# ogulcanaydogan/llm-slo-ebpf-toolkit

Measured on AMD Instinct MI355X. Metric: fault-replay attribution throughput through the agent's BPF-ring -> GPU path (events/s, node-wide); held-out attribution macro-F1 and agent CPU overhead % reported alongside, higher is better.
Workload: dtype fp64 posteriors / fp32 features (exact-int64 time joins)

## Files before the change

### llm_slo_ebpf_toolkit_amd/agent/worker.py

```python

from __future__ import annotations

import collections
import os
import time
import traceback
from dataclasses import dataclass, field
from typing import Deque, Dict, List, Optional, Tuple

import numpy as np

RING_TAIL = 8


@dataclass
class WorkerSpec:
    rank: int
    world: int
    device: int
    engine: str
    source: str
    ring_name: str
    pin_dir: str
    user_rec: int
    sig_cap: int
    span_cap: int
    group_cap: int
    user_cap: int
    window_ms: float
    ttft_slo_ms: float
    halo_ms: float
    import_cap: int
    xchg_cap: int
    model_image: bytes
    pods: Optional[Tuple[np.ndarray, np.ndarray]] = None
    master: Tuple[str, int] = ("127.0.0.1", 0)
    env: Dict[str, str] = field(default_factory=dict)
    halo_windows: int = 3
    split: bool = False
    app_image: bytes = b""
    open_requests: int = 0
    open_reorder_ms: float = 2000.0
    sli_sketch: int = 0
    exemplars: int = 0
    exemplar_windows: int = 3
    pod_breakdown: int = 0
    pod_windows: int = 3
    pod_pairs: int = 4096
    breach_onset: int = 0
    onset_bin_ns: int = 125_000_000
    onset_ref_ppm: int = 20000
    onset_alarm: int = 3


POD_RESULT_KEYS = tuple(f"pod_{s}_{f}" for s in ("win", "rec") for f in ("n", "b", "pods", "pods_b", "k_top", "top"))


def groups_of(rank: int, world: int, n_groups: int) -> int:
    return len(range(rank, n_groups, world))


def merge_results(parts: List[dict], n_groups: int) -> dict:
    world = len(parts)
    out = {}
    for key in ("post", "conf", "feat", "pred", "evbits", "sli", "app", "late", "sli_raw", "late_raw", "deadline",
                "deadline_dup", "ttft_n", "ttft_sum_ms", "ttft_le", "ttft_q", "ttft_q_roll", "ttft_n_roll", "ex_n",
                "ex_k_win", "ex_win", "ex_k_recent", "ex_recent", *POD_RESULT_KEYS, "onset_rows"):
        if key not in parts[0]:
            continue
        ref = np.asarray(parts[0][key])
        arr = np.zeros((n_groups,) + ref.shape[1:], dtype=ref.dtype)
        for r, p in enumerate(parts):
            n = groups_of(r, world, n_groups)
            arr[r::world][:n] = np.asarray(p[key])[:n]
        out[key] = arr
    return out


class PrevJoiner:

    def __init__(self, world: int):
        self.world = int(world)
        self.parts: Dict[int, Dict[int, dict]] = {}

    def add(self, replies) -> List[List[dict]]:
        for r in replies:
            for p in r.get("prevs", ()):
                self.parts.setdefault(int(p["k"]), {})[int(r["rank"])] = p
        out = []
        for k in sorted(self.parts):
            if len(self.parts[k]) < self.world:
                break
            got = self.parts.pop(k)
            out.append([got[i] for i in sorted(got)])
        return out

    def reset(self, world: int) -> None:
        self.world = int(world)
        self.parts.clear()


class WorkerCore:

    def __init__(self, spec: WorkerSpec, comm=None, group=None, shared: bool = True, rings=None):
        from ..collector import bpf
        from ..pipeline.window import RingWindowSource, WindowPipeline
        from ..runtime import load

        self.spec = spec
        shard = spec.rank if spec.split else 0
        if rings is None:
            rt = load()
            names = bpf.RingNames.of(spec.ring_name, shard)
            if spec.source == "bpf":
                ring = rt.Ringbuf.open_pinned(os.path.join(spec.pin_dir, "mislo_events" + (str(shard) if shard else "")))
            else:
                ring = rt.Ringbuf.attach_shm(names.ring)
            rings = (ring, rt.HostRing(0, spec.user_rec, names.user, True), rt.HostRing(0, 64, names.spans, True))
        ring, user, spans = rings
        self.rings = rings
        self.pipe = WindowPipeline(spec.sig_cap, spec.span_cap, spec.group_cap, spec.device, comm, model="bayes",
                                   learn=False, window_ms=2000.0, user_cap=spec.user_cap,
                                   ttft_slo_ms=spec.ttft_slo_ms, halo_ms=spec.halo_ms, halo_windows=spec.halo_windows,
                                   import_cap=spec.import_cap,
                                   xchg_cap=spec.xchg_cap, shard=(spec.rank, spec.world), engine=spec.engine,
                                   group=group, model_image=np.frombuffer(spec.model_image, dtype=np.uint8),
                                   split_rings=spec.split, open_requests=spec.open_requests,
                                   open_reorder_ms=spec.open_reorder_ms, sli_sketch=spec.sli_sketch,
                                   exemplars=spec.exemplars, exemplar_windows=spec.exemplar_windows,
                                   pod_breakdown=spec.pod_breakdown, pod_windows=spec.pod_windows,
                                   pod_pairs=spec.pod_pairs, breach_onset=spec.breach_onset,
                                   onset_bin_ns=spec.onset_bin_ns, onset_ref_ppm=spec.onset_ref_ppm,
                                   onset_alarm=spec.onset_alarm)
        self.src = RingWindowSource(self.pipe, ring, user, spans, cfg_set=lambda i, v: None,
                                    shared=shared and not spec.split)
        if spec.pods is not None:
            self.pipe.eng.set_pods(*spec.pods)
        if spec.app_image:
            from ..ops.engine import app_from_bytes

            img = np.frombuffer(spec.app_image, dtype=np.uint8)
            self.pipe.eng.set_app_model(img)
            self.pipe.app = self.pipe.model.app = app_from_bytes(img)
        self.pending: Deque[Tuple[int, float, int]] = collections.deque()
        self.windows = 0
        self.collect_s = self.collect_wait_s = 0.0

    @classmethod
    def adopt(cls, spec: WorkerSpec, pipe, src) -> "WorkerCore":
        core = cls.__new__(cls)
        core.spec, core.pipe, core.src = spec, pipe, src
        core.rings = (src.ring, src.user_ring, src.span_ring)
        core.pending = collections.deque()
        core.windows = 0
        core.collect_s = core.collect_wait_s = 0.0
        return core

    @property
    def max_pending(self) -> int:
        return max(1, int(self.pipe.nb) - 1)

    def window(self, cut, n_groups: int, pods=None, labels=None) -> dict:
        if pods is not None and len(pods[0]):
            self.pipe.eng.set_pods(*pods)
        t0 = time.perf_counter()
        r = self.src.stage(cut, n_groups, labels, with_labels=labels is not None, learn=False)
        host_us = 1e6 * (time.perf_counter() - t0)
        out = {"rank": self.spec.rank, "k": r["k"], "staged": r, "done": self.src.done()}
        self.pending.append((r["k"], host_us, n_groups))
        prevs = []
        while len(self.pending) > 1 and (len(self.pending) > self.max_pending or
                                         self.pipe.eng.query(self.pending[0][0])):
            prevs.append(self._collect(*self.pending.popleft()))
        out["prevs"] = prevs
        self.windows += 1
        return out

    def start_at(self, kernel: int, user: int, spans: int) -> dict:
        src = self.src
        if src.ring is not None:
            kernel = max(int(kernel), src.kpos)
            src.kpos = src.kernel_done = src.kernel_seen = kernel
            if not src.shared:
                src.ring.set_consumer_pos(max(src.ring.consumer_pos, kernel))
        if src.user_ring is not None:
            du = max(0, int(user) - src.upos)
            src.upos += du
            src._release_user(du, 0)
        if src.span_ring is not None:
            ds = max(0, int(spans) - src.spos)
            src.spos += ds
            src._release_user(0, ds)
        return {"rank": self.spec.rank, "done": src.done()}

    def collect(self, timeout_s: float) -> dict:
        deadline = time.perf_counter() + max(0.0, float(timeout_s))
        prevs = []
        while self.pending:
            k = self.pending[0][0]
            while not self.pipe.eng.query(k):
                if time.perf_counter() >= deadline:
                    return {"rank": self.spec.rank, "prevs": prevs}
                time.sleep(2e-4)
            prevs.append(self._collect(*self.pending.popleft()))
        if prevs:
            self.src.reap()
        return {"rank": self.spec.rank, "prevs": prevs}

    def _collect(self, k: int, host_us: float, n_groups: int) -> dict:
        pipe = self.pipe
        t0 = time.perf_counter()
        pipe.wait(k)
        t1 = time.perf_counter()
        self.collect_wait_s += t1 - t0
        try:
            return self._read(k, host_us, n_groups)
        finally:
            self.collect_s += time.perf_counter() - t0

    def _read(self, k: int, host_us: float, n_groups: int) -> dict:
        pipe = self.pipe
        pk = np.asarray(pipe.eng.packet(k), dtype=np.float64)
        d = {"k": k, "ring": pk[-RING_TAIL:].copy(), "host_us": host_us, "latency_ms": float(pipe.window_ms(k)[0])}
        if self.spec.rank == 0:
            d["packet"] = pk
            d["results"] = pipe.results_all(k, n_groups) if self.spec.world > 1 else [pipe.results(k, n_groups)]
            if pipe.tracker is not None:
                from ..pipeline.openreq import stats_dict

                d["open_requests"] = stats_dict(pipe.open_results(k, n_groups)["stats"])
            if pipe.sketch is not None:
                from ..pipeline.slisketch import stats_dict as sketch_stats

                d["ttft_sketch"] = sketch_stats(pipe.sli_results(k, n_groups)["stats"])
            if pipe.exemplars is not None:
                from ..pipeline.exemplars import stats_dict as exemplar_stats

                d["exemplars"] = exemplar_stats(pipe.exemplar_results(k, n_groups)["stats"])
            if pipe.pods is not None:
                from ..pipeline.podrank import stats_dict as pod_stats

                d["pod_breakdown"] = pod_stats(pipe.pod_results(k, n_groups)["stats"])
            if pipe.onset is not None:
                from ..pipeline.onset import stats_dict as onset_stats

                d["breach_onset"] = onset_stats(pipe.onset_results(k, n_groups)["stats"])
        return d

    def stop(self) -> dict:
        out = {"rank": self.spec.rank, "done": None, "prevs": []}
        while self.pending:
            out["prevs"].append(self._collect(*self.pending.popleft()))
        self.src.drain()
        out["done"] = self.src.done()
        out["summary"] = self.pipe.summary() if self.spec.rank == 0 else None
        return out

    def close(self) -> None:
        self.pipe.close()



def worker_main(spec: WorkerSpec, conn) -> None:
    os.environ.update(spec.env)
    core = None
    group = None
    try:
        comm = None
        if spec.world > 1 and spec.engine == "gpu":
            from ..ops import load_agent

            mod = load_agent()
            if spec.rank == 0:
                uid = mod.unique_id()
                conn.send(("uid", uid))
            else:
                uid = conn.recv()[1]
            comm = (uid, spec.rank, spec.world)
        elif spec.world > 1:
            import torch.distributed as dist

            os.environ.update(MASTER_ADDR=spec.master[0], MASTER_PORT=str(spec.master[1]))
            dist.init_process_group("gloo", rank=spec.rank, world_size=spec.world)
            group = dist.group.WORLD
        core = WorkerCore(spec, comm=comm, group=group, shared=True)
        conn.send(("ready", {"rank": spec.rank, "pid": os.getpid(), "device": spec.device}))
        while True:
            msg = conn.recv()
            if msg[0] == "window":
                conn.send(("window", core.window(*msg[1:])))
            elif msg[0] == "collect":
                conn.send(("collect", core.collect(*msg[1:])))
            elif msg[0] == "start_at":
                conn.send(("start_at", core.start_at(*msg[1:])))
            elif msg[0] == "stop":
                conn.send(("stopped", core.stop()))
                break
            else:
                raise ValueError(f"unknown worker message {msg[0]!r}")
    except (EOFError, KeyboardInterrupt):
        pass
    except Exception:
        try:
            conn.send(("error", traceback.format_exc()))
        except (OSError, BrokenPipeError):
            pass
        raise
    finally:
        if core is not None:
            core.close()
        if group is not None:
            import torch.distributed as dist

            dist.destroy_process_group()


class WorkerError(RuntimeError):
    def __init__(self, msg: str, rank: Optional[int] = None):
        super().__init__(msg)
        self.rank = rank


class RemoteWorker:

    def __init__(self, spec: WorkerSpec, ctx):
        self.spec = spec
        self.conn, child = ctx.Pipe()
        self.proc = ctx.Process(target=worker_main, args=(spec, child), name=f"mislo-worker-{spec.rank}", daemon=True)
        self.proc.start()
        child.close()

    @property
    def pid(self) -> int:
        return int(self.proc.pid or 0)

    def recv(self, timeout: float = 600.0):
        if not self.conn.poll(timeout):
            raise WorkerError(f"worker {self.spec.rank} did not answer in {timeout:.0f} s", self.spec.rank)
        try:
            msg = self.conn.recv()
        except (EOFError, OSError) as exc:
            raise WorkerError(f"worker {self.spec.rank} exited (code {self.proc.exitcode})", self.spec.rank) from exc
        if msg[0] == "error":
            raise WorkerError(f"worker {self.spec.rank} failed:\n{msg[1]}", self.spec.rank)
        return msg

    def ready(self) -> bool:
        return self.conn.poll(0)

    @property
    def alive(self) -> bool:
        return self.proc.is_alive()

    def send(self, msg) -> None:
        self.conn.send(msg)

    def close(self, timeout: float = 30.0) -> None:
        self.proc.join(timeout)
        if self.proc.is_alive():
            self.proc.terminate()
            self.proc.join(10)
        if self.proc.is_alive():
            self.proc.kill()
            self.proc.join(5)


class LocalWorker:

    def __init__(self, spec: WorkerSpec, rings=None):
        self.spec = spec
        self.core = WorkerCore(spec, shared=False, rings=rings)
        self._reply = None

    @property
    def pid(self) -> int:
        return os.getpid()

    def send(self, msg) -> None:
        if msg[0] == "window":
            self._reply = ("window", self.core.window(*msg[1:]))
        elif msg[0] == "collect":
            self._reply = ("collect", self.core.collect(*msg[1:]))
        elif msg[0] == "start_at":
            self._reply = ("start_at", self.core.start_at(*msg[1:]))
        elif msg[0] == "stop":
            self._reply = ("stopped", self.core.stop())

    def recv(self, timeout: float = 600.0):
        r, self._reply = self._reply, None
        return r

    def ready(self) -> bool:
        return True

    alive = True

    def close(self, timeout: float = 30.0) -> None:
        self.core.close()


class WorkerPool:

    def __init__(self, specs: List[WorkerSpec], rings, in_process: bool = False):
        import multiprocessing as mp

        self.rings = rings
        self.world = len(specs)
        if in_process:
            if self.world != 1:
                raise ValueError("in-process workers: exactly one")
            self.workers = [LocalWorker(specs[0], rings)]
        else:
            ctx = mp.get_context("spawn")
            self.workers = [RemoteWorker(s, ctx) for s in specs]
            try:
                if self.world > 1 and specs[0].engine == "gpu":
                    uid = self.workers[0].recv()[1]
                    for w in self.workers[1:]:
                        w.send(("uid", uid))
                for w in self.workers:
                    w.recv()
            except BaseException:
                self.close()
                raise
        self.in_process = in_process
        self.split = bool(specs[0].split) and self.world > 1
        r = rings
        self._rel_user = r[1].tail if r[1] is not None else 0
        self._rel_spans = r[2].tail if r[2] is not None else 0

    def pids(self) -> List[int]:
        return [w.pid for w in self.workers]

    def window(self, cut, n_groups: int, pods=None, timeout: float = 600.0) -> List[dict]:
        for w in self.workers:
            c = cut[w.spec.rank] if isinstance(cut, (list, tuple)) and not hasattr(cut, "kernel") else cut
            try:
                w.send(("window", c, groups_of(w.spec.rank, self.world, n_groups), pods))
            except (OSError, BrokenPipeError) as exc:
                raise WorkerError(f"worker {w.spec.rank} is gone ({exc})", w.spec.rank) from exc
        replies = self._gather(timeout)
        self._release(replies)
        return replies

    def collect(self, wait_s: float, timeout: float = 600.0) -> List[dict]:
        for w in self.workers:
            try:
                w.send(("collect", float(wait_s)))
            except (OSError, BrokenPipeError) as exc:
                raise WorkerError(f"worker {w.spec.rank} is gone ({exc})", w.spec.rank) from exc
        return self._gather(max(timeout, wait_s + 30.0))

    def start_at(self, positions, timeout: float = 120.0) -> List[dict]:
        for w in self.workers:
            pos = positions[w.spec.rank] if isinstance(positions, list) else positions
            try:
                w.send(("start_at",) + tuple(int(x) for x in pos))
            except (OSError, BrokenPipeError) as exc:
                raise WorkerError(f"worker {w.spec.rank} is gone ({exc})", w.spec.rank) from exc
        replies = self._gather(timeout)
        self._release(replies)
        return replies

    def _gather(self, timeout: float) -> List[dict]:
        replies: List[Optional[dict]] = [None] * self.world
        deadline = time.monotonic() + timeout
        while any(r is None for r in replies):
            got = False
            for i, w in enumerate(self.workers):
                if replies[i] is None and w.ready():
                    replies[i] = w.recv()[1]
                    got = True
            if got:
                continue
            dead = self.dead_ranks()
            if dead:
                raise WorkerError(f"worker {dead[0]} exited", dead[0])
            if time.monotonic() > deadline:
                late = next(i for i, r in enumerate(replies) if r is None)
                raise WorkerError(f"worker {late} did not answer in {timeout:.0f} s", late)
            time.sleep(0.0005)
        return replies

    def dead_ranks(self) -> List[int]:
        return [w.spec.rank for w in self.workers if not w.alive]

    def _release(self, replies: List[dict]) -> None:
        if self.in_process or self.split:
            return
        ring, user, spans = self.rings
        dones = [r["done"] for r in replies if r.get("done") is not None]
        if not dones:
            return
        k = min(d[0] for d in dones)
        if ring is not None and k > ring.consumer_pos:
            ring.set_consumer_pos(k)
        u = min(d[1] for d in dones)
        if user is not None and u > self._rel_user:
            user.release(u - self._rel_user)
            self._rel_user = u
        s = min(d[2] for d in dones)
        if spans is not None and s > self._rel_spans:
            spans.release(s - self._rel_spans)
            self._rel_spans = s

    def stop(self) -> List[dict]:
        for w in self.workers:
            w.send(("stop",))
        replies = []
        for w in self.workers:
            try:
                replies.append(w.recv(120)[1])
            except WorkerError:
                replies.append({"rank": w.spec.rank, "done": None})
        self._release(replies)
        return replies

    def close(self, timeout: float = 30.0) -> None:
        for w in self.workers:
            w.close(timeout)
```

### llm_slo_ebpf_toolkit_amd/ops/csrc/agent_bindings.cpp

```cpp
#include <pybind11/numpy.h>
#include <pybind11/pybind11.h>
#include <pybind11/stl.h>

#include <cstring>
#include <memory>
#include <stdexcept>

#include "engine.h"
#include "exemplars.h"
#include "onset.h"
#include "openreq.h"
#include "podrank.h"
#include "slisketch.h"

namespace py = pybind11;
using namespace mislo;

namespace {

template <class T>
py::array_t<T> copy_array(const T* p, std::vector<py::ssize_t> shape) {
  py::array_t<T> a(shape);
  size_t n = 1;
  for (auto s : shape) n *= (size_t)s;
  if (n) std::memcpy(a.mutable_data(), p, n * sizeof(T));
  return a;
}

void set_tables_np(py::array_t<int8_t, py::array::c_style | py::array::forcecast> type_slot,
                   py::array_t<float, py::array::c_style | py::array::forcecast> scale,
                   py::array_t<float, py::array::c_style | py::array::forcecast> warn,
                   py::array_t<float, py::array::c_style | py::array::forcecast> err,
                   py::array_t<float, py::array::c_style | py::array::forcecast> edges) {
  Tables t;
  std::memset(&t, 0, sizeof(t));
  if (type_slot.size() != kMaxTypes || scale.size() != kSlots || warn.size() != kSlots || err.size() != kSlots ||
      edges.size() != kSlots * kBuckets)
    throw std::invalid_argument("table shapes");
  std::memcpy(t.type_slot, type_slot.data(), sizeof(t.type_slot));
  std::memcpy(t.scale, scale.data(), sizeof(t.scale));
  std::memcpy(t.warn, warn.data(), sizeof(t.warn));
  std::memcpy(t.err, err.data(), sizeof(t.err));
  std::memcpy(t.edges, edges.data(), sizeof(t.edges));
  engine_set_tables(t);
}

}

class PyEngine {
 public:
  PyEngine(int device, int sig_cap, int span_cap, int group_cap, int user_cap, int n_buffers, int max_ahead,
           double window_ms, double threshold, int fanout, int group_mode, bool use_graphs, bool device_refit,
           int n_dom, float ttft_slo_ms, double halo_ms, int import_cap, int xchg_cap, int shard_rank,
           int shard_world, int halo_windows, bool split_rings) {
    if (shard_world < 1 || shard_rank < 0 || shard_rank >= shard_world) throw std::invalid_argument("shard rank / world");
    EngineConfig c;
    c.device = device;
    c.sig_cap = sig_cap;
    c.span_cap = span_cap;
    c.group_cap = group_cap;
    c.user_cap = user_cap;
    c.n_buffers = n_buffers;
    c.max_ahead = max_ahead;
    c.window_ms = window_ms;
    c.threshold = threshold;
    c.fanout = fanout;
    c.group_mode = group_mode;
    c.use_graphs = use_graphs;
    c.device_refit = device_refit;
    c.n_dom = n_dom;
    c.ttft_slo_ms = ttft_slo_ms;
    c.halo_ms = halo_ms;
    c.halo_windows = halo_windows;
    c.import_cap = import_cap;
    c.xchg_cap = xchg_cap;
    c.shard_rank = shard_rank;
    c.shard_world = shard_world;
    c.split_rings = split_rings;
    e_ = std::make_unique<WindowEngine>(c);
  }
  bool register_host(uintptr_t addr, size_t bytes) {
    return e_->register_host(reinterpret_cast<const void*>(addr), bytes);
  }
  void submit(int64_t k, const std::vector<std::pair<uintptr_t, size_t>>& kernel,
              const std::vector<std::pair<uintptr_t, size_t>>& user,
              const std::vector<std::pair<uintptr_t, size_t>>& spans, int n_groups, py::object labels,
              std::vector<int64_t> bases, bool with_labels, bool learn, int user_rec) {
    WindowInput in;
    auto conv = [](const std::vector<std::pair<uintptr_t, size_t>>& v, std::vector<Seg>& out) {
      for (auto& p : v) out.push_back(Seg{reinterpret_cast<const void*>(p.first), p.second});
    };
    conv(kernel, in.kernel);
    conv(user, in.user);
    conv(spans, in.spans);
    in.n_groups = n_groups;
    in.user_rec = user_rec;
    std::vector<int32_t> lab;
    if (!labels.is_none()) {
      auto arr = labels.cast<py::array_t<int32_t, py::array::c_style | py::array::forcecast>>();
      lab.assign(arr.data(), arr.data() + arr.size());
      lab.resize(std::max<size_t>(lab.size(), (size_t)std::max(0, n_groups)), -1);
      in.labels = lab.data();
    }
    bases.resize(4, 0);
    for (int q = 0; q < 4; ++q) in.bases[q] = bases[q];
    py::gil_scoped_release nogil;
    e_->submit(k, in, with_labels, learn);
  }
  bool h2d_done(int64_t k) { return e_->h2d_done(k); }
  void wait_h2d(int64_t k) {
    py::gil_scoped_release nogil;
    e_->wait_h2d(k);
  }
  bool query(int64_t k) { return e_->query(k); }
  void wait(int64_t k) {
    py::gil_scoped_release nogil;
    e_->wait(k);
  }
  py::array_t<double> packet(int64_t k) { return copy_array(e_->packet(k), {kPacketLen}); }
  py::dict results(int64_t k, int n_groups) {
    if (n_groups < 0 || n_groups > eng().config().group_cap) throw std::invalid_argument("n_groups");
    return result_dict(e_->results(k), n_groups);
  }
  py::list results_all(int64_t k, int n_groups) {
    WindowEngine& e = eng();
    if (n_groups < 0 || n_groups > e.config().group_cap) throw std::invalid_argument("n_groups");
    const ResultLayout lay = e.layout();
    const uint8_t* base = e.results_all(k);
    py::list out;
    const int w = e.has_comm() ? e.world() : 1;
    for (int r = 0; r < w; ++r) out.append(result_dict(lay.view(base + (size_t)r * lay.bytes()), n_groups));
    return out;
  }
  static py::dict result_dict(const ResultView& r, int n_groups) {
    const py::ssize_t G = n_groups;
    py::dict d;
    d["post"] = copy_array(r.post, {G, 16});
    d["conf"] = copy_array(r.gconf, {G});
    d["feat"] = copy_array(r.feat, {G, 16});
    d["pred"] = copy_array(r.pred, {G});
    d["evbits"] = copy_array(r.evbits, {G, 16});
    d["sli"] = copy_array(r.sli, {G, 2});
    d["app"] = copy_array(r.app, {G, 2});
    d["late"] = copy_array(r.late, {G, 2});
    return d;
  }
  py::tuple window_ms(int64_t k) {
    std::pair<float, float> t;
    {
      py::gil_scoped_release nogil;
      t = e_->window_ms(k);
    }
    return py::make_tuple(t.first, t.second);
  }
  void set_model_bytes(py::array_t<uint8_t, py::array::c_style | py::array::forcecast> b) {
    e_->set_model_bytes(b.data(), (size_t)b.size());
  }
  void set_app_model(py::array_t<uint8_t, py::array::c_style | py::array::forcecast> b) {
    e_->set_app_model(b.data(), (size_t)b.size());
  }
  void set_refit(double alpha, double prior_pseudo, double inv_temp, double min_count, int cap_dom, double ceil) {
    eng().set_refit(alpha, prior_pseudo, inv_temp, min_count, cap_dom, ceil);
  }
  void refit_now() { eng().refit_now(); }
  py::dict score(py::array_t<float, py::array::c_style | py::array::forcecast> feat, py::object labels,
                 py::object app) {
    if (feat.ndim() != 2 || feat.shape(1) != 16) throw std::invalid_argument("feat must be float32 [n, 16]");
    const int n = (int)feat.shape(0);
    std::vector<int32_t> lab;
    if (!labels.is_none()) {
      auto a = labels.cast<py::array_t<int32_t, py::array::c_style | py::array::forcecast>>();
      if (a.size() != n) throw std::invalid_argument("labels must have n entries");
      lab.assign(a.data(), a.data() + n);
    }
    std::vector<uint32_t> appc;
    if (!app.is_none()) {
      auto a = app.cast<py::array_t<uint32_t, py::array::c_style | py::array::forcecast>>();
      if (a.size() != 2 * (py::ssize_t)n) throw std::invalid_argument("app must be uint32 [n, 2]");
      appc.assign(a.data(), a.data() + 2 * (size_t)n);
    }
    std::vector<double> post((size_t)n * 16), conf(n);
    std::vector<int32_t> pred(n);
    std::vector<uint32_t> ev((size_t)n * 16), cm(256);
    {
      py::gil_scoped_release nogil;
      eng().score_features(feat.data(), n, lab.empty() ? nullptr : lab.data(), post.data(), pred.data(), conf.data(),
                           ev.data(), cm.data(), appc.empty() ? nullptr : appc.data());
    }
    py::dict d;
    d["post"] = copy_array(post.data(), {n, 16});
    d["pred"] = copy_array(pred.data(), {n});
    d["conf"] = copy_array(conf.data(), {n});
    d["evbits"] = copy_array(ev.data(), {n, 16});
    d["confusion"] = copy_array(cm.data(), {16, 16});
    return d;
  }
  void set_p0(py::array_t<double, py::array::c_style | py::array::forcecast> p0) {
    if (p0.size() != kSlots * 16 && p0.size() != 2 * kSlots * 16)
      throw std::invalid_argument("p0 must be f64[256] (table) or f64[512] (table, floor)");
    e_->set_p0(p0.data(), (size_t)p0.size());
  }
  void set_pods(py::array_t<uint32_t, py::array::c_style | py::array::forcecast> pods,
                py::array_t<uint32_t, py::array::c_style | py::array::forcecast> sn) {
    if (pods.size() != sn.size()) throw std::invalid_argument("pods / svcnode size mismatch");
    e_->set_pods(pods.data(), sn.data(), (size_t)pods.size());
  }
  void inject_remote(py::buffer blocks, size_t stride, int world, int me) {
    py::buffer_info bi = blocks.request();
    if ((size_t)(bi.size * bi.itemsize) < stride * (size_t)std::max(world, 0)) throw std::invalid_argument("blocks too small");
    py::gil_scoped_release nogil;
    eng().inject_remote(bi.ptr, stride, world, me);
  }
  void set_join_params(double window_ms, double threshold, int fanout, int group_mode) {
    e_->set_join_params(window_ms, threshold, fanout, group_mode);
  }
  void init_comm(py::bytes id, int rank, int world) {
    std::string s = id;
    if (s.size() != sizeof(ncclUniqueId)) throw std::invalid_argument("unique id size");
    ncclUniqueId u;
    std::memcpy(&u, s.data(), sizeof(u));
    py::gil_scoped_release nogil;
    e_->init_comm(u, rank, world);
  }
  py::array_t<double> totals() {
    std::vector<double> t(kPacketLen);
    {
      py::gil_scoped_release nogil;
      e_->totals(t.data());
    }
    return copy_array(t.data(), {kPacketLen});
  }
  void reset_totals() {
    py::gil_scoped_release nogil;
    e_->reset_totals();
  }
  py::array_t<double> stats_acc() {
    std::vector<double> t(kStatsLen);
    {
      py::gil_scoped_release nogil;
      e_->stats_acc(t.data());
    }
    return copy_array(t.data(), {kStatsLen});
  }
  void restore(py::array_t<double, py::array::c_style | py::array::forcecast> stats,
               py::array_t<uint8_t, py::array::c_style | py::array::forcecast> model, int64_t folded) {
    if (stats.size() != kStatsLen) throw std::invalid_argument("stats must be f64[STATS_LEN]");
    eng().restore(stats.data(), model.data(), (size_t)model.size(), folded);
  }
  py::array_t<uint8_t> model_bytes() {
    std::vector<uint8_t> t(sizeof(PosteriorModel));
    {
      py::gil_scoped_release nogil;
      e_->model_bytes(t.data());
    }
    return copy_array(t.data(), {(py::ssize_t)t.size()});
  }
  void sync() {
    py::gil_scoped_release nogil;
    e_->sync();
  }
  std::vector<int64_t> import_state() {
    py::gil_scoped_release nogil;
    return eng().import_state();
  }
  py::bytes sent_block() {
    std::vector<uint8_t> b;
    {
      py::gil_scoped_release nogil;
      b = eng().sent_block();
    }
    return py::bytes(reinterpret_cast<const char*>(b.data()), b.size());
  }
  void close() {
    if (e_) {
      py::gil_scoped_release nogil;
      e_->sync();
      e_.reset();
    }
  }
  WindowEngine& eng() {
    if (!e_) throw std::logic_error("engine closed");
    return *e_;
  }
  int buffers() { return eng().buffers(); }
  int64_t folded() { return eng().windows_folded(); }
  size_t graphs() { return eng().graphs(); }
  double host_issue_us() { return eng().host_issue_us(); }
  double host_wait_us() { return eng().host_wait_us(); }
  double host_dma_issue_us() { return eng().host_dma_issue_us(); }
  double host_launch_us() { return eng().host_launch_us(); }
  bool has_comm() { return eng().has_comm(); }
  size_t staged_bytes() { return eng().staged_bytes(); }
  size_t direct_bytes() { return eng().direct_bytes(); }

 private:
  std::unique_ptr<WindowEngine> e_;
};

class PyOpenRequests {
 public:
  PyOpenRequests(int device, int64_t cap, int span_cap, int group_cap, int n_buffers, double slo_ms, double ttl_ms,
                 double reorder_ms) {
    openreq::Config c;
    c.device = device;
    c.cap = cap;
    c.span_cap = span_cap;
    c.group_cap = group_cap;
    c.n_buffers = n_buffers;
    c.slo_ms = slo_ms;
    c.ttl_ms = ttl_ms;
    c.reorder_ms = reorder_ms;
    openreq::validate(c);
    t_ = std::make_unique<OpenRequests>(c);
  }
  OpenRequests& t() {
    if (!t_) throw std::logic_error("open-request tracker closed");
    return *t_;
  }
  int64_t step(const std::vector<std::pair<uintptr_t, size_t>>& spans, int64_t cut_ns, int64_t prev_cut_ns,
               int n_groups) {
    OpenRequests& tr = t();
    py::gil_scoped_release nogil;
    return tr.step(spans, cut_ns, prev_cut_ns, n_groups);
  }
  bool query(int64_t i) { return t().query(i); }
  py::dict results(int64_t i, int n_groups) {
    OpenRequests& tr = t();
    if (n_groups < 0 || n_groups > tr.config().group_cap) throw std::invalid_argument("n_groups");
    const uint32_t* r;
    {
      py::gil_scoped_release nogil;
      r = tr.results(i);
    }
    const openreq::Layout& l = tr.result_layout();
    py::dict d;
    d["dl"] = copy_array(r + l.dl, {n_groups, 2});
    d["dup"] = copy_array(r + l.dup, {n_groups, 3});
    d["stats"] = copy_array(r + l.stats, {openreq::kStats});
    return d;
  }
  py::tuple step_ms(int64_t i) {
    std::pair<float, float> ms;
    {
      py::gil_scoped_release nogil;
      ms = t().step_ms(i);
    }
    return py::make_tuple(ms.first, ms.second);
  }
  py::tuple entries() {
    std::vector<uint64_t> k;
    std::vector<int64_t> tt;
    std::vector<uint32_t> g, s;
    {
      py::gil_scoped_release nogil;
      t().entries(k, tt, g, s);
    }
    const py::ssize_t n = (py::ssize_t)k.size();
    return py::make_tuple(copy_array(k.data(), {n}), copy_array(tt.data(), {n}), copy_array(g.data(), {n}),
                          copy_array(s.data(), {n}));
  }
  void sync() {
    py::gil_scoped_release nogil;
    t().sync();
  }
  void close() {
    if (t_) {
      py::gil_scoped_release nogil;
      t_.reset();
    }
  }

 private:
  std::unique_ptr<OpenRequests> t_;
};

class PySliSketch {
 public:
  PySliSketch(int device, int span_cap, int group_cap, int windows, int n_buffers) {
    slisketch::Config c;
    c.device = device;
    c.span_cap = span_cap;
    c.group_cap = group_cap;
    c.windows = windows;
    c.n_buffers = n_buffers;
    slisketch::validate(c);
    t_ = std::make_unique<SliSketch>(c);
  }
  SliSketch& t() {
    if (!t_) throw std::logic_error("ttft sketch closed");
    return *t_;
  }
  int64_t step(const std::vector<std::pair<uintptr_t, size_t>>& spans, int n_groups) {
    SliSketch& sk = t();
    py::gil_scoped_release nogil;
    return sk.step(spans, n_groups);
  }
  bool query(int64_t i) { return t().query(i); }
  py::dict results(int64_t i, int n_groups) {
    SliSketch& sk = t();
    if (n_groups < 0 || n_groups > sk.config().group_cap) throw std::invalid_argument("n_groups");
    const uint32_t* r;
    {
      py::gil_scoped_release nogil;
      r = sk.results(i);
    }
    const slisketch::Layout& l = sk.result_layout();
    const py::ssize_t G = n_groups;
    std::vector<uint64_t> sum((size_t)G);
    for (py::ssize_t g = 0; g < G; ++g)
      sum[(size_t)g] = (uint64_t)r[l.sum + 2 * g] | ((uint64_t)r[l.sum + 2 * g + 1] << 32);
    py::dict d;
    d["n"] = copy_array(r + l.n, {G});
    d["sum_milli"] = copy_array(sum.data(), {G});
    d["le"] = copy_array(r + l.le, {G, slisketch::kLe});
    d["q_win"] = copy_array(r + l.q_win, {G, slisketch::kQuantiles});
    d["n_roll"] = copy_array(r + l.n_roll, {G});
    d["q_roll"] = copy_array(r + l.q_roll, {G, slisketch::kQuantiles});
    d["stats"] = copy_array(r + l.stats, {slisketch::kStats});
    return d;
  }
  py::tuple step_ms(int64_t i) {
    std::pair<float, float> ms;
    {
      py::gil_scoped_release nogil;
      ms = t().step_ms(i);
    }
    return py::make_tuple(ms.first, ms.second);
  }
  py::array_t<uint32_t> rolling() { return rows(true); }
  py::array_t<uint32_t> window_hist() { return rows(false); }
  void sync() {
    py::gil_scoped_release nogil;
    t().sync();
  }
  void close() {
    if (t_) {
      py::gil_scoped_release nogil;
      t_.reset();
    }
  }

 private:
  py::array_t<uint32_t> rows(bool roll) {
    SliSketch& sk = t();
    std::vector<uint32_t> h;
    {
      py::gil_scoped_release nogil;
      h = roll ? sk.rolling() : sk.window_hist();
    }
    return copy_array(h.data(), {sk.config().group_cap, slisketch::kK});
  }
  std::unique_ptr<SliSketch> t_;
};

class PyExemplarTracker {
 public:
  PyExemplarTracker(int device, int k, int windows, int64_t span_cap, int group_cap, int n_buffers, bool lds) {
    if (span_cap < 1 || span_cap >= (int64_t(1) << 31))
      throw std::invalid_argument("request exemplars: span_cap must be in [1, 2^31)");
    exemplars::Config c;
    c.device = device;
    c.k = k;
    c.windows = windows;
    c.span_cap = (int)span_cap;
    c.group_cap = group_cap;
    c.n_buffers = n_buffers;
    c.lds = lds;
    exemplars::validate(c);
    t_ = std::make_unique<ExemplarTracker>(c);
  }
  ExemplarTracker& t() {
    if (!t_) throw std::logic_error("request exemplars closed");
    return *t_;
  }
  int64_t step(const std::vector<std::pair<uintptr_t, size_t>>& spans, int n_groups) {
    ExemplarTracker& ex = t();
    py::gil_scoped_release nogil;
    return ex.step(spans, n_groups);
  }
  bool query(int64_t i) { return t().query(i); }
  py::dict results(int64_t i, int n_groups) {
    ExemplarTracker& ex = t();
    if (n_groups < 0 || n_groups > ex.config().group_cap) throw std::invalid_argument("n_groups");
    const uint32_t* r;
    {
      py::gil_scoped_release nogil;
      r = ex.results(i);
    }
    const exemplars::Layout& l = ex.result_layout();
    const py::ssize_t G = n_groups, K = ex.config().k;
    py::dict d;
    d["n"] = copy_array(r + l.n, {G});
    d["k_win"] = copy_array(r + l.k_win, {G});
    d["k_recent"] = copy_array(r + l.k_recent, {G});
    d["win"] = copy_array(reinterpret_cast<const uint8_t*>(r + l.win), {G, K, exemplars::kRowBytes});
    d["recent"] = copy_array(reinterpret_cast<const uint8_t*>(r + l.recent), {G, K, exemplars::kRowBytes});
    d["stats"] = copy_array(r + l.stats, {exemplars::kStats});
    return d;
  }
  py::tuple step_ms(int64_t i) {
    std::vector<float> ms;
    {
      py::gil_scoped_release nogil;
      ms = t().step_ms(i);
    }
    return py::make_tuple(ms[0], ms[1], ms[2]);
  }
  py::tuple resident() {
    ExemplarTracker& ex = t();
    std::pair<std::vector<exemplars::Row>, std::vector<uint32_t>> h;
    {
      py::gil_scoped_release nogil;
      h = ex.resident();
    }
    const py::ssize_t H = ex.config().windows, G = ex.config().group_cap, K = ex.config().k;
    return py::make_tuple(copy_array(reinterpret_cast<const uint8_t*>(h.first.data()), {H, G, K, exemplars::kRowBytes}),
                          copy_array(h.second.data(), {H, G}));
  }
  void sync() {
    py::gil_scoped_release nogil;
    t().sync();
  }
  void close() {
    if (t_) {
      py::gil_scoped_release nogil;
      t_.reset();
    }
  }

 private:
  std::unique_ptr<ExemplarTracker> t_;
};

class PyPodRankTracker {
 public:
  PyPodRankTracker(int device, int k, int windows, int64_t pair_cap, int64_t span_cap, int group_cap, int n_buffers,
                   double slo_ms, bool lds) {
    if (span_cap < 1 || span_cap >= (int64_t(1) << 31))
      throw std::invalid_argument("pod breakdown: span_cap must be >= 1 and span_cap * windows < 2^22");
    if (pair_cap < 1 || pair_cap > podrank::kMaxPairCap)
      throw std::invalid_argument("pod breakdown: pair_cap must be in [1, 2^20]");
    podrank::Config c;
    c.device = device;
    c.k = k;
    c.windows = windows;
    c.pair_cap = (int)pair_cap;
    c.span_cap = (int)span_cap;
    c.group_cap = group_cap;
    c.n_buffers = n_buffers;
    c.slo_ms = slo_ms;
    c.lds = lds;
    podrank::validate(c);
    t_ = std::make_unique<PodRankTracker>(c);
  }
  PodRankTracker& t() {
    if (!t_) throw std::logic_error("pod breakdown closed");
    return *t_;
  }
  int64_t step(const std::vector<std::pair<uintptr_t, size_t>>& spans, int n_groups) {
    PodRankTracker& pr = t();
    py::gil_scoped_release nogil;
    return pr.step(spans, n_groups);
  }
  bool query(int64_t i) { return t().query(i); }
  py::dict results(int64_t i, int n_groups) {
    PodRankTracker& pr = t();
    if (n_groups < 0 || n_groups > pr.config().group_cap) throw std::invalid_argument("n_groups");
    const uint32_t* r;
    {
      py::gil_scoped_release nogil;
      r = pr.results(i);
    }
    const podrank::Layout& l = pr.result_layout();
    const py::ssize_t G = n_groups, K = pr.config().k;
    static const char* scope[2] = {"win", "rec"};
    py::dict d;
    for (int s = 0; s < 2; ++s) {
      const std::string p = std::string(scope[s]) + "_";
      d[py::str(p + "n")] = copy_array(r + l.n[s], {G});
      d[py::str(p + "b")] = copy_array(r + l.b[s], {G});
      d[py::str(p + "pods")] = copy_array(r + l.pods[s], {G});
      d[py::str(p + "pods_b")] = copy_array(r + l.pods_b[s], {G});
      d[py::str(p + "k_top")] = copy_array(r + l.k_top[s], {G});
      d[py::str(p + "top")] = copy_array(reinterpret_cast<const uint8_t*>(r + l.top[s]), {G, K, podrank::kRowBytes});
    }
    d["stats"] = copy_array(r + l.stats, {podrank::kStats});
    return d;
  }
  py::tuple step_ms(int64_t i) {
    std::vector<float> ms;
    {
      py::gil_scoped_release nogil;
      ms = t().step_ms(i);
    }
    return py::make_tuple(ms[0], ms[1], ms[2]);
  }
  py::list resident() {
    PodRankTracker& pr = t();
    std::vector<podrank::PairList> h;
    {
      py::gil_scoped_release nogil;
      h = pr.resident();
    }
    py::list out;
    for (const podrank::PairList& l : h) {
      const py::ssize_t n = (py::ssize_t)l.key.size();
      out.append(py::make_tuple(copy_array(reinterpret_cast<const uint64_t*>(l.key.data()), {n}), copy_array(l.n.data(), {n}),
                                copy_array(l.b.data(), {n}), copy_array(l.max.data(), {n}),
                                copy_array(reinterpret_cast<const uint64_t*>(l.sum.data()), {n})));
    }
    return out;
  }
  void sync() {
    py::gil_scoped_release nogil;
    t().sync();
  }
  void close() {
    if (t_) {
      py::gil_scoped_release nogil;
      t_.reset();
    }
  }

 private:
  std::unique_ptr<PodRankTracker> t_;
};

class PyOnsetTracker {
 public:
  PyOnsetTracker(int device, int64_t bins, int64_t bin_ns, int64_t ref_ppm, int64_t alarm, int64_t span_cap, int group_cap,
                 int n_buffers, double slo_ms, int64_t ring_records_max, bool lds) {
    if (bins < onset::kMinBins || bins > onset::kMaxBins)
      throw std::invalid_argument("breach onset: bins must be a power of two in [64, 8192]");
    if (span_cap < 1) throw std::invalid_argument("breach onset: span_cap must be >= 1");
    if (span_cap >= (int64_t(1) << 31)) throw std::invalid_argument("breach onset: the ring needs more than 2 GiB");
    onset::Config c;
    c.device = device;
    c.bins = (int)bins;
    c.bin_ns = bin_ns;
    c.ref_ppm = ref_ppm;
    c.alarm = alarm;
    c.span_cap = (int)span_cap;
    c.group_cap = group_cap;
    c.n_buffers = n_buffers;
    c.slo_ms = slo_ms;
    c.ring_records_max = ring_records_max;
    c.lds = lds;
    onset::validate(c);
    t_ = std::make_unique<OnsetTracker>(c);
  }
  OnsetTracker& t() {
    if (!t_) throw std::logic_error("breach onset closed");
    return *t_;
  }
  int64_t step(const std::vector<std::pair<uintptr_t, size_t>>& spans, int64_t cut_ns, int n_groups) {
    OnsetTracker& on = t();
    py::gil_scoped_release nogil;
    return on.step(spans, cut_ns, n_groups);
  }
  bool query(int64_t i) { return t().query(i); }
  py::dict results(int64_t i, int n_groups) {
    OnsetTracker& on = t();
    if (n_groups < 0 || n_groups > on.config().group_cap) throw std::invalid_argument("n_groups");
    const uint32_t* r;
    {
      py::gil_scoped_release nogil;
      r = on.results(i);
    }
    const onset::Layout& l = on.result_layout();
    py::dict d;
    d["rows"] = copy_array(reinterpret_cast<const uint8_t*>(r + l.rows), {(py::ssize_t)n_groups, onset::kRowBytes});
    d["stats"] = copy_array(r + l.stats, {onset::kStats});
    return d;
  }
  py::tuple step_ms(int64_t i) {
    std::vector<float> ms;
    {
      py::gil_scoped_release nogil;
      ms = t().step_ms(i);
    }
    return py::make_tuple(ms[0], ms[1], ms[2]);
  }
  py::tuple resident() {
    OnsetTracker& on = t();
    onset::Resident h;
    {
      py::gil_scoped_release nogil;
      h = on.resident();
    }
    return py::make_tuple(copy_array(reinterpret_cast<const uint64_t*>(h.cells.data()),
                                     {(py::ssize_t)on.config().group_cap, (py::ssize_t)on.config().bins}),
                          h.q_hi);
  }
  void sync() {
    py::gil_scoped_release nogil;
    t().sync();
  }
  void close() {
    if (t_) {
      py::gil_scoped_release nogil;
      t_.reset();
    }
  }

 private:
  std::unique_ptr<OnsetTracker> t_;
};

py::bytes unique_id() {
  ncclUniqueId u;
  const ncclResult_t r = ncclGetUniqueId(&u);
  if (r != ncclSuccess) throw std::runtime_error(std::string("ncclGetUniqueId: ") + ncclGetErrorString(r));
  return py::bytes(reinterpret_cast<const char*>(&u), sizeof(u));
}

PYBIND11_MODULE(_mislo_agent, m) {
  m.doc() = "MI355X LLM-SLO native window engine (HIP + RCCL, no PyTorch)";
  m.def("set_tables", &set_tables_np);
  m.def("unique_id", &unique_id);
  m.def("device_count", []() {
    int n = 0;
    return hipGetDeviceCount(&n) == hipSuccess ? n : 0;
  });
  m.attr("PACKET_LEN") = kPacketLen;
  m.attr("PACKET_LAYOUT") = py::make_tuple(kPacketHist, kPacketStatus, kPacketMisc, kPacketDbg, kPacketConf,
                                           kPacketStats, kPacketCount, kPacketRing);
  m.attr("STATS_OFF") = kStatsOff;
  m.attr("STATS_LEN") = kStatsLen;
  m.attr("POSTERIOR_MODEL_BYTES") = (int64_t)sizeof(PosteriorModel);
  m.attr("APP_MODEL_BYTES") = (int64_t)sizeof(AppModel);
  m.attr("APP_EVIDENCE_BIT") = kAppBit;
  m.attr("CTX_ROWS") = kCtxRows;
  m.attr("REC_STRIDE") = kRecStride;
  m.attr("SIGREC_BYTES") = (int)sizeof(SigRec);
  m.attr("RING_STATE") =
      py::make_tuple("first_busy", "foreign", "def_ctx", "def_trace", "discarded", "events", "other_shard");
  m.attr("OPENREQ_LDS_GROUPS") = openreq::kLdsGroups;
  m.attr("OPENREQ_MAX_PROBES") = openreq::kMaxProbes;
  m.attr("OPENREQ_STATS") = (int)openreq::kStats;
  py::class_<PyOpenRequests>(m, "OpenRequests")
      .def(py::init<int, int64_t, int, int, int, double, double, double>(), py::arg("device") = 0,
           py::arg("cap") = (int64_t)1 << 20, py::arg("span_cap") = 16384, py::arg("group_cap") = 64,
           py::arg("n_buffers") = 3, py::arg("slo_ms") = 800.0, py::arg("ttl_ms") = 120000.0,
           py::arg("reorder_ms") = 2000.0)
      .def("step", &PyOpenRequests::step, py::arg("spans"), py::arg("cut_ns"), py::arg("prev_cut_ns"),
           py::arg("n_groups"))
      .def("query", &PyOpenRequests::query)
      .def("results", &PyOpenRequests::results)
      .def("step_ms", &PyOpenRequests::step_ms)
      .def("entries", &PyOpenRequests::entries)
      .def("sync", &PyOpenRequests::sync)
      .def("close", &PyOpenRequests::close);
  m.attr("SLISKETCH_K") = slisketch::kK;
  m.attr("SLISKETCH_LO_KEY") = slisketch::kLo;
  m.attr("SLISKETCH_STATS") = (int)slisketch::kStats;
  {
    py::list edges, q;
    for (int j = 0; j < slisketch::kEdges; ++j) edges.append((double)slisketch::le_edge(j));
    for (int j = 0; j < slisketch::kQuantiles; ++j) q.append(slisketch::quantile_permille(j));
    m.attr("SLISKETCH_EDGES") = py::tuple(edges);
    m.attr("SLISKETCH_PERMILLE") = py::tuple(q);
  }
  py::class_<PySliSketch>(m, "SliSketch")
      .def(py::init<int, int, int, int, int>(), py::arg("device") = 0, py::arg("span_cap") = 16384,
           py::arg("group_cap") = 64, py::arg("windows") = 150, py::arg("n_buffers") = 3)
      .def("step", &PySliSketch::step, py::arg("spans"), py::arg("n_groups"))
      .def("query", &PySliSketch::query)
      .def("results", &PySliSketch::results)
      .def("step_ms", &PySliSketch::step_ms)
      .def("rolling", &PySliSketch::rolling)
      .def("window_hist", &PySliSketch::window_hist)
      .def("sync", &PySliSketch::sync)
      .def("close", &PySliSketch::close);
  m.attr("EXEMPLAR_MAX_K") = exemplars::kMaxK;
  m.attr("EXEMPLAR_MAX_H") = exemplars::kMaxH;
  m.attr("EXEMPLAR_LDS_GROUPS") = exemplars::kLdsGroups;
  m.attr("EXEMPLAR_ROW_BYTES") = exemplars::kRowBytes;
  m.attr("EXEMPLAR_STATS") = (int)exemplars::kStats;
  py::class_<PyExemplarTracker>(m, "ExemplarTracker")
      .def(py::init<int, int, int, int64_t, int, int, bool>(), py::arg("device") = 0, py::arg("k") = 3,
           py::arg("windows") = 3, py::arg("span_cap") = 16384, py::arg("group_cap") = 64, py::arg("n_buffers") = 3,
           py::arg("lds") = true)
      .def("step", &PyExemplarTracker::step, py::arg("spans"), py::arg("n_groups"))
      .def("query", &PyExemplarTracker::query)
      .def("results", &PyExemplarTracker::results)
      .def("step_ms", &PyExemplarTracker::step_ms)
      .def("resident", &PyExemplarTracker::resident)
      .def("sync", &PyExemplarTracker::sync)
      .def("close", &PyExemplarTracker::close);
  m.attr("PODRANK_MAX_K") = podrank::kMaxK;
  m.attr("PODRANK_MAX_H") = podrank::kMaxH;
  m.attr("PODRANK_ROW_BYTES") = podrank::kRowBytes;
  m.attr("PODRANK_STATS") = (int)podrank::kStats;
  m.attr("PODRANK_LDS_SLOTS") = podrank::kLdsSlots;
  m.def("podrank_slot_of", [](uint32_t g, uint32_t pod, uint32_t slots) { return podrank::slot_of(g, pod, slots); });
  py::class_<PyPodRankTracker>(m, "PodRankTracker")
      .def(py::init<int, int, int, int64_t, int64_t, int, int, double, bool>(), py::arg("device") = 0, py::arg("k") = 3,
           py::arg("windows") = 3, py::arg("pair_cap") = 4096, py::arg("span_cap") = 16384, py::arg("group_cap") = 64,
           py::arg("n_buffers") = 3, py::arg("slo_ms") = 800.0, py::arg("lds") = true)
      .def("step", &PyPodRankTracker::step, py::arg("spans"), py::arg("n_groups"))
      .def("query", &PyPodRankTracker::query)
      .def("results", &PyPodRankTracker::results)
      .def("step_ms", &PyPodRankTracker::step_ms)
      .def("resident", &PyPodRankTracker::resident)
      .def("sync", &PyPodRankTracker::sync)
      .def("close", &PyPodRankTracker::close);
  m.attr("ONSET_ROW_BYTES") = onset::kRowBytes;
  m.attr("ONSET_STATS") = (int)onset::kStats;
  m.attr("ONSET_LDS_SLOTS") = onset::kLdsSlots;
  m.attr("ONSET_BINS") = py::make_tuple(onset::kMinBins, onset::kMaxBins);
  py::class_<PyOnsetTracker>(m, "OnsetTracker")
      .def(py::init<int, int64_t, int64_t, int64_t, int64_t, int64_t, int, int, double, int64_t, bool>(),
           py::arg("device") = 0, py::arg("bins") = 1024, py::arg("bin_ns") = (int64_t)125000000,
           py::arg("ref_ppm") = (int64_t)20000, py::arg("alarm") = (int64_t)3, py::arg("span_cap") = 16384,
           py::arg("group_cap") = 64, py::arg("n_buffers") = 3, py::arg("slo_ms") = 800.0,
           py::arg("ring_records_max") = onset::kMaxRingRecords, py::arg("lds") = true)
      .def("step", &PyOnsetTracker::step, py::arg("spans"), py::arg("cut_ns"), py::arg("n_groups"))
      .def("query", &PyOnsetTracker::query)
      .def("results", &PyOnsetTracker::results)
      .def("step_ms", &PyOnsetTracker::step_ms)
      .def("resident", &PyOnsetTracker::resident)
      .def("sync", &PyOnsetTracker::sync)
      .def("close", &PyOnsetTracker::close);
  py::class_<PyEngine>(m, "WindowEngine")
      .def(py::init<int, int, int, int, int, int, int, double, double, int, int, bool, bool, int, float, double, int,
                    int, int, int, int, bool>(),
           py::arg("device") = 0, py::arg("sig_cap") = 1 << 20, py::arg("span_cap") = 16384, py::arg("group_cap") = 64,
           py::arg("user_cap") = 1 << 18, py::arg("n_buffers") = 3, py::arg("max_ahead") = 3,
           py::arg("window_ms") = 2000.0, py::arg("threshold") = 0.7, py::arg("fanout") = 3, py::arg("group_mode") = 1,
           py::arg("use_graphs") = true, py::arg("device_refit") = true, py::arg("n_dom") = 10,
           py::arg("ttft_slo_ms") = 800.0f, py::arg("halo_ms") = 0.0, py::arg("import_cap") = 0,
           py::arg("xchg_cap") = 0, py::arg("shard_rank") = 0, py::arg("shard_world") = 1,
           py::arg("halo_windows") = 3, py::arg("split_rings") = false)
      .def("register_host", &PyEngine::register_host)
      .def("submit", &PyEngine::submit, py::arg("k"), py::arg("kernel"), py::arg("user"), py::arg("spans"),
           py::arg("n_groups"), py::arg("labels") = py::none(), py::arg("bases") = std::vector<int64_t>{},
           py::arg("with_labels") = true, py::arg("learn") = false, py::arg("user_rec") = 64)
      .def("h2d_done", &PyEngine::h2d_done)
      .def("wait_h2d", &PyEngine::wait_h2d)
      .def("query", &PyEngine::query)
      .def("wait", &PyEngine::wait)
      .def("packet", &PyEngine::packet)
      .def("results", &PyEngine::results)
      .def("window_ms", &PyEngine::window_ms)
      .def("copy_ms", [](PyEngine& p, int64_t k) {
        py::gil_scoped_release nogil;
        return p.eng().copy_ms(k);
      })
      .def("set_model_bytes", &PyEngine::set_model_bytes)
      .def("set_app_model", &PyEngine::set_app_model)
      .def("set_p0", &PyEngine::set_p0)
      .def("set_refit", &PyEngine::set_refit, py::arg("alpha") = 2.0, py::arg("prior_pseudo") = 1.0,
           py::arg("inv_temp") = 1.0, py::arg("min_count") = 0.0, py::arg("cap_dom") = -1, py::arg("ceil") = 1.0)
      .def("refit_now", &PyEngine::refit_now)
      .def("set_device_refit", [](PyEngine& p, bool on) { p.eng().set_device_refit(on); })
      .def("score", &PyEngine::score, py::arg("feat"), py::arg("labels") = py::none(), py::arg("app") = py::none())
      .def("set_pods", &PyEngine::set_pods)
      .def("inject_remote", &PyEngine::inject_remote)
      .def("results_all", &PyEngine::results_all)
      .def("set_join_params", &PyEngine::set_join_params)
      .def("init_comm", &PyEngine::init_comm)
      .def("totals", &PyEngine::totals)
      .def("reset_totals", &PyEngine::reset_totals)
      .def("stats_acc", &PyEngine::stats_acc)
      .def("model_bytes", &PyEngine::model_bytes)
      .def("restore", &PyEngine::restore)
      .def("sync", &PyEngine::sync)
      .def("import_state", &PyEngine::import_state)
      .def("sent_block", &PyEngine::sent_block)
      .def("close", &PyEngine::close)
      .def_property_readonly("buffers", &PyEngine::buffers)
      .def_property_readonly("copy_lanes", [](PyEngine& p) { return p.eng().copy_lanes(); })
      .def_property_readonly("windows_folded", &PyEngine::folded)
      .def_property_readonly("graphs", &PyEngine::graphs)
      .def_property_readonly("host_issue_us", &PyEngine::host_issue_us)
      .def_property_readonly("host_wait_us", &PyEngine::host_wait_us)
      .def_property_readonly("host_dma_issue_us", &PyEngine::host_dma_issue_us)
      .def_property_readonly("host_launch_us", &PyEngine::host_launch_us)
      .def_property_readonly("host_pre_us", [](PyEngine& p) { return p.eng().host_pre_us(); })
      .def_property_readonly("host_dma_split_us", [](PyEngine& p) { return p.eng().host_dma_split_us(); })
      .def_property_readonly("host_tail_us", [](PyEngine& p) { return p.eng().host_tail_us(); })
      .def_property_readonly("has_comm", &PyEngine::has_comm)
      .def_property_readonly("rank", [](PyEngine& p) { return p.eng().rank(); })
      .def_property_readonly("world", [](PyEngine& p) { return p.eng().world(); })
      .def_property_readonly("staged_bytes", &PyEngine::staged_bytes)
      .def_property_readonly("direct_bytes", &PyEngine::direct_bytes);
}
```

### llm_slo_ebpf_toolkit_amd/ops/csrc/copylanes.h

```cpp
#pragma once

#include <cstdint>

namespace mislo {

constexpr int kMaxCopyLanes = 2;

inline int copy_lane(int64_t k, int lanes) { return lanes > 1 ? (int)(k % lanes) : 0; }

inline int copy_consults(int64_t k, int lanes, int64_t out[kMaxCopyLanes]) {
  int n = 0;
  for (int i = 0; i < (lanes > 1 ? lanes : 1) && k - i >= 0; ++i) out[n++] = k - i;
  return n;
}

struct CopiedUpTo {
  int64_t n = 0;

  void reused(int64_t k, int nb) {
    if (k - nb + 1 > n) n = k - nb + 1;
  }

  template <class Ready>
  bool done(int64_t k, int lanes, Ready&& ready) {
    if (k < n) return true;
    int64_t w[kMaxCopyLanes];
    const int c = copy_consults(k, lanes, w);
    for (int i = 0; i < c; ++i)
      if (w[i] >= n && !ready(w[i])) return false;
    n = k + 1;
    return true;
  }
};

}
```

### llm_slo_ebpf_toolkit_amd/ops/csrc/engine.h

```cpp
#pragma once

#include <hip/hip_runtime.h>
#include <rccl/rccl.h>

#include <map>
#include <tuple>
#include <type_traits>
#include <vector>

#include "copylanes.h"
#include "mislo_launch.h"
#include "mislo_packet.h"

namespace mislo {

constexpr uint32_t kCtxRows = 1u << 24;
constexpr uint32_t kPodRows = 1u << 20;
constexpr uint32_t kTraceIdRows = 1u << 24;
constexpr int kHeadBytes = 64;

struct Seg {
  const void* ptr;
  size_t bytes;
};

struct EngineConfig {
  int device = 0;
  int sig_cap = 1 << 20, span_cap = 16384, group_cap = 64;
  int user_cap = 1 << 18;
  int n_buffers = 3, max_ahead = 3;
  double window_ms = 2000.0, threshold = 0.7;
  int fanout = 3, group_mode = 1;
  bool use_graphs = true;
  bool device_refit = true;
  double alpha = 2.0, prior_pseudo = 1.0;
  double inv_temp = 1.0, min_count = 0.0;
  int cap_dom = -1;
  double lik_ceil = 1.0;
  int n_dom = 10;
  float ttft_slo_ms = 800.0f;
  double halo_ms = 0.0;
  int halo_windows = 3;
  int import_cap = 0;
  int xchg_cap = 0;
  int shard_rank = 0, shard_world = 1;
  bool split_rings = false;
};

template <class Byte>
struct ResultViewT {
  template <class T>
  using P = std::conditional_t<std::is_const_v<Byte>, const T, T>*;
  P<double> post;
  P<double> gconf;
  P<float> feat;
  P<int32_t> pred;
  P<uint32_t> evbits;
  P<uint32_t> sli;
  P<uint32_t> app;
  P<uint32_t> late;
};
using ResultView = ResultViewT<const uint8_t>;

struct ResultLayout {
  size_t G;
  size_t gconf() const { return 16 * G * 8; }
  size_t feat() const { return gconf() + G * 8; }
  size_t pred() const { return feat() + 16 * G * 4; }
  size_t evbits() const { return pred() + G * 4; }
  size_t sli() const { return evbits() + 16 * G * 4; }
  size_t bytes() const { return sli() + 6 * G * 4; }
  template <class Byte>
  ResultViewT<Byte> view(Byte* r) const {
    ResultViewT<Byte> v;
    auto set = [r](auto& p, size_t off) { p = reinterpret_cast<std::remove_reference_t<decltype(p)>>(r + off); };
    set(v.post, 0), set(v.gconf, gconf()), set(v.feat, feat()), set(v.pred, pred()), set(v.evbits, evbits());
    set(v.sli, sli()), set(v.app, sli() + 2 * G * 4), set(v.late, sli() + 4 * G * 4);
    return v;
  }
};

struct WindowInput {
  std::vector<Seg> kernel;
  std::vector<Seg> user;
  int user_rec = 64;
  std::vector<Seg> spans;
  int n_groups = 0;
  const int32_t* labels = nullptr;
  int64_t bases[4] = {0, 0, 0, 0};
};

class WindowEngine {
 public:
  explicit WindowEngine(const EngineConfig& cfg);
  ~WindowEngine();
  WindowEngine(const WindowEngine&) = delete;
  WindowEngine& operator=(const WindowEngine&) = delete;

  const EngineConfig& config() const { return cfg_; }
  int buffers() const { return nb_; }

  bool register_host(const void* ptr, size_t bytes);
  void submit(int64_t k, const WindowInput& in, bool with_labels, bool learn);
  bool h2d_done(int64_t k);
  void wait_h2d(int64_t k);
  int copy_lanes() const { return lanes_; }
  bool query(int64_t k);
  void wait(int64_t k);
  const double* packet(int64_t k) const { return bufs_[k % nb_].packet_host; }
  ResultView results(int64_t k) const { return layout().view<const uint8_t>(bufs_[k % nb_].res_host); }
  ResultLayout layout() const { return ResultLayout{(size_t)cfg_.group_cap}; }
  std::pair<float, float> window_ms(int64_t k);
  std::vector<float> copy_ms(int64_t k);

  void set_model_bytes(const void* bytes, size_t n);
  void set_refit(double alpha, double prior_pseudo, double inv_temp, double min_count, int cap_dom = -1,
                 double ceil = 1.0);
  void refit_now();
  void set_device_refit(bool on) { cfg_.device_refit = on; }
  void score_features(const float* feat, int n, const int32_t* labels, double* post, int32_t* pred, double* conf,
                      uint32_t* evbits, uint32_t* confusion, const uint32_t* app_cnt = nullptr);
  void set_app_model(const void* bytes, size_t n);
  void set_p0(const double* p0, size_t n);
  void set_pods(const uint32_t* pods, const uint32_t* svcnode, size_t n);
  void inject_remote(const void* blocks, size_t stride, int world, int me);
  void set_join_params(double window_ms, double threshold, int fanout, int group_mode);
  void init_comm(const ncclUniqueId& id, int rank, int world);
  bool has_comm() const { return comm_ != nullptr; }
  int rank() const { return rank_; }
  int world() const { return world_; }
  const uint8_t* results_all(int64_t k) const { return comm_ ? bufs_[k % nb_].res_all_host : bufs_[k % nb_].res_host; }
  size_t result_bytes() const { return layout().bytes(); }

  void totals(double* out);
  void reset_totals();
  void stats_acc(double* out);
  void restore(const double* stats, const void* model, size_t model_bytes, int64_t folded);
  void model_bytes(void* out);
  void sync();
  std::vector<int64_t> import_state();
  std::vector<uint8_t> sent_block();
  int64_t windows_folded() const { return folded_; }
  size_t staged_bytes() const { return staged_bytes_; }
  size_t direct_bytes() const { return direct_bytes_; }
  size_t graphs() const { return graphs_.size(); }
  double host_issue_us() const { return issue_n_ ? issue_us_ / issue_n_ : 0.0; }
  double host_wait_us() const { return issue_n_ ? wait_us_ / issue_n_ : 0.0; }
  double host_dma_issue_us() const { return issue_n_ ? dma_us_ / issue_n_ : 0.0; }
  double host_launch_us() const { return issue_n_ ? launch_us_ / issue_n_ : 0.0; }
  double host_pre_us() const { return issue_n_ ? pre_us_ / issue_n_ : 0.0; }
  double host_tail_us() const { return issue_n_ ? tail_us_ / issue_n_ : 0.0; }

 private:
  int rec_shard_rank() const { return cfg_.split_rings ? 0 : cfg_.shard_rank; }
  int rec_shard_world() const { return cfg_.split_rings ? 1 : cfg_.shard_world; }
  struct Buf;
  enum class Stage : int { Window, Records, Join, XchgSpans, XchgHead, Front, Back };
  static constexpr int kStageSlots = 8;
  void alloc();
  void enable_span_branch();
  void run_begin(const Buf& buf, hipStream_t st);
  void run_part1(const Buf& buf, hipStream_t st, bool xchg);
  void run_join_front(const Buf& buf, hipStream_t st, bool xchg);
  void run_join_back(const Buf& buf, int n_groups, bool with_labels, bool learn, hipStream_t st);
  void run_span_branch(const Buf& buf, hipStream_t st);
  void run_spans(const Buf& buf, hipStream_t st);
  void launch_part(Stage part, const Buf& buf, int n_groups, bool with_labels, bool learn);
  void merge_remote(const Buf& buf, const uint8_t* blocks, size_t stride, int world, int me, hipStream_t st);
  void refit(const double* add);
  SignalCols sig_cols(const Buf& buf) const;
  SpanCols span_cols(const Buf& buf) const;
  bool registered(const void* p, size_t n) const;
  size_t dma(const std::vector<Seg>& segs, uint8_t* dst, size_t cap, uint8_t*& staging, size_t& st_off,
             hipStream_t st);
  struct Owner {
    std::vector<hipEvent_t> events;
    std::vector<void*> dev, host;
    std::vector<hipStream_t> streams;
    void free_dev(void* p);
    ~Owner();
  } own_;
  template <class T>
  T* dalloc(size_t n, bool zero = false);
  void* host_alloc(size_t bytes, unsigned flags);
  void* host_block(size_t bytes);
  hipEvent_t mk_event(unsigned flags);
  hipStream_t mk_stream(bool high_priority = false);

  EngineConfig cfg_;
  int nb_, max_ahead_;
  size_t off_kern_ = 0, off_user_ = 0, off_span_ = 0, in_bytes_ = 0;
  size_t kern_bytes() const { return (size_t)kRecStride * (((size_t)cfg_.sig_cap + kBatchSlots - 1) / kBatchSlots); }
  std::vector<std::pair<const uint8_t*, size_t>> registered_;
  size_t staged_bytes_ = 0, direct_bytes_ = 0;
  uint32_t *pod_sn_ = nullptr, *pod_host_ = nullptr;
  unsigned long long* trace_hash_ = nullptr;
  AppModel* app_dev_ = nullptr;
  int n_rows_ = 0;
  int gens_ = 1;
  int slots_ = 1;
  unsigned long long* tmax_ = nullptr;
  KeyTs* g_keys_ = nullptr;
  uint32_t *remote_n_ = nullptr, *sel_cnt_ = nullptr, *sel_off_ = nullptr;
  unsigned long long* sel_mask_ = nullptr;
  int sel_stride_ = 0;
  uint8_t *xsend_ = nullptr, *xrecv_ = nullptr;
  size_t xstride_ = 0, xrecv_bytes_ = 0;
  int nblk_imp_ = 0;
  bool spin_ = false;
  std::vector<uint8_t> inject_;
  size_t inject_stride_ = 0;
  int inject_world_ = 0, inject_me_ = 0;
  int rank_ = 0, world_ = 1;
  hipStream_t side_ = nullptr;
  hipStream_t front_ = nullptr;
  bool overlap_ = false;
  struct BufSet {
    GenMeta* gen;
    int* rows;
    uint32_t *ring_state, *hist, *status, *confusion, *cnt, *gcnt;
    unsigned long long *misc, *dbg, *top3, *gsum;
    double *stats, *stats_count;
    SpanRec* s_rec;
    PartCodes* s_part;
    uint32_t *s_items, *s_part_base, *probe_work;
    PreSpan* s_pre;
  };
  std::vector<BufSet> sets_;
  struct Buf {
    int b;
    uint8_t* in;
    uint8_t* head_host;
    uint8_t* staging;
    double *packet_dev, *packet_host;
    uint8_t *res_dev, *res_host;
    uint8_t *res_all_dev, *res_all_host;
    ResultViewT<uint8_t> res;
    SigRec* imp;
    uint32_t* remote_n;
    const BufSet* set;
    const GenMeta* gen_prev;
    hipEvent_t h2d_done, head_done, front_done, compute_done, comm_done, xchg_done;
    hipEvent_t t_start, t_comp0, t_comp1, t_end;
    const int* counts() const { return reinterpret_cast<const int*>(in); }
  };
  std::vector<Buf> bufs_;
  hipEvent_t ev_fork_ = nullptr, ev_sigbase_ = nullptr, ev_spans_ = nullptr;
  bool branch_ = false;
  bool xspan_ = false;
  bool exchange() const { return comm_ && cfg_.xchg_cap > 0 && cfg_.import_cap > 0; }
  JoinParams jp_{};
  int nblk_sig_ = 1, nblk_span_ = 1;
  hipStream_t copy_[kMaxCopyLanes] = {nullptr, nullptr};
  int lanes_ = 1;
  CopiedUpTo copied_;
  bool copied_ready(int64_t w, bool block);
  hipStream_t compute_ = nullptr, comm_stream_ = nullptr;
  ncclComm_t comm_ = nullptr;
  ncclComm_t xcomm_ = nullptr;
  uint32_t* ctx_tab_ = nullptr;
  double *totals_ = nullptr, *stats_acc_ = nullptr, *p0_ = nullptr;
  uint8_t* model_dev_ = nullptr;
  std::vector<uint8_t*> model_host_;
  int model_slot_ = 0;
  uint8_t* g_status_ = nullptr;
  PartCodes* g_part_ = nullptr;
  uint32_t *g_part_blk_ = nullptr, *g_part_off_ = nullptr, *g_part_tot_ = nullptr, *g_part_base_ = nullptr,
           *g_items_ = nullptr;
  SigRec* g_rec_ = nullptr;
  uint32_t *s_part_blk_ = nullptr, *s_part_off_ = nullptr, *s_part_tot_ = nullptr;
  float *attrs_ = nullptr, *conf_ = nullptr, *kernel_ms_ = nullptr;
  std::map<std::tuple<int, int, bool, bool>, hipGraphExec_t> graphs_;
  std::vector<bool> warm_;
  std::vector<hipGraph_t> graph_defs_;
  int64_t submitted_ = 0, folded_ = 0;
  double issue_us_ = 0, wait_us_ = 0, dma_us_ = 0, launch_us_ = 0, pre_us_ = 0, tail_us_ = 0;
  double split_us_[4] = {0, 0, 0, 0};

 public:
  std::vector<double> host_dma_split_us() const {
    std::vector<double> v;
    for (double x : split_us_) v.push_back(issue_n_ ? x / issue_n_ : 0.0);
    return v;
  }

 private:
  int64_t issue_n_ = 0;
};

void engine_set_tables(const Tables& t);

}
```

### llm_slo_ebpf_toolkit_amd/ops/csrc/engine.hip

```cpp
#include "engine.h"
#include "mislo_packet_kernels.h"

#include <algorithm>
#include <chrono>
#include <cstdlib>
#include <cmath>
#include <cstring>
#include <stdexcept>
#include <string>

namespace mislo {

namespace {

#define HIPCHECK(x)                                                                                  \
  do {                                                                                               \
    hipError_t _e = (x);                                                                             \
    if (_e != hipSuccess) throw std::runtime_error(std::string("HIP error: ") + hipGetErrorString(_e) + \
                                                   " at " #x);                                       \
  } while (0)

#define NCCLCHECK(x)                                                                                        \
  do {                                                                                                      \
    ncclResult_t _r = (x);                                                                                  \
    if (_r != ncclSuccess) throw std::runtime_error(std::string("RCCL error: ") + ncclGetErrorString(_r) + \
                                                    " at " #x);                                             \
  } while (0)

__global__ void k_accumulate(const double* __restrict__ packet, double* __restrict__ totals, int n,
                             double* __restrict__ host) {
  const int i = blockIdx.x * blockDim.x + threadIdx.x;
  if (i < n) {
    const double v = packet[i];
    totals[i] += v;
    host[i] = v;
  }
}

__global__ __launch_bounds__(256) void k_window_end(const uint32_t* hist, const uint32_t* status,
                                                    const unsigned long long* misc, const unsigned long long* dbg,
                                                    const uint32_t* confusion, const double* stats, const double* count,
                                                    const uint32_t* ring, double* __restrict__ packet,
                                                    double* __restrict__ totals, double* __restrict__ packet_host,
                                                    const uint4* __restrict__ res, uint4* __restrict__ res_host,
                                                    size_t res16) {
  const size_t t = blockIdx.x * (size_t)blockDim.x + threadIdx.x, stride = (size_t)gridDim.x * blockDim.x;
  if (t < (size_t)kPacketLen) {
    const double v = packet_value((int)t, hist, status, misc, dbg, confusion, stats, count, ring);
    packet[t] = v;
    totals[t] += v;
    packet_host[t] = v;
  }
  for (size_t i = t; i < res16; i += stride) res_host[i] = res[i];
}

__global__ void k_to_host(const uint4* __restrict__ src, uint4* __restrict__ dst, size_t n16) {
  for (size_t i = blockIdx.x * (size_t)blockDim.x + threadIdx.x; i < n16; i += (size_t)gridDim.x * blockDim.x)
    dst[i] = src[i];
}

void to_host(const void* src, void* dst, size_t bytes, hipStream_t st) {
  const size_t n16 = (bytes + 15) / 16;
  const int g = (int)std::min<size_t>(64, (n16 + 255) / 256);
  hipLaunchKernelGGL(k_to_host, dim3(g > 0 ? g : 1), dim3(256), 0, st, static_cast<const uint4*>(src),
                     static_cast<uint4*>(dst), n16);
}

constexpr unsigned kEvWait = hipEventDisableTiming | hipEventBlockingSync;
int env_int(const char* name, int unset) {
  const char* v = getenv(name);
  return v ? atoi(v) : unset;
}

struct Lap {
  using clock = std::chrono::steady_clock;
  clock::time_point t = clock::now();
  void operator()(double& acc) {
    const auto n = clock::now();
    acc += std::chrono::duration<double, std::micro>(n - t).count();
    t = n;
  }
};

}

void engine_set_tables(const Tables& t) { set_tables(&t); }

template <class T>
T* WindowEngine::dalloc(size_t n, bool zero) {
  void* p = nullptr;
  HIPCHECK(hipMalloc(&p, n * sizeof(T) + 64));
  own_.dev.push_back(p);
  if (zero) HIPCHECK(hipMemset(p, 0, n * sizeof(T)));
  return static_cast<T*>(p);
}

void* WindowEngine::host_alloc(size_t bytes, unsigned flags) {
  void* h = nullptr;
  HIPCHECK(hipHostMalloc(&h, bytes, flags));
  own_.host.push_back(h);
  return h;
}

void* WindowEngine::host_block(size_t bytes) {
  void* h = host_alloc((bytes + 15) & ~size_t(15), hipHostMallocCoherent | hipHostMallocMapped);
  std::memset(h, 0, bytes);
  return h;
}

hipEvent_t WindowEngine::mk_event(unsigned flags) {
  hipEvent_t e;
  HIPCHECK(hipEventCreateWithFlags(&e, flags));
  own_.events.push_back(e);
  return e;
}

hipStream_t WindowEngine::mk_stream(bool high_priority) {
  hipStream_t s;
  int lo = 0, hi = 0;
  if (high_priority) {
    HIPCHECK(hipDeviceGetStreamPriorityRange(&lo, &hi));
    HIPCHECK(hipStreamCreateWithPriority(&s, hipStreamNonBlocking, hi));
  } else {
    HIPCHECK(hipStreamCreateWithFlags(&s, hipStreamNonBlocking));
  }
  own_.streams.push_back(s);
  return s;
}

void WindowEngine::Owner::free_dev(void* p) {
  if (!p) return;
  dev.erase(std::find(dev.begin(), dev.end(), p));
  HIPCHECK(hipFree(p));
}

WindowEngine::Owner::~Owner() {
  for (hipEvent_t e : events) (void)hipEventDestroy(e);
  for (void* p : host) (void)hipHostFree(p);
  for (void* p : dev) (void)hipFree(p);
  for (hipStream_t s : streams) (void)hipStreamDestroy(s);
}

WindowEngine::WindowEngine(const EngineConfig& cfg) : cfg_(cfg) {
  if (cfg.sig_cap <= 0 || cfg.span_cap <= 0 || cfg.group_cap <= 0 || cfg.group_cap > 4096)
    throw std::invalid_argument("capacities out of range");
  if (cfg.sig_cap >= (1 << 27)) throw std::invalid_argument("sig_cap must be < 2^27 (top-3 key packing)");
  nb_ = std::max(2, cfg.n_buffers);
  max_ahead_ = std::min(nb_, std::max(1, cfg.max_ahead));
  if (cfg.user_cap <= 0 || cfg.user_cap > cfg.sig_cap) throw std::invalid_argument("user_cap must be in [1, sig_cap]");
  if (cfg.import_cap < 0 || cfg.xchg_cap < 0 || cfg.halo_ms < 0) throw std::invalid_argument("negative import sizes");
  if (cfg.halo_windows < 1 || cfg.halo_windows >= kMaxGens)
    throw std::invalid_argument("halo_windows must be in [1, 3] (resident generations)");
  gens_ = cfg.halo_ms > 0 ? 1 + cfg.halo_windows : 1;
  if (2LL * gens_ * ((long long)cfg.sig_cap + cfg.import_cap) >= (1LL << 27))
    throw std::invalid_argument("2 x generations x (sig_cap + import_cap) must be < 2^27 (top-3 key packing)");
  HIPCHECK(hipSetDevice(cfg.device));
  set_join_params(cfg.window_ms, cfg.threshold, cfg.fanout, cfg.group_mode);
  alloc();
}

void WindowEngine::set_join_params(double window_ms, double threshold, int fanout, int group_mode) {
  const int64_t ms = 1000000;
  int64_t outer = (int64_t)llround(window_ms * ms);
  if (outer <= 0) outer = 2000 * ms;
  if (outer >= (1LL << 35)) throw std::invalid_argument("window too large for top-3 key packing (< 34 s)");
  jp_.outer_ns = outer;
  const int64_t tw[4] = {outer, 100 * ms, 250 * ms, 500 * ms};
  for (int k = 0; k < 4; ++k) jp_.win_ns[k] = std::min(outer, tw[k]);
  const float cf[4] = {1.0f, 0.9f, 0.8f, 0.65f};
  for (int k = 0; k < 4; ++k) jp_.conf[k] = cf[k];
  jp_.threshold = threshold > 0 ? (float)threshold : 0.7f;
  if (fanout <= 0) fanout = 3;
  if (fanout > 3) throw std::invalid_argument("GPU join keeps at most 3 candidates per span");
  jp_.fanout = fanout;
  jp_.group_mode = group_mode;
  graphs_.clear();
}

void WindowEngine::alloc() {
  const int64_t S = cfg_.span_cap, G = cfg_.group_cap;
  n_rows_ = cfg_.sig_cap + cfg_.import_cap;
  const int64_t N = n_rows_;
  nblk_sig_ = decode_grid((int)N);
  nblk_span_ = decode_grid((int)S);
  const bool one_stream = env_int("MISLO_ONE_STREAM", 0) == 1;
  compute_ = mk_stream();
  copy_[0] = one_stream ? compute_ : mk_stream();
  spin_ = env_int("MISLO_SPIN_WAIT", 0) == 1;
  overlap_ = env_int("MISLO_WINDOW_OVERLAP", !one_stream) == 1 && !one_stream &&
             !(cfg_.xchg_cap > 0 && cfg_.import_cap > 0);
  if (overlap_) front_ = mk_stream();
  lanes_ = overlap_ && env_int("MISLO_COPY_LANES", nb_ >= 4 ? 2 : 1) == 2 ? 2 : 1;
  copy_[1] = lanes_ == 2 ? mk_stream(env_int("MISLO_COPY_LANE_PRIO", 1) != 0) : copy_[0];
  slots_ = gens_ + (overlap_ ? 1 : 0);
  {
    if (env_int("MISLO_SPAN_STREAM", !one_stream && !overlap_) == 1) enable_span_branch();
  }
  comm_stream_ = compute_;
  const size_t head = (kHeadBytes + 4 * (size_t)G + 63) & ~size_t(63);
  off_kern_ = head;
  off_user_ = (off_kern_ + kern_bytes() + 63) & ~size_t(63);
  off_span_ = off_user_ + 64 * (size_t)cfg_.user_cap;
  in_bytes_ = off_span_ + 64 * (size_t)S;
  const ResultLayout lay = layout();
  bufs_.assign(nb_, Buf{});
  for (Buf& buf : bufs_) {
    buf.in = dalloc<uint8_t>(in_bytes_, true);
    buf.head_host = static_cast<uint8_t*>(host_block(head));
    buf.packet_dev = dalloc<double>(kPacketLen, true);
    buf.packet_host = static_cast<double*>(host_block(kPacketLen * sizeof(double)));
    for (hipEvent_t* e : {&buf.head_done, &buf.compute_done, &buf.comm_done, &buf.front_done, &buf.xchg_done})
      *e = mk_event(kEvWait);
    buf.h2d_done = mk_event(hipEventBlockingSync);
    for (hipEvent_t* e : {&buf.t_start, &buf.t_comp0, &buf.t_comp1, &buf.t_end})
      *e = mk_event(hipEventDefault);
    buf.res_host = static_cast<uint8_t*>(host_block(lay.bytes()));
    buf.res_dev = dalloc<uint8_t>(lay.bytes(), true);
    buf.res = lay.view(buf.res_dev);
    buf.imp = cfg_.import_cap ? dalloc<SigRec>(cfg_.import_cap) : nullptr;
  }
  warm_.assign(kStageSlots * nb_, false);
  pod_sn_ = dalloc<uint32_t>(kPodRows, true);
  pod_host_ = static_cast<uint32_t*>(host_alloc(kPodRows * 4, hipHostMallocDefault));
  std::memset(pod_host_, 0, kPodRows * 4);
  trace_hash_ = dalloc<unsigned long long>(kTraceIdRows, true);
  tmax_ = dalloc<unsigned long long>(1, true);
  remote_n_ = dalloc<uint32_t>(nb_, true);
  for (int i = 0; i < (overlap_ ? nb_ : 1); ++i) {
    BufSet s{};
    s.rows = dalloc<int>(16, true);
    s.ring_state = dalloc<uint32_t>(kRsLen);
    s.gen = dalloc<GenMeta>(1);
    GenMeta g{};
    g.cur = (uint32_t)slots_ - 1;
    for (int a = 0; a < kMaxGens; ++a) g.cut[a] = INT64_MAX;
    HIPCHECK(hipMemcpy(s.gen, &g, sizeof(g), hipMemcpyHostToDevice));
    s.s_part = dalloc<PartCodes>(S);
    s.s_part_base = dalloc<uint32_t>(kKeyTypes * kParts + 1);
    s.s_items = dalloc<uint32_t>(kKeyTypes * S);
    s.s_pre = dalloc<PreSpan>((size_t)kKeyTypes * S);
    s.s_rec = dalloc<SpanRec>(S);
    s.probe_work = dalloc<uint32_t>(kProbeWorkLen, true);
    s.top3 = dalloc<unsigned long long>(3 * S);
    s.cnt = dalloc<uint32_t>(S);
    s.gsum = dalloc<unsigned long long>((size_t)kGroupStripes * G * kSlots);
    s.gcnt = dalloc<uint32_t>((size_t)kGroupStripes * G * kSlots);
    s.hist = dalloc<uint32_t>(kSlots * kBuckets);
    s.status = dalloc<uint32_t>(kSlots * 3);
    s.misc = dalloc<unsigned long long>(kPacketMisc);
    s.dbg = dalloc<unsigned long long>(kPacketDbg);
    s.confusion = dalloc<uint32_t>(kMaxDomains * kMaxDomains);
    s.stats = dalloc<double>(32 * 32);
    s.stats_count = dalloc<double>(kMaxDomains);
    sets_.push_back(s);
  }
  for (int b = 0; b < nb_; ++b) {
    bufs_[b].b = b;
    bufs_[b].set = &sets_[overlap_ ? b : 0];
    bufs_[b].gen_prev = sets_[overlap_ ? (b + nb_ - 1) % nb_ : 0].gen;
    bufs_[b].remote_n = remote_n_ + b;
  }
  sel_cnt_ = dalloc<uint32_t>(1024);
  sel_off_ = dalloc<uint32_t>(1024);
  xstride_ = sizeof(XRec) * (1 + (size_t)cfg_.xchg_cap);
  if (cfg_.xchg_cap) {
    xsend_ = dalloc<uint8_t>(xstride_, true);
    if (env_int("MISLO_SEL_TWO_PASS", 0) != 1) {
      sel_stride_ = decode_sel_stride(n_rows_);
      sel_mask_ = dalloc<unsigned long long>((size_t)decode_grid(n_rows_) * (size_t)sel_stride_);
    }
  }
  ctx_tab_ = dalloc<uint32_t>((size_t)kCtxRows * 4, true);
  totals_ = dalloc<double>(kPacketLen, true);
  stats_acc_ = dalloc<double>(kStatsLen, true);
  p0_ = dalloc<double>(2 * kSlots * 16, true);
  model_dev_ = dalloc<uint8_t>(sizeof(PosteriorModel), true);
  app_dev_ = dalloc<AppModel>(1, true);
  for (int i = 0; i < max_ahead_ + 2; ++i)
    model_host_.push_back(static_cast<uint8_t*>(host_alloc(sizeof(PosteriorModel), hipHostMallocDefault)));
  g_status_ = dalloc<uint8_t>(N);
  g_part_ = dalloc<PartCodes>(N);
  nblk_imp_ = cfg_.xchg_cap ? decode_grid(7 * cfg_.xchg_cap) : 0;
  g_part_blk_ = dalloc<uint32_t>((size_t)(nblk_sig_ + nblk_imp_) * kKeyTypes * kParts);
  g_part_off_ = dalloc<uint32_t>((size_t)(nblk_sig_ + nblk_imp_) * kKeyTypes * kParts);
  g_part_tot_ = dalloc<uint32_t>(kKeyTypes * kParts);
  g_part_base_ = dalloc<uint32_t>((size_t)slots_ * kBaseLen);
  g_items_ = dalloc<uint32_t>((size_t)slots_ * kKeyTypes * N);
  g_keys_ = dalloc<KeyTs>((size_t)slots_ * kKeyTypes * N);
  g_rec_ = dalloc<SigRec>((size_t)slots_ * N);
  s_part_blk_ = dalloc<uint32_t>((size_t)nblk_span_ * kKeyTypes * kParts);
  s_part_off_ = dalloc<uint32_t>((size_t)nblk_span_ * kKeyTypes * kParts);
  s_part_tot_ = dalloc<uint32_t>(kKeyTypes * kParts);
  attrs_ = dalloc<float>(S * kSlots);
  conf_ = dalloc<float>(S);
  kernel_ms_ = dalloc<float>(S);
  HIPCHECK(hipDeviceSynchronize());
}

WindowEngine::~WindowEngine() {
  (void)hipDeviceSynchronize();
  for (auto& kv : graphs_) (void)hipGraphExecDestroy(kv.second);
  for (auto g : graph_defs_) (void)hipGraphDestroy(g);
  if (xcomm_) ncclCommDestroy(xcomm_);
  if (comm_) ncclCommDestroy(comm_);
  for (auto& r : registered_) (void)hipHostUnregister(const_cast<uint8_t*>(r.first));
}

void WindowEngine::enable_span_branch() {
  if (branch_) return;
  side_ = mk_stream(env_int("MISLO_SPAN_STREAM_PRIO", 0) == 1);
  for (hipEvent_t* e : {&ev_fork_, &ev_sigbase_, &ev_spans_}) *e = mk_event(hipEventDisableTiming);
  xspan_ = env_int("MISLO_XCHG_SPAN_SIDE", 1) != 0;
  branch_ = true;
}

SignalCols WindowEngine::sig_cols(const Buf& buf) const {
  return SignalCols{g_rec_, g_status_, g_part_, g_items_, g_keys_, g_part_base_, buf.set->gen, (int64_t)n_rows_, gens_,
                    slots_};
}
SpanCols WindowEngine::span_cols(const Buf& buf) const { return SpanCols{buf.set->s_rec, buf.set->s_part}; }

bool WindowEngine::register_host(const void* ptr, size_t bytes) {
  if (!ptr || !bytes) return false;
  if (registered(ptr, bytes)) return true;
  if (hipHostRegister(const_cast<void*>(ptr), bytes, hipHostRegisterDefault) != hipSuccess) {
    (void)hipGetLastError();
    return false;
  }
  registered_.emplace_back(static_cast<const uint8_t*>(ptr), bytes);
  return true;
}

bool WindowEngine::registered(const void* p, size_t n) const {
  const uint8_t* q = static_cast<const uint8_t*>(p);
  for (const auto& r : registered_)
    if (q >= r.first && q + n <= r.first + r.second) return true;
  return false;
}

size_t WindowEngine::dma(const std::vector<Seg>& segs, uint8_t* dst, size_t cap, uint8_t*& staging, size_t& st_off,
                         hipStream_t st) {
  size_t off = 0;
  for (const Seg& s : segs) {
    if (!s.bytes) continue;
    if (off + s.bytes > cap) throw std::invalid_argument("window input exceeds the engine's capacity");
    const void* src = s.ptr;
    if (!registered(s.ptr, s.bytes)) {
      if (!staging) staging = static_cast<uint8_t*>(host_alloc(in_bytes_ - off_kern_, hipHostMallocDefault));
      std::memcpy(staging + st_off, s.ptr, s.bytes);
      src = staging + st_off;
      st_off += s.bytes;
      staged_bytes_ += s.bytes;
    } else {
      direct_bytes_ += s.bytes;
    }
    HIPCHECK(hipMemcpyAsync(dst + off, src, s.bytes, hipMemcpyHostToDevice, st));
    off += s.bytes;
  }
  return off;
}

bool WindowEngine::copied_ready(int64_t w, bool block) {
  const hipEvent_t ev = bufs_[w % nb_].h2d_done;
  if (block) {
    HIPCHECK(hipEventSynchronize(ev));
    return true;
  }
  const hipError_t e = hipEventQuery(ev);
  if (e == hipErrorNotReady) return false;
  HIPCHECK(e);
  return true;
}

bool WindowEngine::h2d_done(int64_t k) {
  if (k < 0 || k >= submitted_) return false;
  return copied_.done(k, lanes_, [this](int64_t w) { return copied_ready(w, false); });
}

void WindowEngine::wait_h2d(int64_t k) {
  if (k < 0 || k >= submitted_) throw std::invalid_argument("wait_h2d: the window has not been submitted");
  copied_.done(k, lanes_, [this](int64_t w) { return copied_ready(w, true); });
}

void WindowEngine::run_begin(const Buf& buf, hipStream_t st) {
  const BufSet& s = *buf.set;
  const int S = cfg_.span_cap, G = cfg_.group_cap;
  FillList fl{};
  auto add = [&](void* p, size_t bytes, uint32_t v) { fl.seg[fl.count++] = FillSeg{(uint32_t*)p, (uint32_t)(bytes / 4), v}; };
  add(s.hist, kSlots * kBuckets * 4, 0);
  add(s.status, kSlots * 3 * 4, 0);
  add(s.misc, kPacketMisc * 8, 0);
  add(s.dbg, kPacketDbg * 8, 0);
  add(s.confusion, kMaxDomains * kMaxDomains * 4, 0);
  add(s.stats, 32 * 32 * 8, 0);
  add(s.stats_count, kMaxDomains * 8, 0);
  add(s.top3, 3 * (size_t)S * 8, 0xFFFFFFFFu);
  add(s.cnt, (size_t)S * 4, 0);
  add(s.gsum, (size_t)kGroupStripes * G * kSlots * 8, 0);
  add(s.gcnt, (size_t)kGroupStripes * G * kSlots * 4, 0);
  add(buf.res.sli, (size_t)G * 6 * 4, 0);
  launch_window_begin(fl, s.gen, buf.gen_prev, tmax_, gens_, slots_, (long long)llround(cfg_.halo_ms * 1e6),
                      s.ring_state, buf.remote_n, buf.counts(), n_rows_, s.rows, st);
}

void WindowEngine::run_part1(const Buf& buf, hipStream_t st, bool xchg) {
  const BufSet& s = *buf.set;
  const int* counts = buf.counts();
  const int N = n_rows_;
  if (!(xchg && xspan_)) run_begin(buf, st);
  if (branch_ && !xchg) run_span_branch(buf, st);
  const TraceIds tt{trace_hash_, kTraceIdRows};
  launch_ring_defs(buf.in + off_kern_, counts, cfg_.sig_cap, ctx_tab_, kCtxRows, pod_sn_, kPodRows, tt, s.ring_state,
                   st);
  const bool fused_sel = xchg && sel_mask_;
  launch_decode_window(buf.in + off_kern_, buf.in + off_user_, counts, s.rows, N, buf.imp, ctx_tab_, (int)kCtxRows, tt,
                       s.ring_state, tmax_, pod_sn_, kPodRows, sig_cols(buf), s.hist, s.status, g_part_blk_, s.misc, st,
                       0, 0, 0, rec_shard_rank(), rec_shard_world(), fused_sel ? sel_cnt_ : nullptr,
                       fused_sel ? sel_mask_ : nullptr, sel_stride_);
  if (fused_sel)
    launch_select_masked(sig_cols(buf), s.rows, N, sel_cnt_, sel_off_, sel_mask_, sel_stride_,
                         reinterpret_cast<XRec*>(xsend_ + sizeof(XRec)), reinterpret_cast<uint32_t*>(xsend_),
                         (uint32_t)cfg_.xchg_cap, st, s.dbg + kDbgXchgDropped);
  else if (xchg)
    launch_select(sig_cols(buf), s.rows, counts, N, sel_cnt_, sel_off_, reinterpret_cast<XRec*>(xsend_ + sizeof(XRec)),
                  reinterpret_cast<uint32_t*>(xsend_), (uint32_t)cfg_.xchg_cap, st, s.dbg + kDbgXchgDropped);
}

void WindowEngine::run_join_front(const Buf& buf, hipStream_t st, bool xchg) {
  const BufSet& s = *buf.set;
  const int N = n_rows_;
  if (xchg) {
    const TraceIds tt{trace_hash_, kTraceIdRows};
    launch_decode_window(buf.in + off_kern_, buf.in + off_user_, buf.counts(), s.rows, N, buf.imp, ctx_tab_,
                         (int)kCtxRows, tt, s.ring_state, tmax_, pod_sn_, kPodRows, sig_cols(buf), s.hist, s.status,
                         g_part_blk_, s.misc, st, 1, nblk_imp_, nblk_sig_, rec_shard_rank(), rec_shard_world());
  }
  const bool branched = branch_ && !xchg;
  hipEvent_t sig_base = branched ? ev_sigbase_ : nullptr;
  if (!branched && !(xchg && xspan_)) run_spans(buf, st);
  const uint32_t* wspan = branched ? nullptr : s.s_part_base;
  const JoinParams* wjp = branched ? nullptr : &jp_;
  uint32_t* wlist = branched ? nullptr : s.probe_work;
  launch_partition_sig(sig_cols(buf), s.rows, N, nblk_sig_ + (xchg ? nblk_imp_ : 0), g_part_blk_, g_part_off_,
                       g_part_tot_, st, xchg ? nblk_sig_ : 0, sig_base, wspan, wjp, wlist);
  if (branched) {
    HIPCHECK(hipStreamWaitEvent(side_, ev_sigbase_, 0));
    launch_probe_work(s.s_part_base, sig_cols(buf), jp_, s.probe_work, side_);
    HIPCHECK(hipEventRecord(ev_spans_, side_));
    HIPCHECK(hipStreamWaitEvent(st, ev_spans_, 0));
  }
}

void WindowEngine::run_join_back(const Buf& buf, int n_groups, bool with_labels, bool learn, hipStream_t st) {
  const BufSet& s = *buf.set;
  const ResultViewT<uint8_t>& r = buf.res;
  const int* counts = buf.counts();
  const int32_t* labels = reinterpret_cast<const int32_t*>(buf.in + kHeadBytes);
  const int S = cfg_.span_cap, G = cfg_.group_cap;
  launch_probe(span_cols(buf), s.s_items, s.s_part_base, sig_cols(buf), S, jp_, s.top3, s.cnt, n_groups, s.gsum, s.gcnt,
               s.dbg, s.probe_work, s.s_pre, st);
  launch_finalize(counts + 1, S, s.top3, s.cnt, sig_cols(buf), span_cols(buf), jp_, nullptr, attrs_, conf_, kernel_ms_,
                  n_groups, s.gsum, s.gcnt, r.feat, s.dbg, st);
  const PosteriorModel* pm = reinterpret_cast<const PosteriorModel*>(model_dev_);
  if (learn)
    launch_posterior_stats(r.feat, counts + 2, G, pm, with_labels ? labels : nullptr, r.post, r.pred, r.gconf, r.evbits,
                           s.confusion, labels, nullptr, s.stats, s.stats_count, st, app_dev_, r.app);
  else
    launch_posterior(r.feat, counts + 2, G, pm, with_labels ? labels : nullptr, r.post, r.pred, r.gconf, r.evbits,
                     s.confusion, st, app_dev_, r.app);
  if (!comm_) {
    const size_t res16 = (result_bytes() + 15) / 16;
    const int g = (int)std::max<size_t>((kPacketLen + 255) / 256, std::min<size_t>(64, (res16 + 255) / 256));
    hipLaunchKernelGGL(k_window_end, dim3(g), dim3(256), 0, st, s.hist, s.status, s.misc, s.dbg, s.confusion, s.stats,
                       s.stats_count, s.ring_state, buf.packet_dev, totals_, buf.packet_host,
                       reinterpret_cast<const uint4*>(buf.res_dev), reinterpret_cast<uint4*>(buf.res_host), res16);
    return;
  }
  hipLaunchKernelGGL(k_pack, dim3((kPacketLen + 255) / 256), dim3(256), 0, st, s.hist, s.status, s.misc, s.dbg,
                     s.confusion, s.stats, s.stats_count, s.ring_state, buf.packet_dev);
}

void WindowEngine::run_spans(const Buf& buf, hipStream_t st) {
  const BufSet& s = *buf.set;
  const int* counts = buf.counts();
  const int S = cfg_.span_cap, G = cfg_.group_cap;
  const SpanMap sm{1, buf.res.sli, G, cfg_.ttft_slo_ms, cfg_.shard_rank, cfg_.shard_world,
                   s.gen, buf.res.app, buf.res.late};
  launch_decode_spans(buf.in + off_span_, counts + 1, S, span_cols(buf), s_part_blk_, ctx_tab_, (int)kCtxRows, st, &sm);
  launch_partition(s.s_part, counts + 1, S, nblk_span_, s_part_blk_, s_part_off_, s_part_tot_, s.s_part_base, s.s_items,
                   st);
  launch_span_sort(span_cols(buf), s.s_items, s.s_part_base, s.s_pre, st);
}

void WindowEngine::run_span_branch(const Buf& buf, hipStream_t st) {
  HIPCHECK(hipEventRecord(ev_fork_, st));
  HIPCHECK(hipStreamWaitEvent(side_, ev_fork_, 0));
  run_spans(buf, side_);
}

void WindowEngine::launch_part(Stage part, const Buf& buf, int n_groups, bool with_labels, bool learn) {
  hipStream_t cs = part == Stage::XchgSpans ? side_ : part == Stage::Front ? front_ : compute_;
  auto run = [&] {
    switch (part) {
      case Stage::Window:
        run_part1(buf, cs, false);
        run_join_front(buf, cs, false);
        return run_join_back(buf, n_groups, with_labels, learn, cs);
      case Stage::Records: return run_part1(buf, cs, true);
      case Stage::Join:
        run_join_front(buf, cs, true);
        return run_join_back(buf, n_groups, with_labels, learn, cs);
      case Stage::XchgSpans: return run_spans(buf, cs);
      case Stage::XchgHead: return run_begin(buf, cs);
      case Stage::Front:
        run_part1(buf, cs, false);
        return run_join_front(buf, cs, false);
      case Stage::Back: return run_join_back(buf, n_groups, with_labels, learn, cs);
    }
  };
  if (!cfg_.use_graphs) return run();
  const int slot = buf.b * kStageSlots + (int)part;
  auto key = part == Stage::Front ? std::make_tuple(slot, 0, false, false)
                                  : std::make_tuple(slot, n_groups, with_labels, learn);
  auto it = graphs_.find(key);
  if (it == graphs_.end() && !warm_[slot]) {
    run();
    warm_[slot] = true;
    return;
  }
  if (it == graphs_.end()) {
    hipGraph_t g;
    HIPCHECK(hipStreamBeginCapture(cs, hipStreamCaptureModeThreadLocal));
    run();
    HIPCHECK(hipStreamEndCapture(cs, &g));
    hipGraphExec_t ex;
    HIPCHECK(hipGraphInstantiate(&ex, g, nullptr, nullptr, 0));
    graph_defs_.push_back(g);
    it = graphs_.emplace(key, ex).first;
  }
  HIPCHECK(hipGraphLaunch(it->second, cs));
}

void WindowEngine::merge_remote(const Buf& buf, const uint8_t* blocks, size_t stride, int world, int me,
                                hipStream_t st) {
  launch_remote_merge(blocks, stride, world, me, buf.imp, buf.remote_n, (uint32_t)cfg_.import_cap, cfg_.xchg_cap, st,
                      buf.set->dbg + kDbgXchgDropped);
  launch_window_rows(buf.counts(), buf.remote_n, n_rows_, buf.set->rows, buf.set->gen, st);
}

void WindowEngine::refit(const double* add) {
  launch_refit_nb(stats_acc_, add, p0_, cfg_.alpha, cfg_.prior_pseudo, cfg_.n_dom,
                  reinterpret_cast<PosteriorModel*>(model_dev_), compute_, cfg_.inv_temp, cfg_.min_count,
                  p0_ + kSlots * 16, cfg_.cap_dom, cfg_.lik_ceil);
}

void WindowEngine::submit(int64_t k, const WindowInput& in, bool with_labels, bool learn) {
  Lap whole;
  if (k != submitted_) throw std::invalid_argument("windows must be submitted in order");
  const int n_groups = in.n_groups;
  if (n_groups < 0 || n_groups > cfg_.group_cap) throw std::invalid_argument("n_groups exceeds group capacity");
  size_t kb = 0, ub = 0, sb = 0;
  for (const Seg& s : in.kernel) kb += s.bytes;
  for (const Seg& s : in.user) ub += s.bytes;
  for (const Seg& s : in.spans) sb += s.bytes;
  if (in.user_rec != 64 && in.user_rec != 32 && in.user_rec != 24 && in.user_rec != 16)
    throw std::invalid_argument("user records are 64, 32, 24 or 16 bytes");
  if (kb % kRecStride || ub % in.user_rec || sb % 64) throw std::invalid_argument("segments must hold whole records");
  const size_t n_k = kb / kRecStride * kBatchSlots, n_u = ub / in.user_rec, n_s = sb / 64;
  if (n_k + n_u > (size_t)cfg_.sig_cap || n_u > (size_t)cfg_.user_cap || n_s > (size_t)cfg_.span_cap)
    throw std::invalid_argument("window exceeds the engine's capacity (events / user records / spans)");
  Buf& buf = bufs_[k % nb_];
  Lap phase;
  if (k >= max_ahead_) HIPCHECK(hipEventSynchronize(bufs_[(k - max_ahead_) % nb_].compute_done));
  if (k >= nb_) {
    HIPCHECK(hipEventSynchronize(buf.h2d_done));
    copied_.reused(k, nb_);
    HIPCHECK(hipEventSynchronize(buf.head_done));
  }
  phase(wait_us_);
  int32_t* c = reinterpret_cast<int32_t*>(buf.head_host);
  std::memset(c, 0, kHeadBytes);
  c[0] = (int32_t)(n_k + n_u);
  c[1] = (int32_t)n_s;
  c[2] = n_groups;
  c[4] = (int32_t)(uint32_t)(uint64_t)in.bases[0];
  c[5] = (int32_t)(uint32_t)((uint64_t)in.bases[0] >> 32);
  c[6] = in.user_rec;
  c[7] = 64;
  for (int q = 1; q < 4; ++q) {
    c[8 + 2 * (q - 1)] = (int32_t)(uint32_t)(uint64_t)in.bases[q];
    c[9 + 2 * (q - 1)] = (int32_t)(uint32_t)((uint64_t)in.bases[q] >> 32);
  }
  c[15] = (int32_t)n_k;
  int32_t* lab = reinterpret_cast<int32_t*>(buf.head_host + kHeadBytes);
  for (int g = 0; g < cfg_.group_cap; ++g) lab[g] = (in.labels && g < n_groups) ? in.labels[g] : -1;
  const hipStream_t cs = copy_[copy_lane(k, lanes_)];
  HIPCHECK(hipEventRecord(buf.t_start, cs));
  size_t st_off = 0;
  Lap part;
  dma(in.kernel, buf.in + off_kern_, kern_bytes(), buf.staging, st_off, cs);
  part(split_us_[0]);
  part(split_us_[1]);
  dma(in.user, buf.in + off_user_, 64 * (size_t)cfg_.user_cap, buf.staging, st_off, cs);
  part(split_us_[2]);
  dma(in.spans, buf.in + off_span_, 64 * (size_t)cfg_.span_cap, buf.staging, st_off, cs);
  part(split_us_[3]);
  HIPCHECK(hipEventRecord(buf.h2d_done, cs));
  phase(dma_us_);
  hipStream_t fs = overlap_ ? front_ : compute_;
  HIPCHECK(hipStreamWaitEvent(fs, buf.h2d_done, 0));
  if (overlap_ && k >= 2) HIPCHECK(hipStreamWaitEvent(fs, bufs_[(k - 2) % nb_].compute_done, 0));
  HIPCHECK(hipStreamWaitEvent(compute_, buf.comm_done, 0));
  const bool injected = !inject_.empty();
  if (injected) {
    HIPCHECK(hipMemcpyAsync(xrecv_, inject_.data(), inject_.size(), hipMemcpyHostToDevice, compute_));
    HIPCHECK(hipStreamSynchronize(compute_));
  }
  HIPCHECK(hipEventRecord(buf.t_comp0, fs));
  to_host(buf.head_host, buf.in, off_kern_, fs);
  HIPCHECK(hipEventRecord(buf.head_done, fs));
  if (cfg_.device_refit && k >= nb_) {
    refit(buf.packet_dev + kStatsOff);
    ++folded_;
  }
  const bool xchg = exchange() || injected;
  phase(pre_us_);
  if (overlap_) {
    if (xchg) throw std::logic_error("the exchange path does not run with overlapped windows");
    launch_part(Stage::Front, buf, n_groups, with_labels, learn);
    HIPCHECK(hipEventRecord(buf.front_done, front_));
    HIPCHECK(hipStreamWaitEvent(compute_, buf.front_done, 0));
    launch_part(Stage::Back, buf, n_groups, with_labels, learn);
  } else if (!xchg) {
    launch_part(Stage::Window, buf, n_groups, with_labels, learn);
  } else {
    if (xspan_) {
      launch_part(Stage::XchgHead, buf, n_groups, with_labels, learn);
      HIPCHECK(hipEventRecord(ev_fork_, compute_));
      HIPCHECK(hipStreamWaitEvent(side_, ev_fork_, 0));
      launch_part(Stage::XchgSpans, buf, n_groups, with_labels, learn);
      HIPCHECK(hipEventRecord(ev_spans_, side_));
    }
    launch_part(Stage::Records, buf, n_groups, with_labels, learn);
    if (injected) {
      merge_remote(buf, xrecv_, inject_stride_, inject_world_, inject_me_, compute_);
      inject_.clear();
    } else if (xcomm_) {
      NCCLCHECK(ncclAllGather(xsend_, xrecv_, xstride_, ncclUint8, xcomm_, compute_));
      merge_remote(buf, xrecv_, xstride_, world_, rank_, compute_);
    } else {
      HIPCHECK(hipEventRecord(buf.xchg_done, compute_));
      HIPCHECK(hipStreamWaitEvent(comm_stream_, buf.xchg_done, 0));
      NCCLCHECK(ncclAllGather(xsend_, xrecv_, xstride_, ncclUint8, comm_, comm_stream_));
      merge_remote(buf, xrecv_, xstride_, world_, rank_, comm_stream_);
      HIPCHECK(hipEventRecord(buf.xchg_done, comm_stream_));
      HIPCHECK(hipStreamWaitEvent(compute_, buf.xchg_done, 0));
    }
    if (xspan_) HIPCHECK(hipStreamWaitEvent(compute_, ev_spans_, 0));
    launch_part(Stage::Join, buf, n_groups, with_labels, learn);
  }
  phase(launch_us_);
  const size_t res_bytes = result_bytes();
  if (comm_) to_host(buf.res_dev, buf.res_host, res_bytes, compute_);
  HIPCHECK(hipEventRecord(buf.t_comp1, compute_));
  HIPCHECK(hipEventRecord(buf.compute_done, compute_));
  HIPCHECK(hipStreamWaitEvent(comm_stream_, buf.compute_done, 0));
  if (comm_) {
    NCCLCHECK(ncclGroupStart());
    NCCLCHECK(ncclAllReduce(buf.packet_dev, buf.packet_dev, kPacketLen - kPacketRing, ncclFloat64, ncclSum, comm_,
                            comm_stream_));
    NCCLCHECK(ncclAllGather(buf.res_dev, buf.res_all_dev, res_bytes, ncclUint8, comm_, comm_stream_));
    NCCLCHECK(ncclGroupEnd());
    to_host(buf.res_all_dev, buf.res_all_host, res_bytes * world_, comm_stream_);
    hipLaunchKernelGGL(k_accumulate, dim3((kPacketLen + 255) / 256), dim3(256), 0, comm_stream_, buf.packet_dev,
                       totals_, kPacketLen, buf.packet_host);
  }
  HIPCHECK(hipEventRecord(buf.t_end, comm_stream_));
  HIPCHECK(hipEventRecord(buf.comm_done, comm_stream_));
  ++submitted_;
  phase(tail_us_);
  whole(issue_us_);
  ++issue_n_;
}

bool WindowEngine::query(int64_t k) {
  const hipError_t e = hipEventQuery(bufs_[k % nb_].comm_done);
  if (e == hipSuccess) return true;
  if (e == hipErrorNotReady) return false;
  HIPCHECK(e);
  return false;
}

void WindowEngine::wait(int64_t k) {
  if (spin_) {
    while (!query(k)) {
    }
    return;
  }
  HIPCHECK(hipEventSynchronize(bufs_[k % nb_].comm_done));
}

std::vector<float> WindowEngine::copy_ms(int64_t k) {
  const Buf& buf = bufs_[k % nb_];
  float dur = 0.f, gap = -1.f;
  HIPCHECK(hipEventSynchronize(buf.h2d_done));
  HIPCHECK(hipEventElapsedTime(&dur, buf.t_start, buf.h2d_done));
  if (k >= 1 && nb_ > 1) HIPCHECK(hipEventElapsedTime(&gap, bufs_[(k - 1) % nb_].h2d_done, buf.t_start));
  return {dur, gap};
}

std::pair<float, float> WindowEngine::window_ms(int64_t k) {
  const Buf& buf = bufs_[k % nb_];
  float total = 0.f, comp = 0.f;
  HIPCHECK(hipEventSynchronize(buf.t_end));
  HIPCHECK(hipEventElapsedTime(&total, buf.t_start, buf.t_end));
  HIPCHECK(hipEventElapsedTime(&comp, buf.t_comp0, buf.t_comp1));
  return {total, comp};
}

void WindowEngine::set_model_bytes(const void* bytes, size_t n) {
  if (n != sizeof(PosteriorModel)) throw std::invalid_argument("model image must be POSTERIOR_MODEL_BYTES bytes");
  uint8_t* h = model_host_[model_slot_++ % model_host_.size()];
  std::memcpy(h, bytes, n);
  HIPCHECK(hipMemcpyAsync(model_dev_, h, n, hipMemcpyHostToDevice, compute_));
}

void WindowEngine::set_app_model(const void* bytes, size_t n) {
  if (n != sizeof(AppModel)) throw std::invalid_argument("application model must be APP_MODEL_BYTES bytes");
  uint8_t* h = model_host_[model_slot_++ % model_host_.size()];
  static_assert(sizeof(AppModel) <= sizeof(PosteriorModel), "the staging slots fit the application model");
  std::memcpy(h, bytes, n);
  HIPCHECK(hipMemcpyAsync(app_dev_, h, n, hipMemcpyHostToDevice, compute_));
}

void WindowEngine::set_p0(const double* p0, size_t n) {
  if (n != (size_t)kSlots * 16 && n != 2 * (size_t)kSlots * 16) throw std::invalid_argument("p0 must be f64[256] or [512]");
  HIPCHECK(hipMemset(p0_ + kSlots * 16, 0, kSlots * 16 * sizeof(double)));
  HIPCHECK(hipMemcpy(p0_, p0, n * sizeof(double), hipMemcpyHostToDevice));
}

void WindowEngine::set_refit(double alpha, double prior_pseudo, double inv_temp, double min_count, int cap_dom,
                             double ceil) {
  if (!(alpha > 0.0) || !(prior_pseudo >= 0.0) || !(inv_temp > 0.0) || !(min_count >= 0.0) || cap_dom >= cfg_.n_dom ||
      !(ceil > 0.0 && ceil <= 1.0))
    throw std::invalid_argument("refit parameters");
  cfg_.lik_ceil = ceil;
  cfg_.cap_dom = cap_dom < 0 ? -1 : cap_dom;
  cfg_.alpha = alpha;
  cfg_.prior_pseudo = prior_pseudo;
  cfg_.inv_temp = inv_temp;
  cfg_.min_count = min_count;
}

void WindowEngine::refit_now() { refit(nullptr); }

void WindowEngine::score_features(const float* feat, int n, const int32_t* labels, double* post, int32_t* pred,
                                  double* conf, uint32_t* evbits, uint32_t* confusion, const uint32_t* app_cnt) {
  if (n < 0) throw std::invalid_argument("n");
  sync();
  if (n == 0) return;
  const size_t o_n = (size_t)n * 16 * 4, o_lab = o_n + 64, o_post = (o_lab + (size_t)n * 4 + 63) & ~size_t(63);
  const size_t o_pred = o_post + (size_t)n * 16 * 8, o_conf = (o_pred + (size_t)n * 4 + 63) & ~size_t(63);
  const size_t o_ev = o_conf + (size_t)n * 8, o_cm = o_ev + (size_t)n * 16 * 4, o_app = o_cm + 16 * 16 * 4;
  const size_t bytes = o_app + (size_t)n * 2 * 4;
  uint8_t* d = dalloc<uint8_t>(bytes, true);
  HIPCHECK(hipMemcpy(d, feat, o_n, hipMemcpyHostToDevice));
  HIPCHECK(hipMemcpy(d + o_n, &n, sizeof(int), hipMemcpyHostToDevice));
  if (labels) HIPCHECK(hipMemcpy(d + o_lab, labels, (size_t)n * 4, hipMemcpyHostToDevice));
  if (app_cnt) HIPCHECK(hipMemcpy(d + o_app, app_cnt, (size_t)n * 2 * 4, hipMemcpyHostToDevice));
  launch_posterior(reinterpret_cast<const float*>(d), reinterpret_cast<const int*>(d + o_n), n,
                   reinterpret_cast<const PosteriorModel*>(model_dev_),
                   labels ? reinterpret_cast<const int32_t*>(d + o_lab) : nullptr, reinterpret_cast<double*>(d + o_post),
                   reinterpret_cast<int32_t*>(d + o_pred), reinterpret_cast<double*>(d + o_conf),
                   reinterpret_cast<uint32_t*>(d + o_ev), reinterpret_cast<uint32_t*>(d + o_cm), compute_,
                   app_cnt ? app_dev_ : nullptr, app_cnt ? reinterpret_cast<const uint32_t*>(d + o_app) : nullptr);
  HIPCHECK(hipStreamSynchronize(compute_));
  HIPCHECK(hipMemcpy(post, d + o_post, (size_t)n * 16 * 8, hipMemcpyDeviceToHost));
  HIPCHECK(hipMemcpy(pred, d + o_pred, (size_t)n * 4, hipMemcpyDeviceToHost));
  HIPCHECK(hipMemcpy(conf, d + o_conf, (size_t)n * 8, hipMemcpyDeviceToHost));
  HIPCHECK(hipMemcpy(evbits, d + o_ev, (size_t)n * 16 * 4, hipMemcpyDeviceToHost));
  HIPCHECK(hipMemcpy(confusion, d + o_cm, 16 * 16 * 4, hipMemcpyDeviceToHost));
  own_.free_dev(d);
}

void WindowEngine::set_pods(const uint32_t* pods, const uint32_t* svcnode, size_t n) {
  hipStream_t st = overlap_ ? front_ : compute_;
  HIPCHECK(hipStreamSynchronize(st));
  for (size_t i = 0; i < n; ++i)
    if (pods[i] < kPodRows) pod_host_[pods[i]] = svcnode[i];
  HIPCHECK(hipMemcpyAsync(pod_sn_, pod_host_, kPodRows * 4, hipMemcpyHostToDevice, st));
}

std::vector<uint8_t> WindowEngine::sent_block() {
  sync();
  std::vector<uint8_t> out(xsend_ ? xstride_ : 0);
  if (xsend_) HIPCHECK(hipMemcpy(out.data(), xsend_, xstride_, hipMemcpyDeviceToHost));
  return out;
}

std::vector<int64_t> WindowEngine::import_state() {
  sync();
  int rows[2];
  unsigned long long tmax = 0;
  GenMeta g{};
  std::vector<uint32_t> r(nb_);
  const BufSet& s = *bufs_[submitted_ ? (submitted_ - 1) % nb_ : 0].set;
  HIPCHECK(hipMemcpy(rows, s.rows, sizeof(rows), hipMemcpyDeviceToHost));
  HIPCHECK(hipMemcpy(&tmax, tmax_, 8, hipMemcpyDeviceToHost));
  HIPCHECK(hipMemcpy(&g, s.gen, sizeof(g), hipMemcpyDeviceToHost));
  HIPCHECK(hipMemcpy(r.data(), remote_n_, 4 * nb_, hipMemcpyDeviceToHost));
  std::vector<int64_t> out{rows[0], rows[1], (int64_t)tmax, gens_, g.cur, g.filled};
  for (int a = 0; a < kMaxGens; ++a) out.push_back(g.cut[a]);
  for (int a = 0; a < kMaxGens; ++a) out.push_back(a < gens_ ? g.n_rows[(g.cur + slots_ - a) % slots_] : 0);
  for (int b = 0; b < nb_; ++b) out.push_back(r[b]);
  return out;
}

void WindowEngine::inject_remote(const void* blocks, size_t stride, int world, int me) {
  if (!cfg_.import_cap || !cfg_.xchg_cap) throw std::logic_error("inject_remote needs import_cap and xchg_cap > 0");
  if (world < 1 || me < 0 || me >= world || stride < sizeof(XRec)) throw std::invalid_argument("bad exchange blocks");
  const uint8_t* h = static_cast<const uint8_t*>(blocks);
  for (int r = 0; r < world; ++r) {
    uint32_t c;
    std::memcpy(&c, h + (size_t)r * stride, 4);
    if ((size_t)c * sizeof(XRec) + sizeof(XRec) > stride) throw std::invalid_argument("block row count exceeds stride");
    if (r != me && c > (uint32_t)cfg_.xchg_cap) throw std::invalid_argument("block holds more rows than xchg_cap");
  }
  if (stride * world > xrecv_bytes_) {
    sync();
    own_.free_dev(xrecv_);
    xrecv_ = dalloc<uint8_t>(stride * world);
    xrecv_bytes_ = stride * world;
  }
  inject_.assign(h, h + stride * world);
  inject_stride_ = stride;
  inject_world_ = world;
  inject_me_ = me;
}

void WindowEngine::init_comm(const ncclUniqueId& id, int rank, int world) {
  if (comm_) throw std::logic_error("communicator already initialised");
  if (world < 1 || rank < 0 || rank >= world) throw std::invalid_argument("communicator rank / world");
  if (submitted_) throw std::logic_error("init_comm before the first window");
  HIPCHECK(hipSetDevice(cfg_.device));
  if (overlap_) {
    HIPCHECK(hipStreamSynchronize(front_));
    overlap_ = false;
    lanes_ = 1;
    if (!getenv("MISLO_SPAN_STREAM")) enable_span_branch();
  }
  NCCLCHECK(ncclCommInitRank(&comm_, world, id, rank));
  {
    comm_stream_ = mk_stream(env_int("MISLO_COMM_STREAM_PRIO", 1) != 0);
  }
  rank_ = rank;
  world_ = world;
  for (Buf& buf : bufs_) {
    buf.res_all_dev = dalloc<uint8_t>(result_bytes() * world);
    buf.res_all_host = static_cast<uint8_t*>(host_block(result_bytes() * world));
  }
  if (cfg_.xchg_cap) {
    if (world > 8) throw std::invalid_argument("the exchange is sized for <= 8 GPUs per node");
    own_.free_dev(xrecv_);
    xrecv_bytes_ = xstride_ * world;
    xrecv_ = dalloc<uint8_t>(xrecv_bytes_, true);
    const char* xv = getenv("MISLO_XCHG_STREAM");
    int split = (xv && std::strcmp(xv, "compute") == 0) ? 1 : 0;
    int* d_split = dalloc<int>(1);
    HIPCHECK(hipMemcpy(d_split, &split, sizeof(int), hipMemcpyHostToDevice));
    NCCLCHECK(ncclBroadcast(d_split, d_split, 1, ncclInt32, 0, comm_, comm_stream_));
    HIPCHECK(hipStreamSynchronize(comm_stream_));
    HIPCHECK(hipMemcpy(&split, d_split, sizeof(int), hipMemcpyDeviceToHost));
    own_.free_dev(d_split);
    if (split) NCCLCHECK(ncclCommSplit(comm_, 0, rank, &xcomm_, nullptr));
  }
}

void WindowEngine::totals(double* out) {
  sync();
  HIPCHECK(hipMemcpy(out, totals_, kPacketLen * sizeof(double), hipMemcpyDeviceToHost));
}

void WindowEngine::reset_totals() {
  sync();
  HIPCHECK(hipMemset(totals_, 0, kPacketLen * sizeof(double)));
}

void WindowEngine::stats_acc(double* out) {
  sync();
  HIPCHECK(hipMemcpy(out, stats_acc_, kStatsLen * sizeof(double), hipMemcpyDeviceToHost));
}

void WindowEngine::restore(const double* stats, const void* model, size_t n, int64_t folded) {
  if (n && n != sizeof(PosteriorModel)) throw std::invalid_argument("model image must be POSTERIOR_MODEL_BYTES bytes");
  sync();
  HIPCHECK(hipMemcpy(stats_acc_, stats, kStatsLen * sizeof(double), hipMemcpyHostToDevice));
  if (n) {
    HIPCHECK(hipMemcpy(model_dev_, model, n, hipMemcpyHostToDevice));
  } else {
    refit(nullptr);
    HIPCHECK(hipStreamSynchronize(compute_));
  }
  folded_ = folded;
}

void WindowEngine::model_bytes(void* out) {
  sync();
  HIPCHECK(hipMemcpy(out, model_dev_, sizeof(PosteriorModel), hipMemcpyDeviceToHost));
}

void WindowEngine::sync() {
  HIPCHECK(hipStreamSynchronize(copy_[0]));
  if (copy_[1] != copy_[0]) HIPCHECK(hipStreamSynchronize(copy_[1]));
  if (front_) HIPCHECK(hipStreamSynchronize(front_));
  HIPCHECK(hipStreamSynchronize(compute_));
  HIPCHECK(hipStreamSynchronize(comm_stream_));
}

}
```

### llm_slo_ebpf_toolkit_amd/pipeline/cpu.py

```python

from __future__ import annotations

import time
from dataclasses import dataclass
from typing import Dict, Optional

import numpy as np

from ..collector import records
from ..models.bayes import N_DOMAINS, LinearPosteriorModel, SufficientStats, app_counts, soft_labels
from . import oracle
from .window import PACKET_LAYOUT

PACKET_LEN = sum(PACKET_LAYOUT)


@dataclass
class CpuWindowResult:
    packet: np.ndarray
    feat: np.ndarray
    post: np.ndarray
    pred: np.ndarray
    join: oracle.JoinResult


STATS_OFF, STATS_LEN = sum(PACKET_LAYOUT[:5]), PACKET_LAYOUT[5] + PACKET_LAYOUT[6]


def build_packet(hist, status, misc, dbg, confusion, stats: SufficientStats) -> np.ndarray:
    p = np.zeros(PACKET_LEN, dtype=np.float64)
    o = 0
    parts = []
    st = np.zeros((32, 32))
    st[:16, :N_DOMAINS] = stats.elevated_sum
    st[16:, :N_DOMAINS] = stats.x_sum
    st[16:, 16:] = stats.xx
    cnt = np.zeros(16)
    cnt[:N_DOMAINS] = stats.count
    for arr in (hist, status, misc, dbg, confusion, st, cnt):
        parts.append(np.asarray(arr, dtype=np.float64).ravel())
    for part, n in zip(parts, PACKET_LAYOUT):
        assert part.size == n, (part.size, n)
        p[o:o + n] = part
        o += n
    return p


class CpuWindowEngine:
    def __init__(self, model: LinearPosteriorModel, window_ms: float = 2000.0, threshold: float = 0.7,
                 fanout: int = 3, group_mode: int = 1):
        self.model = model
        self.window_ms, self.threshold, self.fanout, self.group_mode = window_ms, threshold, fanout, group_mode

    def run(self, events: np.ndarray, spans: np.ndarray, n_groups: int, labels: Optional[np.ndarray] = None,
            n_local: Optional[int] = None, learn: bool = False, reduce_groups=None) -> CpuWindowResult:
        d = oracle.decode_events(events)
        n = events.shape[0]
        nl = n if n_local is None else int(n_local)
        loc = oracle.Decoded(*(getattr(d, f)[:nl] for f in ("ts", "val", "slot", "status", "pod", "pid",
                                                            "svcnode", "trace", "conn")))
        hist = oracle.histograms(loc)
        status = np.zeros((16, 3), dtype=np.int64)
        ok = loc.slot != oracle.NO_SLOT
        np.add.at(status, (loc.slot[ok].astype(np.int64), loc.status[ok].astype(np.int64)), 1)
        misc = np.zeros(PACKET_LAYOUT[2], dtype=np.int64)
        misc[0] = int((~ok).sum())
        misc[1] = int((loc.ts == 0).sum())
        misc[2:18] = oracle.value_sums_milli(loc)
        j = oracle.join(d, spans, n_groups, self.window_ms, self.threshold, self.fanout, self.group_mode)
        dbg = np.zeros(PACKET_LAYOUT[3], dtype=np.int64)
        dbg[0] = j.debug["candidates"]
        dbg[1] = j.debug["low_confidence"]
        dbg[3] = j.debug["fanout_dropped"]
        dbg[4] = j.debug["spans_enriched"]
        gsum, gcnt = j.gsum, j.gcnt
        if reduce_groups is not None:
            gsum, gcnt = reduce_groups(gsum, gcnt)
        feat = oracle.group_features(gsum, gcnt).astype(np.float64)
        post = self.model.posteriors(feat)
        pred = self.model.predict(feat) if n_groups else np.zeros(0, dtype=np.int64)
        conf = np.zeros((16, 16), dtype=np.int64)
        stats = SufficientStats()
        if labels is not None and n_groups:
            lab = np.asarray(labels[:n_groups], dtype=np.int64)
            m = lab >= 0
            np.add.at(conf, (lab[m], pred[m]), 1)
            if learn and m.any():
                stats.add(feat[m], lab[m])
        return CpuWindowResult(build_packet(hist, status, misc, dbg, conf, stats), feat.astype(np.float32), post,
                               pred, j)

    @staticmethod
    def unpack(packet: np.ndarray) -> Dict[str, np.ndarray]:
        from .window import unpack_packet

        return unpack_packet(packet)



def _read(addr: int, n: int) -> np.ndarray:
    import ctypes

    if n <= 0:
        return np.zeros(0, dtype=np.uint8)
    return np.ctypeslib.as_array((ctypes.c_uint8 * int(n)).from_address(int(addr))).copy()


def _gather(segs) -> np.ndarray:
    parts = [_read(a, n) for a, n in segs]
    return np.concatenate(parts) if parts else np.zeros(0, dtype=np.uint8)


def shard_owner(svcnode: np.ndarray, world: int) -> np.ndarray:
    svc = (np.asarray(svcnode, dtype=np.uint32) >> np.uint32(16)).astype(np.int64)
    return np.where(svc > 0, (svc - 1) % max(1, world), 0)


class CpuRingEngine:

    def __init__(self, device: int = 0, sig_cap: int = 1 << 20, span_cap: int = 16384, group_cap: int = 64, user_cap: int = 1 << 18,
                 n_buffers: int = 3, window_ms: float = 2000.0, threshold: float = 0.7, fanout: int = 3,
                 group_mode: int = 1, n_dom: int = N_DOMAINS, ttft_slo_ms: float = 800.0, halo_ms: float = 0.0,
                 import_cap: int = 0, xchg_cap: int = 0, shard_rank: int = 0, shard_world: int = 1, group=None,
                 halo_windows: int = 3, split_rings: bool = False, **_native_only):
        from ..parallel.exchange import ExchangeModel, torch_allgather

        self.sig_cap, self.span_cap, self.group_cap, self.user_cap = sig_cap, span_cap, group_cap, user_cap
        self.buffers = int(n_buffers)
        self.window_ms_, self.threshold, self.fanout, self.group_mode = window_ms, threshold, fanout, group_mode
        self.n_dom, self.ttft_slo_ms = n_dom, float(ttft_slo_ms)
        self.shard_rank, self.shard_world = int(shard_rank), int(shard_world)
        self.split_rings = bool(split_rings)
        self.group = group
        if group is not None:
            import torch.distributed as dist

            self.rank, self.world = dist.get_rank(group), dist.get_world_size(group)
        else:
            self.rank, self.world = 0, 1
        self.xm = ExchangeModel(self.rank, self.world, halo_ms, import_cap, xchg_cap if self.world > 1 else 0,
                                torch_allgather(group) if group is not None else None, halo_windows=halo_windows)
        self.table, self.tmap = oracle.CtxTable(), oracle.TraceMap()
        self.pod_sn: Dict[int, int] = {}
        self.model = None
        self.app = None
        self.win: Dict[int, dict] = {}
        self._totals = np.zeros(PACKET_LEN)
        self._stats_acc = np.zeros(STATS_LEN)
        self.windows_folded = 0
        self.graphs = 0
        self.staged_bytes = self.direct_bytes = 0
        self.host_issue_us = self.host_wait_us = self.host_dma_issue_us = self.host_launch_us = 0.0
        self.host_pre_us = self.host_tail_us = 0.0
        self.host_dma_split_us = [0.0, 0.0, 0.0, 0.0]

    @property
    def has_comm(self) -> bool:
        return self.group is not None and self.world > 1

    def register_host(self, addr: int, n: int) -> bool:
        return True

    def set_model_bytes(self, b) -> None:
        from ..ops.engine import model_from_bytes

        self.model_image = np.ascontiguousarray(b, dtype=np.uint8).copy()
        self.model = model_from_bytes(self.model_image)

    def model_bytes(self) -> np.ndarray:
        return self.model_image.copy()

    def set_app_model(self, b) -> None:
        from ..ops.engine import app_from_bytes

        self.app = app_from_bytes(b, self.n_dom)

    def set_p0(self, p0) -> None:
        pass

    def set_pods(self, pods, sn) -> None:
        self.pod_sn.update(zip(np.asarray(pods).tolist(), np.asarray(sn).tolist()))

    def init_comm(self, *a) -> None:
        raise RuntimeError("the CPU engine communicates over its torch.distributed group (gloo)")

    def submit(self, k: int, kernel, user, spans, n_groups: int, labels, bases, with_labels: bool, learn: bool,
               user_rec: int) -> None:
        t0 = time.perf_counter()
        framed = _gather(kernel)
        words = records.REC_STRIDE // 4
        fr = framed.view(np.uint32).reshape(-1, words) if len(framed) else np.zeros((0, words), np.uint32)
        busy = np.nonzero(fr[:, 0] & np.uint32(records.RB_BUSY))[0] if len(fr) else np.zeros(0, np.int64)
        first_busy = int(busy[0]) * records.BATCH_SLOTS if len(busy) else -1
        oracle.apply_ring_defs(framed, self.table, self.tmap, self.pod_sn)
        if first_busy >= 0:
            fr = fr.copy()
            fr[int(busy[0]):, 0] = np.uint32(records.RB_BUSY | records.REC_PAYLOAD)
            framed = fr.view(np.uint8).reshape(-1)
        ub = _gather(user)
        udt = {64: records.EVENT, 32: records.USER32, 24: records.USER24, 16: records.USER16}[int(user_rec)]
        u = ub.view(udt) if len(ub) else np.zeros(0, dtype=udt)
        d = oracle.decode_window(framed, u, self.table, self.tmap, bases, pod_sn=self.pod_sn)
        hdr, sl = records.framed_slots(framed) if len(fr) else (np.zeros(0, np.uint32), np.zeros((0, 4), np.uint32))
        valid_k = (hdr == records.REC_PAYLOAD) & ((sl[:, 1] & np.uint32(0xFF)) < records.DEF_FIRST)
        other = 0
        u_rec = u["pid_sig"] != np.uint32(records.USER16_CONT) if u.dtype == records.USER16 else np.ones(len(u), bool)
        is_rec = np.concatenate([valid_k, u_rec])
        if self.shard_world > 1 and not self.split_rings:
            mine = shard_owner(d.svcnode, self.shard_world) == self.shard_rank
            drop = is_rec & ~mine
            other = int(drop.sum())
            d = _holes(d, drop)
            is_rec = is_rec & ~drop
        events = int(valid_k.sum()) + int(u_rec.sum()) - other
        sp = _gather(spans)
        spr = oracle.spans_native(sp.view(records.SPAN) if len(sp) else np.zeros(0, records.SPAN))
        counted = (spr["flags"] & np.uint32(records.SPAN_NO_SLI)) == 0
        G = int(n_groups)
        grp_local = spr["group_id"].astype(np.int64)
        if self.shard_world > 1:
            mine_sp = grp_local % self.shard_world == self.shard_rank
            spr["ts_ns"] = np.where(mine_sp, spr["ts_ns"], 0)
            grp_local = grp_local // self.shard_world
            spr["group_id"] = grp_local.astype(spr["group_id"].dtype)
        else:
            mine_sp = np.ones(len(spr), bool)
        n_loc = len(d.ts)
        res = self.xm.window(d, spr, G, window_ms=self.window_ms_, threshold=self.threshold, fanout=self.fanout,
                             group_mode=self.group_mode)
        hist = oracle.histograms(d)
        status = np.zeros((16, 3), dtype=np.int64)
        ok = d.slot != oracle.NO_SLOT
        np.add.at(status, (d.slot[ok].astype(np.int64), d.status[ok].astype(np.int64)), 1)
        misc = np.zeros(PACKET_LAYOUT[2], dtype=np.int64)
        misc[0] = int(((~ok) & is_rec).sum())
        misc[1] = int(((d.ts == 0) & is_rec).sum())
        misc[2:18] = oracle.value_sums_milli(d)
        dbg = np.zeros(PACKET_LAYOUT[3], dtype=np.int64)
        dbg[0] = res.debug["candidates"]
        dbg[1] = res.debug["low_confidence"]
        dbg[3] = res.debug["fanout_dropped"]
        dbg[4] = res.debug["spans_enriched"]
        dbg[5], dbg[6] = self.xm.xchg_dropped, self.xm.import_dropped
        feat = res.feat.astype(np.float32)
        f64 = feat.astype(np.float64)
        D = self.n_dom
        post = np.zeros((G, 16))
        pred = np.zeros(G, np.int32)
        gconf = np.zeros(G)
        evbits = np.zeros((G, 16), np.uint32)
        okg = mine_sp & (grp_local >= 0) & (grp_local < G)
        app = app_counts(spr, G, mine=okg, groups=grp_local)
        if G and self.model is not None:
            self.model.app = self.app
            st = self.app.state(app, feat) if self.app is not None else None
            post[:, :D] = self.model.posteriors(f64, st)
            pred = self.model.predict(f64, st).astype(np.int32)
            gconf = post[np.arange(G), pred]
            evbits[:, :D] = self.model.evidence_bits(f64, st)
        conf = np.zeros((16, 16), dtype=np.int64)
        stats = SufficientStats()
        if labels is not None and G:
            lab = np.asarray(labels, dtype=np.int64)[:G]
            m = lab >= 0
            if with_labels:
                np.add.at(conf, (lab[m] & 0xFF, pred[m]), 1)
            if learn and m.any():
                stats.add(f64[m], soft_labels(lab[m]))
        sli = np.zeros((G, 2), np.uint32)
        late = np.zeros((G, 2), np.uint32)
        breach = spr["ttft_ms"] > np.float32(self.ttft_slo_ms)
        is_late = breach & ((spr["flags"] & np.uint32(records.SPAN_LATE)) != 0)
        ok = okg & counted
        np.add.at(sli[:, 0], grp_local[ok & ~is_late], 1)
        np.add.at(sli[:, 1], grp_local[ok & breach & ~is_late], 1)
        np.add.at(late[:, 0], grp_local[ok & is_late], 1)
        ring = np.zeros(PACKET_LAYOUT[7])
        ring[:7] = (first_busy, 0, 0, 0, 0, events, other)
        pk = build_packet(hist, status, misc, dbg, conf, stats)
        pk[PACKET_LEN - PACKET_LAYOUT[7]:] = ring
        out = {"post": post, "conf": gconf, "feat": feat, "pred": pred, "evbits": evbits, "sli": sli, "app": app,
               "late": late}
        outs = [out]
        if self.has_comm:
            import torch
            import torch.distributed as dist

            t = torch.from_numpy(pk[:PACKET_LEN - PACKET_LAYOUT[7]].copy())
            dist.all_reduce(t, group=self.group)
            pk[:PACKET_LEN - PACKET_LAYOUT[7]] = t.numpy()
            outs = [None] * self.world
            dist.all_gather_object(outs, out, group=self.group)
        self._totals += pk
        if learn:
            self._stats_acc += pk[STATS_OFF:STATS_OFF + STATS_LEN]
        ms = 1e3 * (time.perf_counter() - t0)
        self.win[k % max(1, self.buffers)] = {"k": k, "packet": pk, "res": out, "all": outs, "ms": ms,
                                             "rows": (n_loc, res.n_rows)}

    def _w(self, k: int) -> dict:
        w = self.win.get(k % max(1, self.buffers))
        if w is None or w["k"] != k:
            raise KeyError(f"window {k} is not held (only the last {self.buffers})")
        return w

    def h2d_done(self, k: int) -> bool:
        return True

    def wait_h2d(self, k: int) -> None:
        pass

    def query(self, k: int) -> bool:
        return True

    def wait(self, k: int) -> None:
        self._w(k)

    def packet(self, k: int) -> np.ndarray:
        return self._w(k)["packet"].copy()

    @staticmethod
    def _cut(r: dict, G: int) -> dict:
        return {key: np.asarray(v)[:G].copy() for key, v in r.items()}

    def results(self, k: int, n_groups: int) -> dict:
        return self._cut(self._w(k)["res"], n_groups)

    def results_all(self, k: int, n_groups: int) -> list:
        return [self._cut(r, n_groups) for r in self._w(k)["all"]]

    def window_ms(self, k: int):
        ms = self._w(k)["ms"]
        return ms, ms

    def copy_ms(self, k: int):
        return [0.0, 0.0]

    def inject_remote(self, blocks, stride, world, me) -> None:
        from ..parallel.exchange import parse_block

        b = np.ascontiguousarray(blocks, dtype=np.uint8)
        for r in range(world):
            if r != me:
                self.xm.injected = oracle.concat(self.xm.injected, parse_block(b[r * stride:(r + 1) * stride]))

    def import_state(self):
        return []

    def totals(self) -> np.ndarray:
        return self._totals.copy()

    def reset_totals(self) -> None:
        self._totals[:] = 0

    def stats_acc(self) -> np.ndarray:
        return self._stats_acc.copy()

    def restore(self, stats, model, folded) -> None:
        if stats is not None and len(stats) == STATS_LEN:
            self._stats_acc = np.asarray(stats, dtype=np.float64).copy()
        if len(model):
            self.set_model_bytes(model)

    def set_refit(self, alpha: float, prior_pseudo: float, inv_temp: float, min_count: float, cap_dom: int = -1,
                  ceil: float = 1.0) -> None:
        self.refit_params = (float(alpha), float(prior_pseudo), float(inv_temp), float(min_count), int(cap_dom),
                             float(ceil))

    def refit_now(self) -> None:
        pass

    def set_device_refit(self, on: bool) -> None:
        pass

    def sync(self) -> None:
        pass

    def close(self) -> None:
        self.win.clear()


def _holes(d: oracle.Decoded, m: np.ndarray) -> oracle.Decoded:
    out = oracle.Decoded(*(getattr(d, f).copy() for f in oracle.Decoded.__dataclass_fields__))
    for f, z in (("ts", 0), ("val", 0), ("slot", oracle.NO_SLOT), ("status", 0), ("pod", 0), ("pid", 0),
                 ("svcnode", 0), ("trace", 0), ("conn", 0)):
        getattr(out, f)[m] = z
    return out
```

### llm_slo_ebpf_toolkit_amd/pipeline/window.py

```python

from __future__ import annotations

import os
import time
from dataclasses import dataclass, field
from typing import Dict, List, Optional, Sequence, Tuple

import numpy as np

from ..collector import records
from ..models.bayes import LDA, N_DOMAINS, NaiveBayes, SufficientStats
from ..models.metrics import macro_f1_from_confusion
from ..signals import catalog

PACKET_LAYOUT = (256, 48, 18, 8, 256, 1024, 16, 8)
RS, BS = records.REC_STRIDE, records.BATCH_SLOTS
RING_FIELDS = ("first_busy", "foreign", "def_ctx", "def_trace", "discarded", "events", "other_shard")
USER_CAP = 1 << 18


def unpack_packet(p: np.ndarray) -> Dict[str, np.ndarray]:
    o = 0
    out = {}
    for name, n in zip(("hist", "status", "misc", "dbg", "confusion", "stats", "count", "ring"), PACKET_LAYOUT):
        out[name] = p[o:o + n]
        o += n
    out["hist"] = out["hist"].reshape(16, 16)
    out["status"] = out["status"].reshape(16, 3)
    out["confusion"] = out["confusion"].reshape(16, 16)
    out["stats"] = out["stats"].reshape(32, 32)
    out["value_sum"] = out["misc"][2:18] * 1e-3
    out["ring_state"] = {k: int(v) for k, v in zip(RING_FIELDS, out["ring"][:len(RING_FIELDS)])}
    return out


def stats_from_packet(p: Dict[str, np.ndarray]) -> SufficientStats:
    st = p["stats"]
    D = N_DOMAINS
    return SufficientStats(count=p["count"][:D].copy(), elevated_sum=st[:16, :D].copy(),
                           x_sum=st[16:, :D].copy(), xx=st[16:, 16:].copy())


def summarize(p: np.ndarray) -> Dict[str, object]:
    u = unpack_packet(p)
    conf = u["confusion"][:N_DOMAINS, :N_DOMAINS].astype(np.int64)
    return {
        "confusion": conf,
        "macro_f1": macro_f1_from_confusion(conf),
        "accuracy": float(np.trace(conf) / conf.sum()) if conf.sum() else 0.0,
        "hist": u["hist"].astype(np.int64),
        "status": u["status"].astype(np.int64),
        "dbg": u["dbg"].astype(np.int64),
        "misc": u["misc"].astype(np.int64),
        "ring": u["ring"].astype(np.int64),
        "stats": stats_from_packet(u),
    }


class WindowPipeline:

    def __init__(self, sig_cap: int, span_cap: int, group_cap: int, device: int = 0, comm=None,
                 model: str = "bayes_learned", seed: int = 42, window_ms: float = 2000.0, threshold: float = 0.7,
                 fanout: int = 3, group_mode: int = 1, learn: bool = True, use_graphs: bool = True,
                 max_ahead: int = 3, n_buffers: int = 3, user_cap: int = USER_CAP, ttft_slo_ms: float = 800.0,
                 halo_ms: float = 0.0, import_cap: int = 0, xchg_cap: int = 0, shard: Tuple[int, int] = (0, 1),
                 engine: str = "gpu", group=None, model_image: Optional[np.ndarray] = None, halo_windows: int = 3,
                 split_rings: bool = False, open_requests: int = 0, open_ttl_ms: float = 120000.0,
                 open_reorder_ms: Optional[float] = None, sli_sketch: int = 0, exemplars: int = 0,
                 exemplar_windows: int = 3, pod_breakdown: int = 0, pod_windows: int = 3, pod_pairs: int = 4096,
                 breach_onset: int = 0, onset_bin_ns: Optional[int] = None, onset_ref_ppm: int = 20000,
                 onset_alarm: int = 3):
        from ..ops.engine import model_bytes

        self.model_name, self.seed, self.learn = model, seed, learn
        self.device_refit = learn and model == "bayes_learned" and engine == "gpu" and model_image is None
        self._model_bytes = model_bytes
        user_cap = max(1, min(int(user_cap), int(sig_cap)))
        kw = dict(device=device, sig_cap=sig_cap, span_cap=span_cap, group_cap=group_cap, user_cap=user_cap,
                  n_buffers=n_buffers, window_ms=window_ms, threshold=threshold, fanout=fanout, group_mode=group_mode,
                  n_dom=N_DOMAINS, ttft_slo_ms=ttft_slo_ms, halo_ms=halo_ms, import_cap=import_cap, xchg_cap=xchg_cap,
                  shard_rank=int(shard[0]), shard_world=int(shard[1]), halo_windows=int(halo_windows),
                  split_rings=bool(split_rings))
        self.engine_kind = engine
        if engine == "cpu":
            from .cpu import CpuRingEngine

            self.mod = None
            self.stats_off, self.stats_len = sum(PACKET_LAYOUT[:5]), PACKET_LAYOUT[5] + PACKET_LAYOUT[6]
            self.eng = CpuRingEngine(group=group, **kw)
        elif engine == "gpu":
            from ..ops import load_agent

            self.mod = load_agent()
            if tuple(self.mod.PACKET_LAYOUT) != PACKET_LAYOUT:
                raise RuntimeError("stale _mislo_agent build: packet layout mismatch (rebuild with ops.build)")
            self.stats_off, self.stats_len = int(self.mod.STATS_OFF), int(self.mod.STATS_LEN)
            if os.environ.get("MISLO_GRAPHS", "") == "0":
                use_graphs = False
            self.eng = self.mod.WindowEngine(max_ahead=max_ahead, use_graphs=use_graphs,
                                             device_refit=self.device_refit, **kw)
        else:
            raise ValueError(f"unknown window engine {engine!r} (gpu | cpu)")
        self.halo_ms, self.import_cap, self.xchg_cap = halo_ms, import_cap, xchg_cap
        self.shard = (int(shard[0]), int(shard[1]))
        self.nb = self.eng.buffers
        self.sig_cap, self.span_cap, self.group_cap, self.user_cap = sig_cap, span_cap, group_cap, user_cap
        if comm is not None and comm[2] >= 1:
            self.eng.init_comm(comm[0], comm[1], comm[2])
        p0 = np.zeros((16, 16), dtype=np.float64)
        p0[:, :N_DOMAINS] = NaiveBayes.random_init_table(seed)
        self.eng.set_p0(p0.ravel())
        self.learned_kw: Dict[str, object] = {"seed": seed}
        self.cum_stats = SufficientStats()
        if model_image is not None:
            from ..ops.engine import model_from_bytes

            self.model = model_from_bytes(model_image)
            self.eng.set_model_bytes(np.ascontiguousarray(model_image, dtype=np.uint8))
        else:
            self.model = self._initial_model()
            self.eng.set_model_bytes(model_bytes(self.model))
        self.k = 0
        self.windows_folded_host = 0
        self.tracker = None
        self.open_skipped = 0
        self._open: Dict[int, Tuple[int, Optional[int]]] = {}
        if open_requests:
            if comm is not None or group is not None or int(shard[1]) > 1:
                raise ValueError("open-request tracking runs on one GPU: no communicator, no sharding "
                                 "(every GPU's results are gathered on the device)")
            tkw = dict(cap=int(open_requests), span_cap=span_cap, group_cap=group_cap, n_buffers=self.nb,
                       slo_ms=ttft_slo_ms, ttl_ms=open_ttl_ms,
                       reorder_ms=2.0 * window_ms if open_reorder_ms is None else open_reorder_ms, device=device)
            if engine == "gpu":
                from ..ops.openreq import OpenRequestTable

                self.tracker = OpenRequestTable(**tkw)
            else:
                from .openreq import OpenRequestOracle

                self.tracker = OpenRequestOracle(**tkw)
        self.sketch = None
        self._sli: Dict[int, Tuple[int, int]] = {}
        if sli_sketch:
            if comm is not None or group is not None or int(shard[1]) > 1:
                raise ValueError("the TTFT sketch runs on one GPU: no communicator, no sharding "
                                 "(every GPU's results are gathered on the device)")
            skw = dict(span_cap=span_cap, group_cap=group_cap, windows=int(sli_sketch), n_buffers=self.nb,
                       device=device)
            if engine == "gpu":
                from ..ops.slisketch import SliSketch

                self.sketch = SliSketch(**skw)
            else:
                from .slisketch import SliSketchOracle

                self.sketch = SliSketchOracle(**skw)
        self.exemplars = None
        self._ex: Dict[int, Tuple[int, int]] = {}
        if exemplars:
            if comm is not None or group is not None or int(shard[1]) > 1:
                raise ValueError("request exemplars run on one GPU: no communicator, no sharding "
                                 "(every GPU's results are gathered on the device)")
            ekw = dict(k=int(exemplars), windows=int(exemplar_windows), span_cap=span_cap, group_cap=group_cap,
                       n_buffers=self.nb, device=device)
            if engine == "gpu":
                from ..ops.exemplars import ExemplarTracker

                self.exemplars = ExemplarTracker(**ekw)
            else:
                from .exemplars import ExemplarOracle

                self.exemplars = ExemplarOracle(**ekw)
        self.pods = None
        self._pod: Dict[int, Tuple[int, int]] = {}
        if pod_breakdown:
            if comm is not None or group is not None or int(shard[1]) > 1:
                raise ValueError("the pod breakdown runs on one GPU: no communicator, no sharding "
                                 "(every GPU's results are gathered on the device)")
            pkw = dict(k=int(pod_breakdown), windows=int(pod_windows), pair_cap=int(pod_pairs), span_cap=span_cap,
                       group_cap=group_cap, n_buffers=self.nb, slo_ms=ttft_slo_ms, device=device)
            if engine == "gpu":
                from ..ops.podrank import PodRankTracker

                self.pods = PodRankTracker(**pkw)
            else:
                from .podrank import PodRankOracle

                self.pods = PodRankOracle(**pkw)
        self.onset = None
        self.onset_skipped = 0
        self._onset: Dict[int, Tuple[int, Optional[int]]] = {}
        if breach_onset:
            if comm is not None or group is not None or int(shard[1]) > 1:
                raise ValueError("the breach onset runs on one GPU: no communicator, no sharding "
                                 "(every GPU's results are gathered on the device)")
            bin_ns = max(1_000_000, int(round(window_ms * 1e6 / 16))) if onset_bin_ns is None else int(onset_bin_ns)
            okw = dict(bins=int(breach_onset), bin_ns=bin_ns, ref_ppm=int(onset_ref_ppm), alarm=int(onset_alarm),
                       span_cap=span_cap, group_cap=group_cap, n_buffers=self.nb, slo_ms=ttft_slo_ms, device=device)
            if engine == "gpu":
                from ..ops.onset import OnsetTracker

                self.onset = OnsetTracker(**okw)
            else:
                from .onset import OnsetOracle

                self.onset = OnsetOracle(**okw)

    def _initial_model(self):
        if self.model_name == "bayes":
            return NaiveBayes.ref()
        if self.model_name == "bayes_gpu":
            return NaiveBayes.gpu()
        return NaiveBayes.learned(SufficientStats(), seed=self.seed)

    def set_prior(self, init: Optional[np.ndarray] = None, floor: Optional[np.ndarray] = None,
                  cap_domain: Optional[str] = None, ceil: Optional[float] = None) -> None:
        p0 = np.zeros((2, 16, 16), dtype=np.float64)
        p0[0, :, :N_DOMAINS] = init if init is not None else NaiveBayes.random_init_table(self.seed)
        if floor is not None:
            p0[1, :, :N_DOMAINS] = floor
        self.eng.set_p0(p0.ravel())
        self.learned_kw = {"seed": self.seed, "init": init, "floor": floor, "cap_domain": cap_domain, "ceil": ceil}

    def lik_ceil(self) -> float:
        c = self.learned_kw.get("ceil")
        return 1.0 if c is None else float(c)

    def cap_dom(self) -> int:
        c = self.learned_kw.get("cap_domain")
        return -1 if c is None else catalog.DOMAIN_INDEX[str(c)]

    def submit(self, kernel, user, spans, n_groups: int, labels=None, bases=(0, 0, 0, 0), with_labels: bool = True,
               learn: Optional[bool] = None, user_rec: int = 64) -> int:
        if user_rec in (16, 24) and not any(int(b) for b in bases) and any(int(n) for _, n in user):
            raise ValueError("USER24 records need the window's epoch bases (all are 0)")
        k = self.k
        learn = (self.learn and with_labels) if learn is None else learn
        lab = None if labels is None else np.ascontiguousarray(labels, dtype=np.int32)
        self.eng.submit(k, list(kernel), list(user), list(spans), int(n_groups), lab, [int(b) for b in bases],
                        bool(with_labels), bool(learn), int(user_rec))
        self.k += 1
        if self.learn and not self.device_refit and k >= 2:
            self._host_refit(k - 2)
        return k

    def _host_refit(self, j: int) -> None:
        self.eng.wait(j)
        pk = unpack_packet(self.eng.packet(j))
        self.cum_stats = self.cum_stats.merge(stats_from_packet(pk))
        self.windows_folded_host += 1
        if self.model_name == "lda" and self.cum_stats.count.sum() > 32:
            self.model = LDA.fit(self.cum_stats)
        elif self.model_name in ("bayes_learned", "lda"):
            self.model = NaiveBayes.learned(self.cum_stats, **self.learned_kw)
        self.model.app = getattr(self, "app", None)
        self.eng.set_model_bytes(self._model_bytes(self.model))

    def wait(self, k: int) -> None:
        self.eng.wait(k)

    def packet(self, k: int) -> Dict[str, np.ndarray]:
        self.eng.wait(k)
        return unpack_packet(self.eng.packet(k))

    def results(self, k: int, n_groups: int) -> Dict[str, np.ndarray]:
        self.eng.wait(k)
        res = self.eng.results(k, n_groups)
        if self.tracker is not None:
            from .openreq import correct_results

            res = correct_results(res, self.open_results(k, n_groups))
        if self.sketch is not None:
            from .slisketch import result_keys

            res = dict(res)
            res.update(result_keys(self.sli_results(k, n_groups)))
        if self.exemplars is not None:
            from .exemplars import result_keys as exemplar_keys

            res = dict(res)
            res.update(exemplar_keys(self.exemplar_results(k, n_groups)))
        if self.pods is not None:
            from .podrank import result_keys as pod_keys

            res = dict(res)
            res.update(pod_keys(self.pod_results(k, n_groups)))
        if self.onset is not None:
            from .onset import result_keys as onset_keys

            res = dict(res)
            res.update(onset_keys(self.onset_results(k, n_groups)))
        return res

    def track_open(self, spans, cut_ns: int, prev_cut_ns: int, n_groups: int) -> None:
        if self.tracker is None:
            return
        step = None
        if int(cut_ns) > 0:
            step = self.tracker.step(list(spans), int(cut_ns), min(int(prev_cut_ns), int(cut_ns)), int(n_groups))
        else:
            self.open_skipped += 1
        self._open[self.k % self.nb] = (self.k, step)

    def open_results(self, k: int, n_groups: int) -> Dict[str, np.ndarray]:
        held = self._open.get(k % self.nb)
        if held is not None and held[0] == k and held[1] is not None:
            return self.tracker.results(held[1], n_groups)
        from .openreq import N_STATS

        return {"dl": np.zeros((n_groups, 2), np.uint32), "dup": np.zeros((n_groups, 3), np.uint32),
                "stats": np.zeros(N_STATS, np.uint32)}

    def track_sli(self, spans, n_groups: int) -> None:
        if self.sketch is None:
            return
        self._sli[self.k % self.nb] = (self.k, self.sketch.step(list(spans), int(n_groups)))

    def sli_results(self, k: int, n_groups: int) -> Dict[str, np.ndarray]:
        held = self._sli.get(k % self.nb)
        if held is not None and held[0] == k:
            return self.sketch.results(held[1], n_groups)
        from .slisketch import empty_result

        return empty_result(n_groups)

    def track_exemplars(self, spans, n_groups: int) -> None:
        if self.exemplars is None:
            return
        self._ex[self.k % self.nb] = (self.k, self.exemplars.step(list(spans), int(n_groups)))

    def exemplar_results(self, k: int, n_groups: int) -> Dict[str, np.ndarray]:
        held = self._ex.get(k % self.nb)
        if held is not None and held[0] == k:
            return self.exemplars.results(held[1], n_groups)
        from .exemplars import empty_result

        return empty_result(n_groups, self.exemplars.k)

    def track_pods(self, spans, n_groups: int) -> None:
        if self.pods is None:
            return
        self._pod[self.k % self.nb] = (self.k, self.pods.step(list(spans), int(n_groups)))

    def pod_results(self, k: int, n_groups: int) -> Dict[str, np.ndarray]:
        held = self._pod.get(k % self.nb)
        if held is not None and held[0] == k:
            return self.pods.results(held[1], n_groups)
        from .podrank import empty_result

        return empty_result(n_groups, self.pods.k)

    def track_onset(self, spans, cut_ns: int, n_groups: int) -> None:
        if self.onset is None:
            return
        step = None
        if int(cut_ns) > 0:
            step = self.onset.step(list(spans), int(cut_ns), int(n_groups))
        else:
            self.onset_skipped += 1
        self._onset[self.k % self.nb] = (self.k, step)

    def onset_results(self, k: int, n_groups: int) -> Dict[str, np.ndarray]:
        held = self._onset.get(k % self.nb)
        if held is not None and held[0] == k and held[1] is not None:
            return self.onset.results(held[1], n_groups)
        from .onset import empty_result

        return empty_result(n_groups)

    def close(self) -> None:
        if self.tracker is not None:
            self.tracker.close()
        if self.onset is not None:
            self.onset.close()
        if self.pods is not None:
            self.pods.close()
        if self.exemplars is not None:
            self.exemplars.close()
        if self.sketch is not None:
            self.sketch.close()
        self.eng.close()

    def results_all(self, k: int, n_groups: int) -> List[Dict[str, np.ndarray]]:
        self.eng.wait(k)
        return self.eng.results_all(k, n_groups)

    def inject_remote(self, blocks: np.ndarray, world: int, me: int) -> None:
        self.eng.inject_remote(np.ascontiguousarray(blocks, dtype=np.uint8), len(blocks) // world, world, me)

    def window_ms(self, k: int):
        return self.eng.window_ms(k)

    def set_model(self, model) -> None:
        self.model = model
        self.eng.set_model_bytes(self._model_bytes(model))
        if getattr(self, "app", None) is not None and model.app is None:
            model.app = self.app
        if model.app is not None:
            self.set_app(model.app)

    def set_app(self, app) -> None:
        from ..ops.engine import app_model_bytes

        self.app = app
        self.model.app = app
        self.eng.set_app_model(app_model_bytes(self.model))

    def drain(self) -> None:
        self.eng.sync()
        if self.tracker is not None:
            self.tracker.sync()
        if self.sketch is not None:
            self.sketch.sync()
        if self.exemplars is not None:
            self.exemplars.sync()
        if self.pods is not None:
            self.pods.sync()
        if self.onset is not None:
            self.onset.sync()

    def reset_totals(self) -> None:
        self.eng.reset_totals()

    @property
    def windows_folded(self) -> int:
        return int(self.eng.windows_folded) + self.windows_folded_host

    def summary(self) -> Dict[str, object]:
        return summarize(self.eng.totals())

    def state(self) -> Tuple[Dict[str, np.ndarray], Dict[str, object]]:
        self.drain()
        c = self.cum_stats
        stats = np.asarray(self.eng.stats_acc(), dtype=np.float64).copy()
        off, n = self.stats_off, self.stats_len
        pending = range(max(0, self.k - self.nb), self.k) if self.device_refit else range(0)
        for j in pending:
            stats += np.asarray(self.eng.packet(j), dtype=np.float64)[off:off + n]
        arrays = {"stats_acc": stats,
                  "model": np.asarray(self.eng.model_bytes(), dtype=np.uint8),
                  "host_count": c.count, "host_elevated_sum": c.elevated_sum, "host_x_sum": c.x_sum,
                  "host_xx": c.xx}
        meta = {"model": self.model_name, "seed": self.seed, "learn": self.learn, "windows": self.k,
                "windows_folded_device": int(self.eng.windows_folded) + len(pending),
                "windows_folded_host": self.windows_folded_host, "n_domains": N_DOMAINS}
        return arrays, meta

    def restore(self, arrays: Dict[str, np.ndarray], meta: Dict[str, object]) -> None:
        if meta.get("model") != self.model_name or int(meta.get("n_domains", N_DOMAINS)) != N_DOMAINS:
            raise ValueError(f"checkpoint of model {meta.get('model')!r} cannot resume {self.model_name!r}")
        model = np.zeros(0, np.uint8) if self.device_refit else np.asarray(arrays["model"], dtype=np.uint8)
        self.eng.restore(np.asarray(arrays["stats_acc"], dtype=np.float64), model,
                         int(meta.get("windows_folded_device", 0)))
        self.cum_stats = SufficientStats(count=np.array(arrays["host_count"], dtype=np.float64),
                                         elevated_sum=np.array(arrays["host_elevated_sum"], dtype=np.float64),
                                         x_sum=np.array(arrays["host_x_sum"], dtype=np.float64),
                                         xx=np.array(arrays["host_xx"], dtype=np.float64))
        self.windows_folded_host = int(meta.get("windows_folded_host", 0))
        if not self.device_refit and self.learn and self.cum_stats.count.sum() > 0:
            if self.model_name == "lda" and self.cum_stats.count.sum() > 32:
                self.model = LDA.fit(self.cum_stats)
            else:
                self.model = NaiveBayes.learned(self.cum_stats, **self.learned_kw)

    def save_checkpoint(self, path: str, extra_meta: Optional[Dict[str, object]] = None) -> None:
        from ..utils import checkpoint

        arrays, meta = self.state()
        meta.update(extra_meta or {})
        checkpoint.save(path, arrays, meta)

    def load_checkpoint(self, path: str) -> Dict[str, object]:
        from ..utils import checkpoint

        arrays, meta = checkpoint.load(path)
        self.restore(arrays, meta)
        return meta

    def host_model(self):
        if not self.device_refit:
            return self.model
        st = self.eng.stats_acc()
        s = SufficientStats(count=st[1024:1024 + N_DOMAINS].copy(),
                            elevated_sum=st[:1024].reshape(32, 32)[:16, :N_DOMAINS].copy(),
                            x_sum=st[:1024].reshape(32, 32)[16:, :N_DOMAINS].copy(),
                            xx=st[:1024].reshape(32, 32)[16:, 16:].copy())
        return NaiveBayes.learned(s, **self.learned_kw)



@dataclass
class Cut:
    kernel: int = (1 << 64) - 1
    user: int = (1 << 64) - 1
    spans: int = (1 << 64) - 1
    bases: Sequence[int] = (0, 0, 0, 0)
    t_ns: int = 0


class RingWindowSource:

    def __init__(self, pipe: WindowPipeline, ring=None, user_ring=None, span_ring=None, cfg_set=None,
                 shared: bool = False, flush=None):
        from ..runtime import load

        self.rt = load()
        self.pipe = pipe
        self.ring, self.user_ring, self.span_ring = ring, user_ring, span_ring
        if cfg_set is None and ring is not None and getattr(ring, "emulated", False):
            cfg_set = lambda i, v: ring.cfg_set(i, v)
        self.cfg_set = cfg_set
        self.flush = flush
        self.clock = records.EpochClock()
        self.direct = {}
        if ring is not None:
            self.direct["ring"] = pipe.eng.register_host(ring.data_address, ring.size)
            self.kpos = ring.consumer_pos
            self.kmask = ring.size - 1
        self.user_rec = int(user_ring.rec_size) if user_ring is not None else 64
        if self.user_rec not in (16, 24, 32, 64):
            raise ValueError(f"user ring holds {self.user_rec}-byte records (EVENT = 64, USER32 = 32, USER24 = 24, "
                             "USER16 = 16)")
        if user_ring is not None:
            self.direct["user"] = pipe.eng.register_host(user_ring.address, user_ring.capacity * self.user_rec)
            self.upos = user_ring.tail
        if span_ring is not None:
            self.direct["spans"] = pipe.eng.register_host(span_ring.address, span_ring.capacity * 64)
            self.spos = span_ring.tail
        self.shared = shared
        self.kernel_done = self.kpos if ring is not None else 0
        self.kernel_seen = self.kernel_done
        self.user_done = self.upos if user_ring is not None else 0
        self.span_done = self.spos if span_ring is not None else 0
        self.pending: List[tuple] = []
        self.late: List[tuple] = []
        self.late_dropped = 0
        self.last: Dict[str, int] = {}
        self.host_s = 0.0
        self.n = 0
        self.resubmitted = 0
        self.carried = 0
        self.reap_s = self.submit_s = 0.0
        self.prev_cut_ns = 0

    def publish_epoch(self, now_ns: Optional[int] = None) -> int:
        v = self.clock.publish(int(now_ns if now_ns is not None else time.time_ns()))
        if self.cfg_set is not None:
            self.cfg_set(self.rt.CFG_EPOCH, v)
        return v

    def cut(self, now_ns: Optional[int] = None) -> Cut:
        t = int(now_ns if now_ns is not None else time.time_ns())
        self.publish_epoch(t)
        if self.flush is not None:
            self.flush()
        return Cut(kernel=self.ring.producer_pos if self.ring is not None else 0,
                   user=self.user_ring.head if self.user_ring is not None else 0,
                   spans=self.span_ring.head if self.span_ring is not None else 0,
                   bases=self.clock.bases(), t_ns=t)

    def reap(self, keep: Optional[int] = None) -> None:
        eng = self.pipe.eng
        while self.pending and (eng.query(self.pending[0][0]) or (keep is not None and len(self.pending) > keep)):
            k, ranges, nu, ns, released = self.pending.pop(0)
            eng.wait(k)
            if not released:
                self._release_user(nu, ns)
            fb = int(eng.packet(k)[sum(PACKET_LAYOUT[:7])])
            if fb >= 0:
                skip = fb // BS
                for pos, n, k0 in ranges:
                    if skip >= n:
                        skip -= n
                        continue
                    self.late.append((pos + RS * skip, n - skip, k0))
                    self.resubmitted += BS * (n - skip)
                    skip = 0
            if ranges:
                self.kernel_seen = max(self.kernel_seen, max(p + RS * n for p, n, _ in ranges))
        if self.ring is not None:
            hold = min([p for p, _, _ in self.late] + [p for e in self.pending for p, _, _ in e[1]], default=None)
            self.kernel_done = max(self.kernel_done, min(hold, self.kernel_seen) if hold is not None else self.kernel_seen)
            if not self.shared:
                self.ring.set_consumer_pos(max(self.ring.consumer_pos, self.kernel_done))
        for e in self.pending:
            if not e[4] and eng.h2d_done(e[0]):
                self._release_user(e[2], e[3])
                e[4] = True

    def _release_user(self, nu: int, ns: int) -> None:
        self.user_done += nu
        self.span_done += ns
        if self.shared:
            return
        if self.user_ring is not None and nu:
            self.user_ring.release(nu)
        if self.span_ring is not None and ns:
            self.span_ring.release(ns)

    def done(self) -> Tuple[int, int, int]:
        return int(self.kernel_done), int(self.user_done), int(self.span_done)

    def _kernel_segments(self, pos: int, nbytes: int) -> List[Tuple[int, int]]:
        idx = pos & self.kmask
        first = min(nbytes, self.ring.size - idx)
        out = [(self.ring.data_address + idx, first)]
        if nbytes > first:
            out.append((self.ring.data_address, nbytes - first))
        return out

    def _ring_ranges(self, start: int, stop: int, rec: int, base: int, cap_pos: int, max_n: int):
        n = max(0, min(stop - start, max_n))
        out, pos, left = [], start, n
        while left:
            idx = pos & (cap_pos - 1)
            take = min(left, cap_pos - idx)
            out.append((base + idx * rec, take * rec))
            pos += take
            left -= take
        return out, n

    def stage(self, cut: Cut, n_groups: int, labels: Optional[np.ndarray] = None, with_labels: Optional[bool] = None,
              learn: Optional[bool] = None) -> Dict[str, int]:
        t0 = time.perf_counter()
        pipe = self.pipe
        self.reap(keep=pipe.nb - 1)
        t1 = time.perf_counter()
        self.reap_s += t1 - t0
        budget = pipe.sig_cap
        k_ranges, kern = [], []
        n_k = 0
        if self.ring is not None:
            late, self.late = self.late, []
            for pos, n, k0 in late:
                if pipe.k - k0 >= 3:
                    self.late_dropped += BS * n
                    continue
                take = min(n, (budget - n_k) // BS)
                if take < n:
                    self.late.append((pos + RS * take, n - take, k0))
                if take:
                    k_ranges.append((pos, take, k0))
                    kern += self._kernel_segments(pos, RS * take)
                    n_k += BS * take
            span_b = cut.kernel - self.kpos
            if span_b % RS:
                raise RuntimeError("BPF ring holds records of another size (the probes emit 8-slot batches only)")
            take = min(span_b // RS, (budget - n_k) // BS)
            self.carried += BS * (span_b // RS - take)
            if take:
                k_ranges.append((self.kpos, take, pipe.k))
                kern += self._kernel_segments(self.kpos, RS * take)
                n_k += BS * take
                self.kpos += RS * take
        user, n_u = [], 0
        if self.user_ring is not None:
            cap = self.user_ring.capacity
            user, n_u = self._ring_ranges(self.upos, cut.user, self.user_rec, self.user_ring.address, cap,
                                          min(pipe.user_cap, budget - n_k))
            self.carried += max(0, cut.user - self.upos) - n_u
            self.upos += n_u
        spans, n_s = [], 0
        if self.span_ring is not None:
            spans, n_s = self._ring_ranges(self.spos, cut.spans, 64, self.span_ring.address, self.span_ring.capacity,
                                           pipe.span_cap)
            self.carried += max(0, cut.spans - self.spos) - n_s
            self.spos += n_s
        wl = labels is not None if with_labels is None else with_labels
        if pipe.tracker is not None:
            pipe.track_open(spans, cut.t_ns, self.prev_cut_ns, n_groups)
            if int(cut.t_ns) > 0:
                self.prev_cut_ns = int(cut.t_ns)
        if pipe.sketch is not None:
            pipe.track_sli(spans, n_groups)
        if pipe.exemplars is not None:
            pipe.track_exemplars(spans, n_groups)
        if pipe.pods is not None:
            pipe.track_pods(spans, n_groups)
        if pipe.onset is not None:
            pipe.track_onset(spans, cut.t_ns, n_groups)
        t2 = time.perf_counter()
        k = pipe.submit(kern, user, spans, n_groups, labels, cut.bases, with_labels=wl, learn=learn,
                        user_rec=self.user_rec)
        self.submit_s += time.perf_counter() - t2
        self.pending.append([k, k_ranges, n_u, n_s, False])
        self.host_s += time.perf_counter() - t0
        self.n += 1
        self.last = {"k": k, "n_kernel": n_k, "n_user": n_u, "n_spans": n_s, "n_events": n_k + n_u}
        return self.last

    def step(self, n_groups: int, labels=None, cut: Optional[Cut] = None, with_labels: Optional[bool] = None) -> int:
        c = cut if cut is not None else self.cut()
        return self.stage(c, n_groups, labels, with_labels)["k"]

    def group_sli(self, k: int) -> np.ndarray:
        return self.pipe.results(k, self.pipe.group_cap)["sli"].astype(np.float64)

    def drain(self) -> None:
        self.pipe.drain()
        self.reap(keep=0)


@dataclass
class ReplayImage:
    framed: np.ndarray
    spans: np.ndarray
    user: np.ndarray
    bases: tuple
    n_groups: int
    labels: np.ndarray
    domains: List[List[str]] = field(default_factory=list)
    n_kernel: int = 0


def kernel_event_mask(events: np.ndarray) -> np.ndarray:
    from ..signals import catalog

    gpu_types = np.array([s.kernel_type for s in catalog.SIGNALS if s.name in catalog.GPU_SIGNALS], dtype=np.uint16)
    return ~np.isin(events["signal_type"], gpu_types)


def build_replay_images(windows, shift=None, window_ns: int = 1_000_000_000, sim_ring=None,
                        user_rec: int = 64) -> List[ReplayImage]:
    from ..runtime import load

    rt = load()
    shift = records.milli_shift_table() if shift is None else shift
    own = sim_ring is None
    if own:
        sim_ring = rt.Ringbuf.create_shm(f"/mislo-sim-{os.getpid()}-{id(windows)}", 1 << 16)
    sim = rt.ProbeSim(sim_ring, shift)
    clock = records.EpochClock()
    out = []
    for i, w in enumerate(windows):
        if i == 0:
            sim_ring.cfg_set(rt.CFG_EPOCH, clock.publish(int(w.t0_ns) - window_ns))
        km = kernel_event_mask(w.events)
        kev = np.ascontiguousarray(w.events[km])
        early = (kev["ts_ns"] < int(w.t0_ns)) & (kev["ts_ns"] != 0)
        parts = [sim.encode(np.ascontiguousarray(kev[early]), flush=False)]
        sim_ring.cfg_set(rt.CFG_EPOCH, clock.publish(int(w.t0_ns)))
        parts.append(sim.encode(np.ascontiguousarray(kev[~early]), flush=True))
        payload = np.concatenate(parts)
        uev = np.ascontiguousarray(w.events[~km])
        out.append(ReplayImage(framed=rt.frame_records(payload), spans=np.ascontiguousarray(w.spans),
                               user=records.to_user(uev, user_rec), bases=clock.bases(),
                               n_groups=w.n_groups,
                               labels=np.asarray(w.group_labels, dtype=np.int32), domains=list(w.group_domains),
                               n_kernel=int(km.sum())))
    return out


def build_shard_images(windows, world: int, pods, window_ns: int = 1_000_000_000,
                       user_rec: int = 64) -> List[List[ReplayImage]]:
    import dataclasses

    from ..collector.bpf import ShardRouter

    router = ShardRouter(world)
    router.set_pods(*pods)
    per_shard = []
    for r in range(world):
        ws = []
        for w in windows:
            ev = w.events[router.pod_shard(w.events["pod_id"]) == r]
            sp = w.spans[router.span_shard(w.spans) == r]
            ws.append(dataclasses.replace(w, events=np.ascontiguousarray(ev), spans=np.ascontiguousarray(sp)))
        per_shard.append(build_replay_images(ws, window_ns=window_ns, user_rec=user_rec))
    return [[per_shard[r][j] for r in range(world)] for j in range(len(windows))]
```

Before: 2.429 billion.

## Split window submit into copy-ahead H2D phase and chain phase

Splits engine submission into submit_copy (issue the H2D DMA for a window) and submit_chain (queue the compute chain). The worker now issues window k's copy before collecting older windows and waiting on compute_done, so the host-to-device transfer overlaps prior compute. Copy-completion events move into a separate ring of 2*nb marks so copies can run ahead of the buffer's compute cycle. It also adds an on-request second copy lane, warmed with a dummy transfer. The cost is more state-machine complexity and an extra front_done sync before buffer reuse, and the path only activates when no trackers, sketches, exemplars, pods or onset are configured.

```diff
diff --git a/llm_slo_ebpf_toolkit_amd/agent/worker.py b/llm_slo_ebpf_toolkit_amd/agent/worker.py
--- a/llm_slo_ebpf_toolkit_amd/agent/worker.py
+++ b/llm_slo_ebpf_toolkit_amd/agent/worker.py
@@ -145,6 +145,7 @@
         self.pending: Deque[Tuple[int, float, int]] = collections.deque()
         self.windows = 0
         self.collect_s = self.collect_wait_s = 0.0
+        self.pipe.prepare_copy_ahead()
 
     @classmethod
     def adopt(cls, spec: WorkerSpec, pipe, src) -> "WorkerCore":
@@ -154,6 +155,7 @@
         core.pending = collections.deque()
         core.windows = 0
         core.collect_s = core.collect_wait_s = 0.0
+        pipe.prepare_copy_ahead()
         return core
 
     @property
@@ -163,6 +165,8 @@
     def window(self, cut, n_groups: int, pods=None, labels=None) -> dict:
         if pods is not None and len(pods[0]):
             self.pipe.eng.set_pods(*pods)
+        if self.pipe.copy_ahead:
+            return self._window_copy_ahead(cut, n_groups, labels)
         t0 = time.perf_counter()
         r = self.src.stage(cut, n_groups, labels, with_labels=labels is not None, learn=False)
         host_us = 1e6 * (time.perf_counter() - t0)
@@ -171,6 +175,25 @@
         prevs = []
         while len(self.pending) > 1 and (len(self.pending) > self.max_pending or
                                          self.pipe.eng.query(self.pending[0][0])):
+            prevs.append(self._collect(*self.pending.popleft()))
+        out["prevs"] = prevs
+        self.windows += 1
+        return out
+
+    def _window_copy_ahead(self, cut, n_groups: int, labels) -> dict:
+        src = self.src
+        t0 = time.perf_counter()
+        src.stage_copy(cut, n_groups, labels)
+        t1 = time.perf_counter()
+        prevs = []
+        while len(self.pending) > self.max_pending:
+            prevs.append(self._collect(*self.pending.popleft()))
+        t2 = time.perf_counter()
+        r = src.stage_chain(with_labels=labels is not None, learn=False)
+        host_us = 1e6 * ((t1 - t0) + (time.perf_counter() - t2))
+        out = {"rank": self.spec.rank, "k": r["k"], "staged": r, "done": src.done()}
+        self.pending.append((r["k"], host_us, n_groups))
+        while len(self.pending) > 1 and self.pipe.eng.query(self.pending[0][0]):
             prevs.append(self._collect(*self.pending.popleft()))
         out["prevs"] = prevs
         self.windows += 1
diff --git a/llm_slo_ebpf_toolkit_amd/ops/csrc/agent_bindings.cpp b/llm_slo_ebpf_toolkit_amd/ops/csrc/agent_bindings.cpp
--- a/llm_slo_ebpf_toolkit_amd/ops/csrc/agent_bindings.cpp
+++ b/llm_slo_ebpf_toolkit_amd/ops/csrc/agent_bindings.cpp
@@ -82,10 +82,28 @@
   bool register_host(uintptr_t addr, size_t bytes) {
     return e_->register_host(reinterpret_cast<const void*>(addr), bytes);
   }
-  void submit(int64_t k, const std::vector<std::pair<uintptr_t, size_t>>& kernel,
-              const std::vector<std::pair<uintptr_t, size_t>>& user,
-              const std::vector<std::pair<uintptr_t, size_t>>& spans, int n_groups, py::object labels,
-              std::vector<int64_t> bases, bool with_labels, bool learn, int user_rec) {
+  using Ranges = std::vector<std::pair<uintptr_t, size_t>>;
+  void submit(int64_t k, const Ranges& kernel, const Ranges& user, const Ranges& spans, int n_groups,
+              py::object labels, std::vector<int64_t> bases, bool with_labels, bool learn, int user_rec) {
+    std::vector<int32_t> lab;
+    const WindowInput in = window_input(kernel, user, spans, n_groups, labels, std::move(bases), user_rec, lab);
+    py::gil_scoped_release nogil;
+    e_->submit(k, in, with_labels, learn);
+  }
+  void submit_copy(int64_t k, const Ranges& kernel, const Ranges& user, const Ranges& spans, int n_groups,
+                   py::object labels, std::vector<int64_t> bases, int user_rec) {
+    std::vector<int32_t> lab;
+    const WindowInput in = window_input(kernel, user, spans, n_groups, labels, std::move(bases), user_rec, lab);
+    py::gil_scoped_release nogil;
+    e_->submit_copy(k, in);
+  }
+  void submit_chain(int64_t k, int n_groups, bool with_labels, bool learn) {
+    py::gil_scoped_release nogil;
+    e_->submit_chain(k, n_groups, with_labels, learn);
+  }
+  static WindowInput window_input(const Ranges& kernel, const Ranges& user, const Ranges& spans, int n_groups,
+                                  py::object labels, std::vector<int64_t> bases, int user_rec,
+                                  std::vector<int32_t>& lab) {
     WindowInput in;
     auto conv = [](const std::vector<std::pair<uintptr_t, size_t>>& v, std::vector<Seg>& out) {
       for (auto& p : v) out.push_back(Seg{reinterpret_cast<const void*>(p.first), p.second});
@@ -95,7 +113,6 @@
     conv(spans, in.spans);
     in.n_groups = n_groups;
     in.user_rec = user_rec;
-    std::vector<int32_t> lab;
     if (!labels.is_none()) {
       auto arr = labels.cast<py::array_t<int32_t, py::array::c_style | py::array::forcecast>>();
       lab.assign(arr.data(), arr.data() + arr.size());
@@ -104,8 +121,7 @@
     }
     bases.resize(4, 0);
     for (int q = 0; q < 4; ++q) in.bases[q] = bases[q];
-    py::gil_scoped_release nogil;
-    e_->submit(k, in, with_labels, learn);
+    return in;
   }
   bool h2d_done(int64_t k) { return e_->h2d_done(k); }
   void wait_h2d(int64_t k) {
@@ -836,6 +852,11 @@
       .def("submit", &PyEngine::submit, py::arg("k"), py::arg("kernel"), py::arg("user"), py::arg("spans"),
            py::arg("n_groups"), py::arg("labels") = py::none(), py::arg("bases") = std::vector<int64_t>{},
            py::arg("with_labels") = true, py::arg("learn") = false, py::arg("user_rec") = 64)
+      .def("submit_copy", &PyEngine::submit_copy, py::arg("k"), py::arg("kernel"), py::arg("user"), py::arg("spans"),
+           py::arg("n_groups"), py::arg("labels") = py::none(), py::arg("bases") = std::vector<int64_t>{},
+           py::arg("user_rec") = 64)
+      .def("submit_chain", &PyEngine::submit_chain, py::arg("k"), py::arg("n_groups"), py::arg("with_labels") = true,
+           py::arg("learn") = false)
       .def("h2d_done", &PyEngine::h2d_done)
       .def("wait_h2d", &PyEngine::wait_h2d)
       .def("query", &PyEngine::query)
@@ -871,6 +892,11 @@
       .def("close", &PyEngine::close)
       .def_property_readonly("buffers", &PyEngine::buffers)
       .def_property_readonly("copy_lanes", [](PyEngine& p) { return p.eng().copy_lanes(); })
+      .def_property_readonly("copy_ahead", [](PyEngine& p) { return p.eng().copy_ahead(); })
+      .def("take_copy_lanes", [](PyEngine& p) {
+        py::gil_scoped_release nogil;
+        return p.eng().take_copy_lanes();
+      })
       .def_property_readonly("windows_folded", &PyEngine::folded)
       .def_property_readonly("graphs", &PyEngine::graphs)
       .def_property_readonly("host_issue_us", &PyEngine::host_issue_us)
diff --git a/llm_slo_ebpf_toolkit_amd/ops/csrc/copylanes.h b/llm_slo_ebpf_toolkit_amd/ops/csrc/copylanes.h
--- a/llm_slo_ebpf_toolkit_amd/ops/csrc/copylanes.h
+++ b/llm_slo_ebpf_toolkit_amd/ops/csrc/copylanes.h
@@ -13,6 +13,9 @@
   for (int i = 0; i < (lanes > 1 ? lanes : 1) && k - i >= 0; ++i) out[n++] = k - i;
   return n;
 }
+
+inline int copy_mark_slots(int nb) { return 2 * nb; }
+inline int copy_mark_slot(int64_t k, int nb) { return (int)(k % copy_mark_slots(nb)); }
 
 struct CopiedUpTo {
   int64_t n = 0;
diff --git a/llm_slo_ebpf_toolkit_amd/ops/csrc/engine.h b/llm_slo_ebpf_toolkit_amd/ops/csrc/engine.h
--- a/llm_slo_ebpf_toolkit_amd/ops/csrc/engine.h
+++ b/llm_slo_ebpf_toolkit_amd/ops/csrc/engine.h
@@ -102,9 +102,13 @@
 
   bool register_host(const void* ptr, size_t bytes);
   void submit(int64_t k, const WindowInput& in, bool with_labels, bool learn);
+  void submit_copy(int64_t k, const WindowInput& in);
+  void submit_chain(int64_t k, int n_groups, bool with_labels, bool learn);
+  bool copy_ahead() const { return copy_ahead_; }
   bool h2d_done(int64_t k);
   void wait_h2d(int64_t k);
   int copy_lanes() const { return lanes_; }
+  bool take_copy_lanes();
   bool query(int64_t k);
   void wait(int64_t k);
   const double* packet(int64_t k) const { return bufs_[k % nb_].packet_host; }
@@ -240,11 +244,16 @@
     uint32_t* remote_n;
     const BufSet* set;
     const GenMeta* gen_prev;
-    hipEvent_t h2d_done, head_done, front_done, compute_done, comm_done, xchg_done;
-    hipEvent_t t_start, t_comp0, t_comp1, t_end;
+    hipEvent_t head_done, front_done, compute_done, comm_done, xchg_done;
+    hipEvent_t t_comp0, t_comp1, t_end;
     const int* counts() const { return reinterpret_cast<const int*>(in); }
   };
   std::vector<Buf> bufs_;
+  struct CopyMark {
+    hipEvent_t t_start, h2d_done;
+  };
+  std::vector<CopyMark> marks_;
+  const CopyMark& mark(int64_t k) const { return marks_[copy_mark_slot(k, nb_)]; }
   hipEvent_t ev_fork_ = nullptr, ev_sigbase_ = nullptr, ev_spans_ = nullptr;
   bool branch_ = false;
   bool xspan_ = false;
@@ -253,6 +262,11 @@
   int nblk_sig_ = 1, nblk_span_ = 1;
   hipStream_t copy_[kMaxCopyLanes] = {nullptr, nullptr};
   int lanes_ = 1;
+  bool copy_ahead_ = false;
+  bool lane_on_request_ = false;
+  bool copy_open_ = false;
+  int copy_groups_ = 0;
+  int64_t copied_windows() const { return submitted_ + (copy_open_ ? 1 : 0); }
   CopiedUpTo copied_;
   bool copied_ready(int64_t w, bool block);
   hipStream_t compute_ = nullptr, comm_stream_ = nullptr;
diff --git a/llm_slo_ebpf_toolkit_amd/ops/csrc/engine.hip b/llm_slo_ebpf_toolkit_amd/ops/csrc/engine.hip
--- a/llm_slo_ebpf_toolkit_amd/ops/csrc/engine.hip
+++ b/llm_slo_ebpf_toolkit_amd/ops/csrc/engine.hip
@@ -66,6 +66,7 @@
                      static_cast<uint4*>(dst), n16);
 }
 
+constexpr int kCopyAheadDefault = 1;
 constexpr unsigned kEvWait = hipEventDisableTiming | hipEventBlockingSync;
 int env_int(const char* name, int unset) {
   const char* v = getenv(name);
@@ -190,7 +191,10 @@
   overlap_ = env_int("MISLO_WINDOW_OVERLAP", !one_stream) == 1 && !one_stream &&
              !(cfg_.xchg_cap > 0 && cfg_.import_cap > 0);
   if (overlap_) front_ = mk_stream();
-  lanes_ = overlap_ && env_int("MISLO_COPY_LANES", nb_ >= 4 ? 2 : 1) == 2 ? 2 : 1;
+  copy_ahead_ = overlap_ && env_int("MISLO_COPY_AHEAD", kCopyAheadDefault) == 1;
+  const char* lanes_env = getenv("MISLO_COPY_LANES");
+  lanes_ = overlap_ && (lanes_env ? atoi(lanes_env) == 2 : nb_ >= 4) ? 2 : 1;
+  lane_on_request_ = copy_ahead_ && !lanes_env && lanes_ == 1 && nb_ >= 3;
   copy_[1] = lanes_ == 2 ? mk_stream(env_int("MISLO_COPY_LANE_PRIO", 1) != 0) : copy_[0];
   slots_ = gens_ + (overlap_ ? 1 : 0);
   {
@@ -211,13 +215,16 @@
     buf.packet_host = static_cast<double*>(host_block(kPacketLen * sizeof(double)));
     for (hipEvent_t* e : {&buf.head_done, &buf.compute_done, &buf.comm_done, &buf.front_done, &buf.xchg_done})
       *e = mk_event(kEvWait);
-    buf.h2d_done = mk_event(hipEventBlockingSync);
-    for (hipEvent_t* e : {&buf.t_start, &buf.t_comp0, &buf.t_comp1, &buf.t_end})
-      *e = mk_event(hipEventDefault);
+    for (hipEvent_t* e : {&buf.t_comp0, &buf.t_comp1, &buf.t_end}) *e = mk_event(hipEventDefault);
     buf.res_host = static_cast<uint8_t*>(host_block(lay.bytes()));
     buf.res_dev = dalloc<uint8_t>(lay.bytes(), true);
     buf.res = lay.view(buf.res_dev);
     buf.imp = cfg_.import_cap ? dalloc<SigRec>(cfg_.import_cap) : nullptr;
+  }
+  marks_.assign((size_t)copy_mark_slots(nb_), CopyMark{});
+  for (CopyMark& m : marks_) {
+    m.t_start = mk_event(hipEventDefault);
+    m.h2d_done = mk_event(hipEventBlockingSync);
   }
   warm_.assign(kStageSlots * nb_, false);
   pod_sn_ = dalloc<uint32_t>(kPodRows, true);
@@ -361,7 +368,7 @@
 }
 
 bool WindowEngine::copied_ready(int64_t w, bool block) {
-  const hipEvent_t ev = bufs_[w % nb_].h2d_done;
+  const hipEvent_t ev = mark(w).h2d_done;
   if (block) {
     HIPCHECK(hipEventSynchronize(ev));
     return true;
@@ -373,12 +380,12 @@
 }
 
 bool WindowEngine::h2d_done(int64_t k) {
-  if (k < 0 || k >= submitted_) return false;
+  if (k < 0 || k >= copied_windows()) return false;
   return copied_.done(k, lanes_, [this](int64_t w) { return copied_ready(w, false); });
 }
 
 void WindowEngine::wait_h2d(int64_t k) {
-  if (k < 0 || k >= submitted_) throw std::invalid_argument("wait_h2d: the window has not been submitted");
+  if (k < 0 || k >= copied_windows()) throw std::invalid_argument("wait_h2d: the window has not been submitted");
   copied_.done(k, lanes_, [this](int64_t w) { return copied_ready(w, true); });
 }
 
@@ -554,9 +561,42 @@
                   p0_ + kSlots * 16, cfg_.cap_dom, cfg_.lik_ceil);
 }
 
+bool WindowEngine::take_copy_lanes() {
+  if (!lane_on_request_ || copy_open_) return lanes_ == 2;
+  lane_on_request_ = false;
+  HIPCHECK(hipSetDevice(cfg_.device));
+  const hipStream_t lane = mk_stream(env_int("MISLO_COPY_LANE_PRIO", 1) != 0);
+  const size_t n = std::min<size_t>(in_bytes_ - off_kern_, size_t(64) << 20);
+  void *h = nullptr, *d = nullptr;
+  hipError_t e = hipHostMalloc(&h, 2 * n, hipHostMallocDefault);
+  if (e == hipSuccess) e = hipMalloc(&d, 2 * n);
+  if (e == hipSuccess) {
+    std::memset(h, 0, 2 * n);
+    uint8_t *hp = static_cast<uint8_t*>(h), *dp = static_cast<uint8_t*>(d);
+    for (int round = 0; round < 2 && e == hipSuccess; ++round) {
+      e = hipMemcpyAsync(dp, hp, n, hipMemcpyHostToDevice, copy_[0]);
+      if (e == hipSuccess) e = hipMemcpyAsync(dp + n, hp + n, n, hipMemcpyHostToDevice, lane);
+    }
+    const hipError_t e0 = hipStreamSynchronize(copy_[0]), e1 = hipStreamSynchronize(lane);
+    if (e == hipSuccess) e = e0 != hipSuccess ? e0 : e1;
+  }
+  if (d) (void)hipFree(d);
+  if (h) (void)hipHostFree(h);
+  HIPCHECK(e);
+  copy_[1] = lane;
+  lanes_ = 2;
+  return true;
+}
+
 void WindowEngine::submit(int64_t k, const WindowInput& in, bool with_labels, bool learn) {
+  submit_copy(k, in);
+  submit_chain(k, in.n_groups, with_labels, learn);
+}
+
+void WindowEngine::submit_copy(int64_t k, const WindowInput& in) {
   Lap whole;
   if (k != submitted_) throw std::invalid_argument("windows must be submitted in order");
+  if (copy_open_) throw std::logic_error("submit_copy: the window's chain phase has not been queued");
   const int n_groups = in.n_groups;
   if (n_groups < 0 || n_groups > cfg_.group_cap) throw std::invalid_argument("n_groups exceeds group capacity");
   size_t kb = 0, ub = 0, sb = 0;
@@ -570,12 +610,14 @@
   if (n_k + n_u > (size_t)cfg_.sig_cap || n_u > (size_t)cfg_.user_cap || n_s > (size_t)cfg_.span_cap)
     throw std::invalid_argument("window exceeds the engine's capacity (events / user records / spans)");
   Buf& buf = bufs_[k % nb_];
+  const CopyMark& mk = mark(k);
   Lap phase;
-  if (k >= max_ahead_) HIPCHECK(hipEventSynchronize(bufs_[(k - max_ahead_) % nb_].compute_done));
+  if (!copy_ahead_ && k >= max_ahead_) HIPCHECK(hipEventSynchronize(bufs_[(k - max_ahead_) % nb_].compute_done));
   if (k >= nb_) {
-    HIPCHECK(hipEventSynchronize(buf.h2d_done));
+    HIPCHECK(hipEventSynchronize(mark(k - nb_).h2d_done));
     copied_.reused(k, nb_);
     HIPCHECK(hipEventSynchronize(buf.head_done));
+    if (copy_ahead_) HIPCHECK(hipEventSynchronize(buf.front_done));
   }
   phase(wait_us_);
   int32_t* c = reinterpret_cast<int32_t*>(buf.head_host);
@@ -595,7 +637,7 @@
   int32_t* lab = reinterpret_cast<int32_t*>(buf.head_host + kHeadBytes);
   for (int g = 0; g < cfg_.group_cap; ++g) lab[g] = (in.labels && g < n_groups) ? in.labels[g] : -1;
   const hipStream_t cs = copy_[copy_lane(k, lanes_)];
-  HIPCHECK(hipEventRecord(buf.t_start, cs));
+  HIPCHECK(hipEventRecord(mk.t_start, cs));
   size_t st_off = 0;
   Lap part;
   dma(in.kernel, buf.in + off_kern_, kern_bytes(), buf.staging, st_off, cs);
@@ -605,10 +647,24 @@
   part(split_us_[2]);
   dma(in.spans, buf.in + off_span_, 64 * (size_t)cfg_.span_cap, buf.staging, st_off, cs);
   part(split_us_[3]);
-  HIPCHECK(hipEventRecord(buf.h2d_done, cs));
+  HIPCHECK(hipEventRecord(mk.h2d_done, cs));
   phase(dma_us_);
+  copy_open_ = true;
+  copy_groups_ = n_groups;
+  whole(issue_us_);
+}
+
+void WindowEngine::submit_chain(int64_t k, int n_groups, bool with_labels, bool learn) {
+  Lap whole;
+  if (!copy_open_ || k != submitted_) throw std::logic_error("submit_chain: not the window submit_copy queued last");
+  if (n_groups != copy_groups_) throw std::invalid_argument("submit_chain: n_groups differs from the copy phase's");
+  Buf& buf = bufs_[k % nb_];
+  const CopyMark& mk = mark(k);
+  Lap phase;
+  if (copy_ahead_ && k >= max_ahead_) HIPCHECK(hipEventSynchronize(bufs_[(k - max_ahead_) % nb_].compute_done));
+  phase(wait_us_);
   hipStream_t fs = overlap_ ? front_ : compute_;
-  HIPCHECK(hipStreamWaitEvent(fs, buf.h2d_done, 0));
+  HIPCHECK(hipStreamWaitEvent(fs, mk.h2d_done, 0));
   if (overlap_ && k >= 2) HIPCHECK(hipStreamWaitEvent(fs, bufs_[(k - 2) % nb_].compute_done, 0));
   HIPCHECK(hipStreamWaitEvent(compute_, buf.comm_done, 0));
   const bool injected = !inject_.empty();
@@ -678,6 +734,7 @@
   HIPCHECK(hipEventRecord(buf.t_end, comm_stream_));
   HIPCHECK(hipEventRecord(buf.comm_done, comm_stream_));
   ++submitted_;
+  copy_open_ = false;
   phase(tail_us_);
   whole(issue_us_);
   ++issue_n_;
@@ -701,11 +758,11 @@
 }
 
 std::vector<float> WindowEngine::copy_ms(int64_t k) {
-  const Buf& buf = bufs_[k % nb_];
+  const CopyMark& mk = mark(k);
   float dur = 0.f, gap = -1.f;
-  HIPCHECK(hipEventSynchronize(buf.h2d_done));
-  HIPCHECK(hipEventElapsedTime(&dur, buf.t_start, buf.h2d_done));
-  if (k >= 1 && nb_ > 1) HIPCHECK(hipEventElapsedTime(&gap, bufs_[(k - 1) % nb_].h2d_done, buf.t_start));
+  HIPCHECK(hipEventSynchronize(mk.h2d_done));
+  HIPCHECK(hipEventElapsedTime(&dur, mk.t_start, mk.h2d_done));
+  if (k >= 1) HIPCHECK(hipEventElapsedTime(&gap, mark(k - 1).h2d_done, mk.t_start));
   return {dur, gap};
 }
 
@@ -713,7 +770,7 @@
   const Buf& buf = bufs_[k % nb_];
   float total = 0.f, comp = 0.f;
   HIPCHECK(hipEventSynchronize(buf.t_end));
-  HIPCHECK(hipEventElapsedTime(&total, buf.t_start, buf.t_end));
+  HIPCHECK(hipEventElapsedTime(&total, mark(k).t_start, buf.t_end));
   HIPCHECK(hipEventElapsedTime(&comp, buf.t_comp0, buf.t_comp1));
   return {total, comp};
 }
@@ -841,11 +898,12 @@
 void WindowEngine::init_comm(const ncclUniqueId& id, int rank, int world) {
   if (comm_) throw std::logic_error("communicator already initialised");
   if (world < 1 || rank < 0 || rank >= world) throw std::invalid_argument("communicator rank / world");
-  if (submitted_) throw std::logic_error("init_comm before the first window");
+  if (submitted_ || copy_open_) throw std::logic_error("init_comm before the first window");
   HIPCHECK(hipSetDevice(cfg_.device));
   if (overlap_) {
     HIPCHECK(hipStreamSynchronize(front_));
     overlap_ = false;
+    copy_ahead_ = lane_on_request_ = false;
     lanes_ = 1;
     if (!getenv("MISLO_SPAN_STREAM")) enable_span_branch();
   }
diff --git a/llm_slo_ebpf_toolkit_amd/pipeline/cpu.py b/llm_slo_ebpf_toolkit_amd/pipeline/cpu.py
--- a/llm_slo_ebpf_toolkit_amd/pipeline/cpu.py
+++ b/llm_slo_ebpf_toolkit_amd/pipeline/cpu.py
@@ -127,6 +127,7 @@
 
         self.sig_cap, self.span_cap, self.group_cap, self.user_cap = sig_cap, span_cap, group_cap, user_cap
         self.buffers = int(n_buffers)
+        self.copy_ahead = False
         self.window_ms_, self.threshold, self.fanout, self.group_mode = window_ms, threshold, fanout, group_mode
         self.n_dom, self.ttft_slo_ms = n_dom, float(ttft_slo_ms)
         self.shard_rank, self.shard_world = int(shard_rank), int(shard_world)
diff --git a/llm_slo_ebpf_toolkit_amd/pipeline/window.py b/llm_slo_ebpf_toolkit_amd/pipeline/window.py
--- a/llm_slo_ebpf_toolkit_amd/pipeline/window.py
+++ b/llm_slo_ebpf_toolkit_amd/pipeline/window.py
@@ -240,6 +240,35 @@
         lab = None if labels is None else np.ascontiguousarray(labels, dtype=np.int32)
         self.eng.submit(k, list(kernel), list(user), list(spans), int(n_groups), lab, [int(b) for b in bases],
                         bool(with_labels), bool(learn), int(user_rec))
+        self.k += 1
+        if self.learn and not self.device_refit and k >= 2:
+            self._host_refit(k - 2)
+        return k
+
+    @property
+    def copy_ahead(self) -> bool:
+        return bool(getattr(self.eng, "copy_ahead", False)) and all(
+            t is None for t in (self.tracker, self.sketch, self.exemplars, self.pods, self.onset))
+
+    def prepare_copy_ahead(self) -> bool:
+        if not self.copy_ahead:
+            return False
+        self.eng.take_copy_lanes()
+        return True
+
+    def submit_copy(self, kernel, user, spans, n_groups: int, labels=None, bases=(0, 0, 0, 0),
+                    user_rec: int = 64) -> int:
+        if user_rec in (16, 24) and not any(int(b) for b in bases) and any(int(n) for _, n in user):
+            raise ValueError("USER24 records need the window's epoch bases (all are 0)")
+        lab = None if labels is None else np.ascontiguousarray(labels, dtype=np.int32)
+        self.eng.submit_copy(self.k, list(kernel), list(user), list(spans), int(n_groups), lab,
+                             [int(b) for b in bases], int(user_rec))
+        return self.k
+
+    def submit_chain(self, n_groups: int, with_labels: bool = True, learn: Optional[bool] = None) -> int:
+        k = self.k
+        learn = (self.learn and with_labels) if learn is None else learn
+        self.eng.submit_chain(k, int(n_groups), bool(with_labels), bool(learn))
         self.k += 1
         if self.learn and not self.device_refit and k >= 2:
             self._host_refit(k - 2)
@@ -543,6 +572,8 @@
         self.carried = 0
         self.reap_s = self.submit_s = 0.0
         self.prev_cut_ns = 0
+        self.staged: Optional[list] = None
+        self._staged_groups = 0
 
     def publish_epoch(self, now_ns: Optional[int] = None) -> int:
         v = self.clock.publish(int(now_ns if now_ns is not None else time.time_ns()))
@@ -580,7 +611,8 @@
             if ranges:
                 self.kernel_seen = max(self.kernel_seen, max(p + RS * n for p, n, _ in ranges))
         if self.ring is not None:
-            hold = min([p for p, _, _ in self.late] + [p for e in self.pending for p, _, _ in e[1]], default=None)
+            held = self.pending + ([self.staged] if self.staged is not None else [])
+            hold = min([p for p, _, _ in self.late] + [p for e in held for p, _, _ in e[1]], default=None)
             self.kernel_done = max(self.kernel_done, min(hold, self.kernel_seen) if hold is not None else self.kernel_seen)
             if not self.shared:
                 self.ring.set_consumer_pos(max(self.ring.consumer_pos, self.kernel_done))
@@ -621,13 +653,8 @@
             left -= take
         return out, n
 
-    def stage(self, cut: Cut, n_groups: int, labels: Optional[np.ndarray] = None, with_labels: Optional[bool] = None,
-              learn: Optional[bool] = None) -> Dict[str, int]:
-        t0 = time.perf_counter()
+    def _take(self, cut: Cut):
         pipe = self.pipe
-        self.reap(keep=pipe.nb - 1)
-        t1 = time.perf_counter()
-        self.reap_s += t1 - t0
         budget = pipe.sig_cap
         k_ranges, kern = [], []
         n_k = 0
@@ -667,6 +694,16 @@
                                            pipe.span_cap)
             self.carried += max(0, cut.spans - self.spos) - n_s
             self.spos += n_s
+        return k_ranges, kern, n_k, user, n_u, spans, n_s
+
+    def stage(self, cut: Cut, n_groups: int, labels: Optional[np.ndarray] = None, with_labels: Optional[bool] = None,
+              learn: Optional[bool] = None) -> Dict[str, int]:
+        t0 = time.perf_counter()
+        pipe = self.pipe
+        self.reap(keep=pipe.nb - 1)
+        t1 = time.perf_counter()
+        self.reap_s += t1 - t0
+        k_ranges, kern, n_k, user, n_u, spans, n_s = self._take(cut)
         wl = labels is not None if with_labels is None else with_labels
         if pipe.tracker is not None:
             pipe.track_open(spans, cut.t_ns, self.prev_cut_ns, n_groups)
@@ -688,6 +725,42 @@
         self.host_s += time.perf_counter() - t0
         self.n += 1
         self.last = {"k": k, "n_kernel": n_k, "n_user": n_u, "n_spans": n_s, "n_events": n_k + n_u}
+        return self.last
+
+    def stage_copy(self, cut: Cut, n_groups: int, labels: Optional[np.ndarray] = None) -> int:
+        if not self.pipe.copy_ahead:
+            raise RuntimeError("stage_copy needs a pipeline with copy_ahead (use stage)")
+        if self.staged is not None:
+            raise RuntimeError("stage_copy: the previous window's stage_chain has not run")
+        t0 = time.perf_counter()
+        pipe = self.pipe
+        self.reap()
+        t1 = time.perf_counter()
+        self.reap_s += t1 - t0
+        k_ranges, kern, n_k, user, n_u, spans, n_s = self._take(cut)
+        t2 = time.perf_counter()
+        k = pipe.submit_copy(kern, user, spans, n_groups, labels, cut.bases, user_rec=self.user_rec)
+        self.submit_s += time.perf_counter() - t2
+        self.staged = [k, k_ranges, n_u, n_s, False]
+        self.last = {"k": k, "n_kernel": n_k, "n_user": n_u, "n_spans": n_s, "n_events": n_k + n_u}
+        self._staged_groups = n_groups
+        self.host_s += time.perf_counter() - t0
+        return k
+
+    def stage_chain(self, with_labels: bool = True, learn: Optional[bool] = None) -> Dict[str, int]:
+        if self.staged is None:
+            raise RuntimeError("stage_chain without stage_copy")
+        t0 = time.perf_counter()
+        pipe = self.pipe
+        self.reap(keep=pipe.nb - 1)
+        t1 = time.perf_counter()
+        self.reap_s += t1 - t0
+        pipe.submit_chain(self._staged_groups, with_labels=with_labels, learn=learn)
+        self.submit_s += time.perf_counter() - t1
+        self.pending.append(self.staged)
+        self.staged = None
+        self.host_s += time.perf_counter() - t0
+        self.n += 1
         return self.last
 
     def step(self, n_groups: int, labels=None, cut: Optional[Cut] = None, with_labels: Optional[bool] = None) -> int:
```

New measurement: 2.628 billion (median of 6 runs). 1.08x the previous value.
